# ShinYwings/SingleHDR-tf2

Hardware: AMD Instinct MI355X
Metric: HDR images/sec (512x512) end-to-end inference, deq+lin+hal (higher is better)
Workload: dtype f32

## Files before the change

include/shdr.h:

```cpp
#ifndef SHDR_H_
#define SHDR_H_

#include <stdint.h>

#ifdef __cplusplus
extern "C" {
#endif

void shdr_config_reload(void);

#define SHDR_OK          0
#define SHDR_E_SHAPE    (-1)
#define SHDR_E_ALIGN    (-2)
#define SHDR_E_ARCH     (-3)
#define SHDR_E_LAUNCH   (-4)
#define SHDR_E_NULL     (-5)

#define SHDR_ACT_NONE   0
#define SHDR_ACT_RELU   1
#define SHDR_ACT_LRELU  2
#define SHDR_ACT_TANH   3

#define SHDR_ALGO_AUTO    0
#define SHDR_ALGO_MFMA    1
#define SHDR_ALGO_DIRECT  2
#define SHDR_ALGO_MFMA_REG 3
#define SHDR_ALGO_MFMA_F16  4
#define SHDR_ALGO_MFMA_BF16 5
#define SHDR_ALGO_AUTO_F16  6
#define SHDR_ALGO_AUTO_BF16 7
#define SHDR_ALGO_AUTO_EXACT 8

const char* shdr_last_error(void);
const char* shdr_version(void);

uint32_t shdr_crc32c(const void* data, uint64_t n, uint32_t crc);

int shdr_same_pad(int in_size, int k, int stride, int* out_size, int* pad_before);

typedef struct shdr_conv2d_desc {
  int32_t N, H, W;
  int32_t C1, C2;
  int32_t Cout, KH, KW;
  int32_t stride;
  int32_t pad_t, pad_l;
  int32_t Ho, Wo;
  float   x2_scale;
  int32_t act1, act2;
  int32_t res_cstride;
  int32_t y_cstride;
  int32_t algo;
  int32_t cout_valid;
  int64_t w_batch_stride;
  int32_t y_pix_stride, y_off_h, y_off_w, y_H, y_W;
  int32_t prologue;
  int32_t pool;
} shdr_conv2d_desc;
enum { SHDR_POOL_MAX = 0, SHDR_POOL_AVG = 1 };
enum { SHDR_PROLOGUE_NONE = 0, SHDR_PROLOGUE_BILINEAR2X = 1,
       SHDR_PROLOGUE_RANGE_SCALE = 2 };

int shdr_conv2d_fwd_f32(const shdr_conv2d_desc* d,
                        const float* x1, const float* x2, const float* w,
                        const float* bias, const float* scale, const float* shift,
                        const float* residual, float* y, void* stream);

int shdr_conv2d_fwd_yrange_f32(const shdr_conv2d_desc* d,
                               const float* x1, const float* x2, const float* w,
                               const float* bias, const float* scale, const float* shift,
                               const float* residual, float* y, float* y_range, void* stream);

enum {
  SHDR_PLAN_DIRECT = 0,
  SHDR_PLAN_MFMA = 1,
  SHDR_PLAN_WINOGRAD_FUSED = 2,
  SHDR_PLAN_WINOGRAD_PLANES = 3,
  SHDR_PLAN_X3 = 4,
  SHDR_PLAN_X3N = 5
};
int shdr_conv2d_plan_f32(const shdr_conv2d_desc* d, int has_residual);
int64_t shdr_conv2d_prepared_filter_elems_f32(const shdr_conv2d_desc* d, int has_residual);
int shdr_conv2d_filter_is_plain_f32(const shdr_conv2d_desc* d, int has_residual);
int shdr_conv2d_prepare_filter_f32(const shdr_conv2d_desc* d, int has_residual, const float* w, float* prepared, void* stream);
int64_t shdr_conv2d_workspace_bytes_f32(const shdr_conv2d_desc* d, int has_residual);
int shdr_conv2d_fwd_prepared_f32(const shdr_conv2d_desc* d, const float* x1, const float* x2, const float* prepared,
                                 const float* bias, const float* scale, const float* shift, const float* residual, float* y,
                                 float* y_pool, void* workspace, void* stream);
int shdr_conv2d_fwd_prepared_ranged_f32(const shdr_conv2d_desc* d, const float* x1, const float* x2, const float* prepared,
                                        const float* bias, const float* scale, const float* shift, const float* residual, float* y,
                                        float* y_pool, void* workspace, const float* x1_range, const float* x2_range, float* y_range,
                                        void* stream);
int shdr_conv2d_projected_ok_f32(const shdr_conv2d_desc* d);
int shdr_conv2d_fwd_prepared_projected_f32(const shdr_conv2d_desc* d, const float* x1, const float* x2, const float* prepared,
                                           const float* bias, const float* scale, const float* shift, const float* proj, float* y_proj,
                                           float* y, float* y_pool, void* workspace, const float* x1_range, const float* x2_range,
                                           float* y_range, void* stream);

int shdr_conv2d_up2_lowres_ok_f32(const shdr_conv2d_desc* d);
int64_t shdr_conv2d_up2_lowres_filter_elems_f32(const shdr_conv2d_desc* d);
int shdr_conv2d_up2_lowres_prepare_filter_f32(const shdr_conv2d_desc* d, const float* w, float* prepared, void* stream);
int64_t shdr_conv2d_up2_lowres_workspace_bytes_f32(const shdr_conv2d_desc* d);
int shdr_conv2d_fwd_up2_lowres_f32(const shdr_conv2d_desc* d, const float* x, const float* prepared, const float* bias,
                                   const float* scale, const float* shift, float* y, void* workspace, const float* x_range,
                                   float* y_range, void* stream);

int shdr_conv2d_up2_fused_ok_f32(const shdr_conv2d_desc* d);
int shdr_conv2d_up2_narrow_enabled(void);
int64_t shdr_conv2d_up2_fused_filter_elems_f32(const shdr_conv2d_desc* d);
int shdr_conv2d_up2_fused_prepare_filter_f32(const shdr_conv2d_desc* d, const float* w, float* prepared, void* stream);
int shdr_conv2d_fwd_up2_fused_f32(const shdr_conv2d_desc* d, const float* x, const float* prepared, const float* bias,
                                  const float* scale, const float* shift, const float* proj, float* y_proj, float* y,
                                  const float* x_range, float* y_range, void* stream);

int shdr_conv2d_wgrad_f32(const shdr_conv2d_desc* d, const float* x, int which, const float* dz,
                          float* dw, void* stream);
int shdr_filter_transform_f32(const float* w, float* wt, int KH, int KW, int Cin, int Cout,
                              int c_begin, int c_count, float scale, void* stream);
int64_t shdr_conv2d_dgrad_workspace_bytes_f32(const shdr_conv2d_desc* d, int which);
int shdr_conv2d_dgrad_f32(const shdr_conv2d_desc* d, int which, const float* dz, const float* w, float* dx, void* workspace,
                          void* stream);
int shdr_conv2d_dgrad_tracks_range_f32(const shdr_conv2d_desc* d, int which);
int shdr_conv2d_dgrad_ranged_f32(const shdr_conv2d_desc* d, int which, const float* dz, const float* w, float* dx, void* workspace,
                                 const float* dz_range, float* dx_range, void* stream);
enum { SHDR_OP_CONV2D_FWD = 0, SHDR_OP_CONV2D_DGRAD = 1, SHDR_OP_CONV2D_WGRAD_WINOGRAD = 2, SHDR_OP_BATCHNORM = 3,
       SHDR_OP_ACT_BWD_BIAS = 4  };
#define SHDR_BN_MAX_BLOCKS 1024
int64_t shdr_workspace_bytes(int op, const shdr_conv2d_desc* d, int arg);
int shdr_bias_grad_f32(const float* dz, float* db, int64_t npix, int C, void* stream);

int shdr_soft_hist_fwd_f32(const float* x, float* y, int64_t npix, int C, int B, void* stream);
int shdr_soft_hist_bwd_f32(const float* x, const float* dy, float* dx, int64_t npix, int C, int B, void* stream);

int shdr_lin_frontend_fwd_f32(const float* img, float* y, int N, int H, int W,
                              int y_channels, void* stream);

int shdr_avgpool2_fwd_f32(const float* x, float* y, int N, int H, int W, int C, void* stream);
int shdr_maxpool2_fwd_f32(const float* x, float* y, int N, int H, int W, int C, void* stream);
int shdr_maxpool3s2_fwd_f32(const float* x, float* y, int N, int H, int W, int C, void* stream);
int shdr_resize2x_fwd_f32(const float* x, float* y, int N, int H, int W, int C, void* stream);
int shdr_gap_fwd_f32(const float* x, float* y, int N, int HW, int C, void* stream);

int shdr_invcrf_decode_fwd_f32(const float* feat, const float* wfc, const float* bfc,
                               const float* table, float* out, int B, int F, int K,
                               void* stream);
int shdr_increase_fwd_f32(const float* rf, float* out, int B, int K, void* stream);
int shdr_apply_rf_fwd_f32(const float* x, const float* rf, float* y, int B,
                          int64_t n_per_batch, int K, void* stream);

int shdr_clip_fwd_f32(const float* x, float* y, int64_t n, float lo, float hi, void* stream);
int shdr_vgg_preprocess_fwd_f32(const float* x, float* y, int64_t npix, int out_channels,
                                void* stream);
int shdr_reverse3_fwd_f32(const float* x, float* y, int64_t npix, void* stream);
int shdr_alpha_blend_fwd_f32(const float* b, const float* hal, float* a, float* alpha_out,
                             int64_t npix, float thr, void* stream);
int shdr_pack3_fwd_f32(const float* s0, const float* s1, const float* s2, const float* s3,
                       int nsrc, float* y, int out_channels, int64_t npix, void* stream);
int shdr_pad_channels_f32(const float* x, float* y, int64_t npix, int Cin, int Cout, void* stream);
int shdr_logc_fwd_f32(const float* x, float* y, int64_t n, void* stream);
int shdr_affine_act_f32(const float* x, const float* scale, const float* shift, const float* residual, float* y,
                        int64_t npix, int C, int act, void* stream);

int shdr_act_bwd_f32(const float* dy, const float* y, float* dx, int64_t n, int act, void* stream);
int shdr_clip_bwd_f32(const float* dy, const float* x, float* dx, int64_t n, float lo, float hi, void* stream);
int shdr_add_f32(const float* a, const float* b, float* y, int64_t n, void* stream);
int shdr_add_ranged_f32(const float* a, const float* b, float* y, int64_t n, float* y_range, void* stream);
int shdr_avgpool2_bwd_f32(const float* dy, float* dx, int N, int H, int W, int C, void* stream);
int shdr_maxpool2_bwd_f32(const float* x, const float* dy, float* dx, int N, int H, int W, int C, void* stream);
int shdr_maxpool3s2_bwd_f32(const float* x, const float* y, const float* dy, float* dx, int N, int H, int W, int C, void* stream);
int shdr_resize2x_bwd_f32(const float* dy, float* dx, int N, int H, int W, int C, void* stream);
int shdr_resize2x_bwd_ranged_f32(const float* dy, float* dx, int N, int H, int W, int C, float* dx_range, void* stream);
int shdr_gap_bwd_f32(const float* dy, float* dx, int N, int HW, int C, void* stream);
int shdr_upsample_zero2_f32(const float* dy, float* dx, int N, int H, int W, int C, void* stream);
int shdr_bn_stats_f32(const float* x, double* ws, float* mean, float* var, float* moving_mean,
                      float* moving_var, int64_t npix, int C, float momentum, void* stream);
int shdr_bn_train_apply_f32(const float* x, const float* mean, const float* var, const float* gamma,
                            const float* beta, float* y, int64_t npix, int C, float eps, int relu,
                            void* stream);
int shdr_bn_train_apply_ranged_f32(const float* x, const float* mean, const float* var, const float* gamma, const float* beta, float* y,
                                   int64_t npix, int C, float eps, int relu, float* y_range, void* stream);
int shdr_bn_bwd_f32(const float* dy, const float* x, const float* y_relu, const float* mean,
                    const float* var, const float* gamma, double* ws, float* dgamma, float* dbeta,
                    float* dx, int64_t npix, int C, float eps, void* stream);
int shdr_bn_bwd_ranged_f32(const float* dy, const float* x, const float* y_relu, const float* mean,
                           const float* var, const float* gamma, double* ws, float* dgamma, float* dbeta,
                           float* dx, int64_t npix, int C, float eps, float* dx_range, void* stream);
int shdr_invcrf_decode_bwd_f32(const float* dinv, const float* feat, const float* wfc,
                               const float* table, float* dfeat, float* dwfc, float* dbfc, int B,
                               int F, int K, void* stream);
int shdr_increase_bwd_f32(const float* rf, const float* dout, float* drf, int B, int K, void* stream);
int shdr_apply_rf_bwd_f32(const float* x, const float* rf, const float* dy, float* drf, float* dx,
                          int B, int64_t n_per_batch, int K, void* stream);
int shdr_diff_loss_f32(const float* a, const float* b, float* out, int B, int64_t n_per_sample,
                       int mode, void* stream);
int shdr_diff_loss_bwd_f32(const float* a, const float* b, const float* g, float* da, int B,
                           int64_t n_per_sample, int mode, int accumulate, void* stream);
int shdr_tv_loss_f32(const float* y, float* out, int N, int H, int W, int C, void* stream);
int shdr_tv_loss_bwd_f32(const float* y, const float* g, float* dy, int N, int H, int W, int C,
                         int accumulate, void* stream);
int shdr_logc_bwd_f32(const float* dy, const float* x, float* dx, int64_t n, void* stream);
int shdr_alpha_mask_f32(const float* x, float* alpha, int64_t npix, float thr, void* stream);
int shdr_alpha_blend_bwd_f32(const float* dA, const float* alpha, float* dhal, int64_t npix, void* stream);
int shdr_vgg_preprocess_bwd_f32(const float* dy, float* dx, int64_t npix, int in_channels, void* stream);
int shdr_adam_f32(float* p, const float* g, float* m, float* v, int64_t n, float lr_t, float beta1,
                  float beta2, float eps, float grad_scale, void* stream);

int shdr_winograd_filter_f32(const float* w, float* u, int Cin, int Cout, void* stream);
int64_t shdr_winograd_tiles(int N, int H, int W);
int shdr_winograd_input_f32(const float* x, float* v, int N, int H, int W, int C, void* stream);
int shdr_winograd_output_f32(const float* m, float* y, const float* bias, const float* scale,
                             const float* shift, int N, int H, int W, int C, int act1, int act2,
                             void* stream);

int shdr_lin_frontend_bwd_f32(const float* img, const float* dF, float* dimg, int N, int H, int W,
                              int y_channels, void* stream);
int shdr_alpha_blend_full_bwd_f32(const float* b, const float* hal, const float* dA, float* dB,
                                  float* dhal, int64_t npix, float thr, void* stream);
int shdr_unpack3_f32(const float* y, float* o0, float* o1, float* o2, float* o3, int nout,
                     int channels, int64_t npix, void* stream);
int shdr_sample_dot_f32(const float* a, const float* b, float* out, int B, int64_t n_per_sample, void* stream);
int shdr_mean_norm_fwd_f32(const float* r, const float* sum, float* out, int B, int64_t n_per_sample,
                           float eps, float target, void* stream);
int shdr_mean_norm_bwd_f32(const float* g, const float* sum, const float* gdot, float* dr, int B,
                           int64_t n_per_sample, float eps, float target, void* stream);

int shdr_act_bwd_bias_f32(const float* dy, const float* y, float* dz, float* db, float* ws, int64_t npix, int C, int act, void* stream);

int shdr_winograd_filter_packed_f32(const float* w, float* up, int Cin, int Cout, void* stream);
int shdr_conv2d_winograd_fused_f32(const float* x, const float* u, const float* bias, const float* scale,
                                   const float* shift, float* y, int N, int H, int W, int Cin, int Cout,
                                   int act1, int act2, void* stream);

int shdr_conv2d_winograd_fused2_f32(const float* x, const float* x2, const float* u, const float* bias,
                                    const float* scale, const float* shift, float* y, float* y_pool, int N, int H, int W,
                                    int C1, int C2, int Cout, int act1, int act2, void* stream);

int shdr_conv2d_winograd_fused_up2_f32(const float* x, const float* u, const float* bias, const float* scale,
                                       const float* shift, float* y, int N, int H, int W, int Cin, int Cout,
                                       int act1, int act2, void* stream);

int shdr_conv2d_x3_ok_f32(const shdr_conv2d_desc* d);
int64_t shdr_conv2d_x3_filter_elems_f32(const shdr_conv2d_desc* d);
int shdr_conv2d_x3_prepare_filter_f32(const shdr_conv2d_desc* d, const float* w, float* prepared, void* stream);
int shdr_conv2d_x3_input_absmax_f32(const float* x, int64_t n, float* prepared, void* stream);
int shdr_conv2d_fwd_x3_f32(const shdr_conv2d_desc* d, const float* x1, const float* x2, const float* prepared, const float* bias,
                           const float* scale, const float* shift, float* y, float* y_pool, void* stream);
int shdr_conv2d_fwd_x3_ranged_f32(const shdr_conv2d_desc* d, const float* x1, const float* x2, const float* prepared, const float* bias,
                                  const float* scale, const float* shift, float* y, float* y_pool, const float* x1_range,
                                  const float* x2_range, float* y_range, void* stream);
int shdr_conv2d_fwd_x3_residual_f32(const shdr_conv2d_desc* d, const float* x1, const float* x2, const float* prepared, const float* bias,
                                    const float* scale, const float* shift, const float* residual, float* y, const float* x1_range,
                                    const float* x2_range, float* y_range, void* stream);
int shdr_conv2d_fwd_x3_projected_f32(const shdr_conv2d_desc* d, const float* x1, const float* x2, const float* prepared, const float* bias,
                                     const float* scale, const float* shift, const float* proj, float* y_proj, float* y, float* y_pool,
                                     const float* x1_range, const float* x2_range, float* y_range, void* stream);
int shdr_absmax_f32(const float* x, int64_t n, float* range, void* stream);

int shdr_conv2d_x3n_ok_f32(const shdr_conv2d_desc* d);
int64_t shdr_conv2d_x3n_filter_elems_f32(const shdr_conv2d_desc* d);
int shdr_conv2d_x3n_prepare_filter_f32(const shdr_conv2d_desc* d, const float* w, float* prepared, void* stream);
int shdr_conv2d_fwd_x3n_f32(const shdr_conv2d_desc* d, const float* x1, const float* x2, const float* prepared, const float* bias,
                            const float* scale, const float* shift, const float* residual, float* y, float* y_pool, void* stream);
int shdr_conv2d_fwd_x3n_ranged_f32(const shdr_conv2d_desc* d, const float* x1, const float* x2, const float* prepared, const float* bias,
                                   const float* scale, const float* shift, const float* residual, float* y, float* y_pool,
                                   const float* x1_range, const float* x2_range, float* y_range, void* stream);

int shdr_x3_split_planes_f32(const float* x, int64_t n, const float* range, void* hi, void* lo, void* stream);
int shdr_conv2d_wgrad_x3_ok_f32(const shdr_conv2d_desc* d, int which);
int shdr_conv2d_wgrad_x3_f32(const shdr_conv2d_desc* d, const void* xh, const void* xl, int which, const void* zh, const void* zl,
                             const float* x_range, const float* z_range, float* dw, void* stream);

int shdr_conv2d_wgrad_winograd_f32(const float* x, const float* dz, float* du, float* dw, int N, int H, int W, int Cx,
                                   int Cout, int Ct, int ci_off, float x_scale, void* stream);

int shdr_u8_to_unit_f32(const uint8_t* x, float* y, int64_t npix, int reverse_channels, void* stream);
int shdr_resize_cubic_f32(const float* x, float* y, int N, int H, int W, int C, int Ho, int Wo, void* stream);
int shdr_pad_symmetric_f32(const float* x, float* y, int N, int H, int W, int C, int pad, void* stream);
int shdr_rgbe_encode_f32(const float* x, uint8_t* y, int64_t npix, int reverse_channels, void* stream);

int64_t shdr_rgbe_rle_encode(const uint8_t* rgbe, int width, int height, uint8_t* out, int64_t capacity);
int64_t shdr_rgbe_rle_decode(const uint8_t* data, int64_t size, int width, int height, uint8_t* rgbe);

#define SHDR_RLE_STAGES 4
int shdr_rgbe_rle_encode_batch_sizes(const int32_t* shapes, int n_images, int64_t* out_bytes, int64_t* workspace_bytes);
int shdr_rgbe_rle_encode_batch(const uint8_t* rgbe, const int32_t* shapes, const int32_t* shapes_dev, int n_images, uint8_t* out,
                               int64_t out_capacity, int64_t* offsets, void* workspace, void* stream);
int shdr_rgbe_rle_encode_batch_timed(const uint8_t* rgbe, const int32_t* shapes, const int32_t* shapes_dev, int n_images, uint8_t* out,
                                     int64_t out_capacity, int64_t* offsets, void* workspace, void* stream, float* stage_ms);

#define SHDR_RGBE_DEC_OK               0
#define SHDR_RGBE_DEC_TRUNCATED        1
#define SHDR_RGBE_DEC_CORRUPT_RUN      2
#define SHDR_RGBE_DEC_CORRUPT_LITERAL  3
#define SHDR_RGBE_DEC_TRUNCATED_FLAT   4
#define SHDR_RGBE_DEC_FALLBACK         5
int64_t shdr_rgbe_rle_decode_status(const uint8_t* data, int64_t size, int width, int height, uint8_t* rgbe, int* status, int* line,
                                    int64_t* stop);
#define SHDR_RGBE_DEC_STAGES 4
int shdr_rgbe_rle_decode_batch_sizes(const int32_t* shapes, const int64_t* src_off, int n_files, int64_t* out_bytes,
                                     int64_t* workspace_bytes);
int shdr_rgbe_rle_decode_batch(const uint8_t* src, int64_t src_bytes, const int64_t* src_off, const int64_t* src_off_dev,
                               const int32_t* shapes, const int32_t* shapes_dev, int n_files, uint8_t* out, int64_t out_bytes,
                               int64_t* out_off_dev, void* workspace, int64_t workspace_bytes, int32_t* status, int32_t* line,
                               int64_t* consumed, void* stream, float* stage_ms);

int shdr_hdr_load_resize_f32(const uint8_t* rgbe, float* y, int H0, int W0, int H, int W, void* stream);
int shdr_hdr_window_means_f32(const float* arena, const int64_t* offsets, const int32_t* dims, int n_files, float* partials,
                              float* means, void* stream);
int shdr_hdr_patch_sample_f32(const float* arena, const int64_t* offsets, const int32_t* dims, const float* means,
                              const int32_t* params, int param_stride, int N, int n_files, int P, float* y, void* stream);

#define SHDR_EXR_HALF   1
#define SHDR_EXR_FLOAT  2
int64_t shdr_exr_rle_decode(const uint8_t* data, int64_t size, uint8_t* out, int64_t capacity);
int shdr_exr_unpredict_u8(const uint8_t* payload, uint8_t* out, int64_t size, const int64_t* chunk_off, const uint8_t* coded,
                          int n_chunks, void* stream);
int shdr_exr_load_resize_f32(const uint8_t* planes, int64_t size, const int64_t* chunk_off, int n_chunks, int lines,
                             int64_t row_bytes, const int64_t* chan_off, const int32_t* chan_type, int H0, int W0, float* y,
                             int H, int W, int clip, void* stream);

#define SHDR_INFLATE_OK               0
#define SHDR_INFLATE_TRUNCATED        1
#define SHDR_INFLATE_HEADER           2
#define SHDR_INFLATE_DICTIONARY       3
#define SHDR_INFLATE_BLOCK_TYPE       4
#define SHDR_INFLATE_STORED_LENGTH    5
#define SHDR_INFLATE_COUNTS           6
#define SHDR_INFLATE_CODE_LENGTH_SET  7
#define SHDR_INFLATE_REPEAT           8
#define SHDR_INFLATE_RUN              9
#define SHDR_INFLATE_NO_END_OF_BLOCK 10
#define SHDR_INFLATE_LITERAL_SET     11
#define SHDR_INFLATE_DISTANCE_SET    12
#define SHDR_INFLATE_LITERAL_CODE    13
#define SHDR_INFLATE_DISTANCE_CODE   14
#define SHDR_INFLATE_DISTANCE_FAR    15
#define SHDR_INFLATE_OVERFLOW        16
#define SHDR_INFLATE_SHORT           17
#define SHDR_INFLATE_CHECKSUM        18
#define SHDR_INFLATE_RAW_SIZE        19
#define SHDR_INFLATE_MODE            20
int64_t shdr_inflate_host(const uint8_t* src, int64_t n, uint8_t* dst, int64_t capacity, int* status);
#define SHDR_INFLATE_STAGES 1
int shdr_inflate_batch_sizes(const int64_t* src_off, const int64_t* dst_off, int n_chunks, int64_t* src_bytes, int64_t* dst_bytes);
int shdr_inflate_batch(const uint8_t* src, int64_t src_bytes, const int64_t* src_off, const int64_t* src_off_dev, uint8_t* dst,
                       int64_t dst_bytes, const int64_t* dst_off, const int64_t* dst_off_dev, const uint8_t* mode, int n_chunks,
                       int32_t* status, int64_t* written, void* stream, float* stage_ms);

#define SHDR_PIZ_OK               0
#define SHDR_PIZ_TRUNCATED        1
#define SHDR_PIZ_BITMAP           2
#define SHDR_PIZ_LENGTH           3
#define SHDR_PIZ_NO_DATA          4
#define SHDR_PIZ_HUFF_HEADER      5
#define SHDR_PIZ_TABLE_TRUNCATED  6
#define SHDR_PIZ_TABLE_RUN        7
#define SHDR_PIZ_OVER_SUBSCRIBED  8
#define SHDR_PIZ_NBITS            9
#define SHDR_PIZ_BAD_CODE        10
#define SHDR_PIZ_DATA_TRUNCATED  11
#define SHDR_PIZ_RUN_NO_PREV     12
#define SHDR_PIZ_TOO_MANY        13
#define SHDR_PIZ_TOO_FEW         14
#define SHDR_PIZ_RAW_SIZE        15
#define SHDR_PIZ_MODE            16
int64_t shdr_piz_decode_host(const uint8_t* src, int64_t n, int width, int rows, const int32_t* chan_words, int n_chan, uint8_t* dst,
                             int64_t capacity, int* status);
#define SHDR_PIZ_STAGES 2
#define SHDR_PIZ_ROUND_STATS 9
int shdr_piz_batch_sizes(const int64_t* src_off, const int64_t* dst_off, const int32_t* geom, const int32_t* chan_words, int n_words,
                         int n_chunks, int sub_bits, int64_t* src_bytes, int64_t* dst_bytes, int64_t* workspace_bytes);
int shdr_piz_batch(const uint8_t* src, int64_t src_bytes, const int64_t* src_off, const int64_t* src_off_dev, uint8_t* dst,
                   int64_t dst_bytes, const int64_t* dst_off, const int64_t* dst_off_dev, const uint8_t* mode, const int32_t* geom,
                   const int32_t* geom_dev, const int32_t* chan_words, const int32_t* chan_words_dev, int n_words, int n_chunks,
                   int sub_bits, void* workspace, int64_t workspace_bytes, int32_t* status, int64_t* written, int32_t* rounds,
                   void* stream, float* stage_ms);

int64_t shdr_deflate_huffman_host(const uint8_t* src, int64_t n, uint8_t* dst, int64_t capacity);
int shdr_deflate_huffman_lengths_host(const uint8_t* src, int64_t n, uint8_t* lengths);
#define SHDR_DEFLATE_STAGES 3
#define SHDR_DEFLATE_TILE 1024
int shdr_deflate_huffman_batch_sizes(const int64_t* offsets, int n_chunks, int pad, int64_t* out_bytes, int64_t* workspace_bytes);
int shdr_deflate_huffman_batch(const uint8_t* data, const uint8_t* raw, const int64_t* offsets, const int64_t* offsets_dev,
                               int n_chunks, int pad, uint8_t* out, int64_t out_capacity, int64_t* out_offsets, uint8_t* coded,
                               void* workspace, void* stream, float* stage_ms);
int64_t shdr_deflate_lz_host(const uint8_t* src, int64_t n, uint8_t* dst, int64_t capacity);
#define SHDR_DEFLATE_LZ_LITERAL 0x80000000u
int shdr_deflate_lz_parse_host(const uint8_t* src, int64_t n, uint32_t* tokens);
#define SHDR_DEFLATE_LZ_TILE 1024
int shdr_deflate_lz_batch_sizes(const int64_t* offsets, int n_chunks, int pad, int64_t* out_bytes, int64_t* workspace_bytes);
int shdr_deflate_lz_batch(const uint8_t* data, const uint8_t* raw, const int64_t* offsets, const int64_t* offsets_dev,
                          int n_chunks, int pad, uint8_t* out, int64_t out_capacity, int64_t* out_offsets, uint8_t* coded,
                          void* workspace, void* stream, float* stage_ms);

int shdr_exr_pack_sizes(const int32_t* shapes, int n_images, int pixel_type, int lines, int64_t* n_chunks, int64_t* bytes,
                        int64_t* table, int64_t* chunk_off);
int shdr_exr_pack_f32(const float* pixels, const int32_t* shapes, int n_images, int pixel_type, int lines, int reverse_channels,
                      int saturate, const int64_t* table_dev, const int64_t* chunk_off, uint8_t* planar, uint8_t* predicted,
                      void* stream);
int shdr_exr_finish_chunks(uint8_t* records, uint8_t* tables, const int64_t* out_offsets, const int64_t* table_dev,
                           const int64_t* header_len, int n_images, int64_t n_chunks, int lines, void* stream);

int shdr_philox4x32_10(const uint32_t counter[4], const uint32_t key[2], uint32_t out[4]);
int shdr_camera_expose_f32(const float* hdr, const float* t, float* hdr_t, float* clipped, int N, int H, int W,
                           uint64_t seed, void* stream);
int shdr_jpeg_round_trip_f32(const float* ldr, const int32_t* quality, float* jpeg, float* loss_mask,
                             uint8_t* ws_planes, int32_t* ws_counts, int N, int H, int W, void* stream);

int shdr_flip_rot90_f32(const float* x, float* y, const int32_t* flip, const int32_t* rot, int N, int S, int C,
                        float divisor, void* stream);

int shdr_pair_patch_stats(const uint8_t* ldr, const float* hdr, int64_t arena_pixels, const int64_t* images_host,
                          const int64_t* images, int n_images, const int32_t* patches_host, const int32_t* patches, int n_patches,
                          int size, int32_t* count, float* mean, void* stream);
int shdr_pair_patch_gather_f32(const uint8_t* ldr, const float* hdr, int64_t arena_pixels, const int64_t* images_host,
                               const int64_t* images, int n_images, const int32_t* patches_host, const int32_t* patches,
                               int n_patches, const float* mean, const int32_t* samples_host, const int32_t* samples, int b, int size,
                               float* out_ldr, float* out_hdr, void* stream);


int64_t shdr_conv2d_packed_filter_elems_f16(int KH, int KW, int C1, int C2, int Cout);
int shdr_conv2d_pack_filter_f16(const float* w, void* wp, int KH, int KW, int C1, int C2, int Cout, float x2_scale, void* stream);
int shdr_conv2d_fwd_f16(const shdr_conv2d_desc* d, const void* x1, const void* x2, const void* wp, const float* bias, void* y,
                        int y_is_f32, void* stream);
int shdr_conv2d_fwd_fused_f16(const shdr_conv2d_desc* d, const void* x1, const void* x2, const void* wp, const float* bias,
                              const float* scale, const float* shift, const void* residual, int residual_is_f32, void* y, int y_is_f32,
                              void* stream);
int shdr_conv2d_wgrad_f16(const shdr_conv2d_desc* d, const void* x, int which, const void* dz, int dz_channels, int c1_rows,
                          int c2_rows, float* dw, void* stream);
int shdr_conv2d_patch_ok_f16(const shdr_conv2d_desc* d);
int shdr_conv2d_fwd_patch_f16(const shdr_conv2d_desc* d, const void* x1, const void* x2, const void* wp, const float* bias, void* y,
                              int y_is_f32, void* stream);
int shdr_conv2d_w3_ok_f16(const shdr_conv2d_desc* d);
int shdr_conv2d_fwd_w3_f16(const shdr_conv2d_desc* d, const void* x1, const void* x2, const void* wp, const float* bias, void* y,
                           void* stream);
int shdr_conv2d_wgrad_alltaps_ok_f16(const shdr_conv2d_desc* d, int which, int dz_channels);
int shdr_conv2d_wgrad_alltaps_f16(const shdr_conv2d_desc* d, const void* x, int which, const void* dz, int dz_channels, int c1_rows,
                                  int c2_rows, float* dw, void* stream);
int shdr_cast_f32_to_f16(const float* x, void* y, int64_t n, void* stream);
int shdr_cast_f16_to_f32(const void* x, float* y, int64_t n, void* stream);
int shdr_pad_channels_f32_to_f16(const float* x, void* y, int64_t npix, int Cin, int Cout, void* stream);
int shdr_pack3_f16(const float* s0, const float* s1, const float* s2, const float* s3, int nsrc, void* y, int out_channels,
                   int64_t npix, int vgg_preprocess, void* stream);
int shdr_unpack3_f16(const void* y, float* o0, float* o1, float* o2, float* o3, int nout, int channels, int64_t npix,
                     int vgg_preprocess_bwd, void* stream);
int shdr_act_bwd_bias_f16(const void* dy, const void* y, void* dz, float* db, float* ws, int64_t npix, int C, int act, void* stream);
int shdr_add_f16(const void* a, const void* b, void* y, int64_t n, int relu, void* stream);
int shdr_avgpool2_fwd_f16(const void* x, void* y, int N, int H, int W, int C, void* stream);
int shdr_avgpool2_bwd_f16(const void* dy, void* dx, int N, int H, int W, int C, void* stream);
int shdr_maxpool2_fwd_f16(const void* x, void* y, int N, int H, int W, int C, void* stream);
int shdr_maxpool2_bwd_f16(const void* x, const void* dy, void* dx, int N, int H, int W, int C, void* stream);
int shdr_maxpool3s2_fwd_f16(const void* x, void* y, int N, int H, int W, int C, void* stream);
int shdr_maxpool3s2_bwd_f16(const void* x, const void* y, const void* dy, void* dx, int N, int H, int W, int C, void* stream);
int shdr_resize2x_fwd_f16(const void* x, void* y, int N, int H, int W, int C, void* stream);
int shdr_resize2x_bwd_f16(const void* dy, void* dx, int N, int H, int W, int C, void* stream);
int shdr_upsample_zero2_f16(const void* dy, void* dx, int N, int H, int W, int C, void* stream);
int shdr_gap_fwd_f16(const void* x, float* y, int N, int HW, int C, void* stream);
int shdr_gap_bwd_f16(const float* dy, void* dx, int N, int HW, int C, void* stream);
int shdr_bn_stats_f16(const void* x, double* ws, float* mean, float* var, float* moving_mean, float* moving_var, int64_t npix, int C,
                      float momentum, void* stream);
int shdr_bn_train_apply_f16(const void* x, const float* mean, const float* var, const float* gamma, const float* beta, void* y,
                            int64_t npix, int C, float eps, int relu, void* stream);
int shdr_bn_bwd_f16(const void* dy, const void* x, const void* y_relu, const float* mean, const float* var, const float* gamma,
                    double* ws, float* dgamma, float* dbeta, void* dx, int64_t npix, int C, float eps, void* stream);
int shdr_lin_frontend_fwd_f16(const float* img, void* y, int N, int H, int W, int y_channels, void* stream);
int shdr_lin_frontend_bwd_f16(const float* img, const void* dF, float* dimg, int N, int H, int W, int y_channels, void* stream);

int64_t shdr_metrics_workspace_bytes(int N, int H, int W);
int shdr_pair_moments_f32(const float* pred, const float* gt, int N, int H, int W, int normalise, double* scale_pred,
                          double* scale_gt, double* peak, void* workspace, void* stream);
#define SHDR_METRICS_TILE_H 16
#define SHDR_METRICS_TILE_W 32
int shdr_hdr_metrics_f32(const float* pred, const float* gt, int N, int H, int W, float mu, const double* scale_pred,
                         const double* scale_gt, const double* peak, double* mse_l, double* mse_mu, double* l1_logc,
                         double* ssim_mu, void* workspace, void* stream);
int shdr_tonemap_u8_f32(const float* x, const double* scale, const double* peak, uint8_t* y, int N, int H, int W, float mu,
                        int reverse_channels, void* stream);

#define SHDR_JPEG_HUFF_BYTES 1416
#define SHDR_JPEG_TABLE_BYTES (512 + 4 * SHDR_JPEG_HUFF_BYTES)
#define SHDR_JPEG_E_CODE 1
#define SHDR_JPEG_E_BITS 2
#define SHDR_JPEG_E_OVERRUN 3
typedef struct shdr_jpeg_component {
  int32_t h, v;
  int32_t tq, dc_slot, ac_slot;
  int32_t bw, bh;
  int32_t blk_off;
  int32_t plane_off;
  int32_t cw, ch;
} shdr_jpeg_component;
typedef struct shdr_jpeg_image {
  int64_t blk_off;
  int64_t plane_off;
  int64_t out_off;
  int64_t table_off;
  int32_t width, height, ncomp;
  int32_t mcus_x, mcus_y, blocks_per_mcu, restart_interval;
  int32_t first_wg, n_wg;
  int32_t reserved, reserved2;
  shdr_jpeg_component comp[3];
} shdr_jpeg_image;
#define SHDR_JPEG_SEG_FIELDS 6
#define SHDR_JPEG_SEG_DWORD 0
#define SHDR_JPEG_SEG_BITS 1
#define SHDR_JPEG_SEG_FIRST_SUB 2
#define SHDR_JPEG_SEG_FIRST_BLOCK 3
#define SHDR_JPEG_SEG_BLOCKS 4
#define SHDR_JPEG_SEG_IMAGE 5
#define SHDR_JPEG_STAGES 6
typedef struct shdr_jpeg_batch {
  const uint8_t* data;
  const uint8_t* tables;
  const shdr_jpeg_image* images;
  const shdr_jpeg_image* images_dev;
  const int32_t* segs;
  const int32_t* segs_dev;
  const int32_t* sub_seg;
  const int32_t* sub_seg_dev;
  int32_t* passes;
  float* stage_ms;
  int64_t data_bytes, table_bytes, n_sub, n_blocks, plane_bytes, out_bytes;
  int32_t n_images, n_segs, subseq_bits, reserved;
} shdr_jpeg_batch;
int64_t shdr_jpeg_workspace_bytes(int64_t n_sub, int64_t n_blocks, int64_t plane_bytes);
int shdr_jpeg_entropy_decode(const shdr_jpeg_batch* batch, int16_t* coef, int32_t* errors, void* workspace, void* stream);
int shdr_jpeg_decode_u8(const shdr_jpeg_batch* batch, int16_t* coef, uint8_t* out, int32_t* errors, void* workspace, void* stream);
int shdr_jpeg_sync_rounds(const void* workspace, int64_t n_sub, int64_t n_blocks, int64_t plane_bytes, int32_t* rounds, void* stream);

#define SHDR_JPEG_SCAN_TILE 4096
typedef struct shdr_jpeg_scan_image {
  int64_t offset;
  int64_t length;
  int64_t first_tile;
  int32_t seg_cap;
  int32_t first_bound;
  int32_t first_seg;
  int32_t reserved;
} shdr_jpeg_scan_image;
typedef struct shdr_jpeg_scan_report {
  int64_t end;
  int64_t kept;
  int32_t n_rst;
  int32_t fill;
  int32_t end_marker;
// ... 45 lines not shown
```

singlehdr-tf2_amd/_lib.py:

```python
import ctypes
import os

_HERE = os.path.dirname(os.path.abspath(__file__))
LIB_PATH = os.environ.get("SHDR_LIB") or os.path.join(_HERE, "libshdr.so")

c_int = ctypes.c_int
c_i64 = ctypes.c_int64
c_f32 = ctypes.c_float
c_ptr = ctypes.c_void_p


class ConvDesc(ctypes.Structure):
    _fields_ = [("N", ctypes.c_int32), ("H", ctypes.c_int32), ("W", ctypes.c_int32),
                ("C1", ctypes.c_int32), ("C2", ctypes.c_int32),
                ("Cout", ctypes.c_int32), ("KH", ctypes.c_int32), ("KW", ctypes.c_int32),
                ("stride", ctypes.c_int32), ("pad_t", ctypes.c_int32), ("pad_l", ctypes.c_int32),
                ("Ho", ctypes.c_int32), ("Wo", ctypes.c_int32),
                ("x2_scale", ctypes.c_float),
                ("act1", ctypes.c_int32), ("act2", ctypes.c_int32),
                ("res_cstride", ctypes.c_int32), ("y_cstride", ctypes.c_int32),
                ("algo", ctypes.c_int32), ("cout_valid", ctypes.c_int32),
                ("w_batch_stride", ctypes.c_int64),
                ("y_pix_stride", ctypes.c_int32), ("y_off_h", ctypes.c_int32), ("y_off_w", ctypes.c_int32),
                ("y_H", ctypes.c_int32), ("y_W", ctypes.c_int32),
                ("prologue", ctypes.c_int32), ("pool", ctypes.c_int32)]


OP_CONV2D_FWD, OP_CONV2D_DGRAD, OP_CONV2D_WGRAD_WINOGRAD, OP_BATCHNORM, OP_ACT_BWD_BIAS = 0, 1, 2, 3, 4

SIGNATURES = {
    "shdr_last_error": (ctypes.c_char_p, []),
    "shdr_version": (ctypes.c_char_p, []),
    "shdr_u8_to_unit_f32": (c_int, [c_ptr, c_ptr, c_i64, c_int, c_ptr]),
    "shdr_resize_cubic_f32": (c_int, [c_ptr, c_ptr, c_int, c_int, c_int, c_int, c_int, c_int, c_ptr]),
    "shdr_pad_symmetric_f32": (c_int, [c_ptr, c_ptr, c_int, c_int, c_int, c_int, c_int, c_ptr]),
    "shdr_rgbe_encode_f32": (c_int, [c_ptr, c_ptr, c_i64, c_int, c_ptr]),
    "shdr_rgbe_rle_encode": (c_i64, [c_ptr, c_int, c_int, c_ptr, c_i64]),
    "shdr_rgbe_rle_decode": (c_i64, [c_ptr, c_i64, c_int, c_int, c_ptr]),
    "shdr_rgbe_rle_encode_batch_sizes": (c_int, [c_ptr, c_int, ctypes.POINTER(c_i64), ctypes.POINTER(c_i64)]),
    "shdr_rgbe_rle_encode_batch": (c_int, [c_ptr, c_ptr, c_ptr, c_int, c_ptr, c_i64, c_ptr, c_ptr, c_ptr]),
    "shdr_rgbe_rle_encode_batch_timed": (c_int, [c_ptr, c_ptr, c_ptr, c_int, c_ptr, c_i64, c_ptr, c_ptr, c_ptr, c_ptr]),
    "shdr_rgbe_rle_decode_status": (c_i64, [c_ptr, c_i64, c_int, c_int, c_ptr, ctypes.POINTER(c_int), ctypes.POINTER(c_int),
                                            ctypes.POINTER(c_i64)]),
    "shdr_rgbe_rle_decode_batch_sizes": (c_int, [c_ptr, c_ptr, c_int, ctypes.POINTER(c_i64), ctypes.POINTER(c_i64)]),
    "shdr_rgbe_rle_decode_batch": (c_int, [c_ptr, c_i64, c_ptr, c_ptr, c_ptr, c_ptr, c_int, c_ptr, c_i64, c_ptr, c_ptr, c_i64, c_ptr, c_ptr,
                                           c_ptr, c_ptr, c_ptr]),
    "shdr_hdr_load_resize_f32": (c_int, [c_ptr, c_ptr, c_int, c_int, c_int, c_int, c_ptr]),
    "shdr_hdr_window_means_f32": (c_int, [c_ptr, c_ptr, c_ptr, c_int, c_ptr, c_ptr, c_ptr]),
    "shdr_hdr_patch_sample_f32": (c_int, [c_ptr] * 5 + [c_int] * 4 + [c_ptr, c_ptr]),
    "shdr_exr_rle_decode": (c_i64, [c_ptr, c_i64, c_ptr, c_i64]),
    "shdr_exr_unpredict_u8": (c_int, [c_ptr, c_ptr, c_i64, c_ptr, c_ptr, c_int, c_ptr]),
    "shdr_exr_load_resize_f32": (c_int, [c_ptr, c_i64, c_ptr, c_int, c_int, c_i64, c_ptr, c_ptr, c_int, c_int, c_ptr, c_int, c_int,
                                         c_int, c_ptr]),
    "shdr_deflate_huffman_host": (c_i64, [c_ptr, c_i64, c_ptr, c_i64]),
    "shdr_deflate_huffman_lengths_host": (c_int, [c_ptr, c_i64, c_ptr]),
    "shdr_deflate_huffman_batch_sizes": (c_int, [c_ptr, c_int, c_int, ctypes.POINTER(c_i64), ctypes.POINTER(c_i64)]),
    "shdr_deflate_huffman_batch": (c_int, [c_ptr, c_ptr, c_ptr, c_ptr, c_int, c_int, c_ptr, c_i64, c_ptr, c_ptr, c_ptr, c_ptr, c_ptr]),
    "shdr_deflate_lz_host": (c_i64, [c_ptr, c_i64, c_ptr, c_i64]),
    "shdr_deflate_lz_parse_host": (c_int, [c_ptr, c_i64, c_ptr]),
    "shdr_deflate_lz_batch_sizes": (c_int, [c_ptr, c_int, c_int, ctypes.POINTER(c_i64), ctypes.POINTER(c_i64)]),
    "shdr_deflate_lz_batch": (c_int, [c_ptr, c_ptr, c_ptr, c_ptr, c_int, c_int, c_ptr, c_i64, c_ptr, c_ptr, c_ptr, c_ptr, c_ptr]),
    "shdr_inflate_host": (c_i64, [c_ptr, c_i64, c_ptr, c_i64, ctypes.POINTER(c_int)]),
    "shdr_inflate_batch_sizes": (c_int, [c_ptr, c_ptr, c_int, ctypes.POINTER(c_i64), ctypes.POINTER(c_i64)]),
    "shdr_piz_decode_host": (c_i64, [c_ptr, c_i64, c_int, c_int, c_ptr, c_int, c_ptr, c_i64, ctypes.POINTER(c_int)]),
    "shdr_piz_batch_sizes": (c_int, [c_ptr, c_ptr, c_ptr, c_ptr, c_int, c_int, c_int] + [ctypes.POINTER(c_i64)] * 3),
    "shdr_piz_batch": (c_int, [c_ptr, c_i64, c_ptr, c_ptr, c_ptr, c_i64, c_ptr, c_ptr, c_ptr, c_ptr, c_ptr, c_ptr, c_ptr, c_int, c_int, c_int,
                               c_ptr, c_i64, c_ptr, c_ptr, c_ptr, c_ptr, c_ptr]),
    "shdr_inflate_batch": (c_int, [c_ptr, c_i64, c_ptr, c_ptr, c_ptr, c_i64, c_ptr, c_ptr, c_ptr, c_int, c_ptr, c_ptr, c_ptr, c_ptr]),
    "shdr_exr_pack_sizes": (c_int, [c_ptr, c_int, c_int, c_int, ctypes.POINTER(c_i64), ctypes.POINTER(c_i64), c_ptr, c_ptr]),
    "shdr_exr_pack_f32": (c_int, [c_ptr, c_ptr, c_int, c_int, c_int, c_int, c_int, c_ptr, c_ptr, c_ptr, c_ptr, c_ptr]),
    "shdr_exr_finish_chunks": (c_int, [c_ptr, c_ptr, c_ptr, c_ptr, c_ptr, c_int, c_i64, c_int, c_ptr]),
    "shdr_philox4x32_10": (c_int, [c_ptr, c_ptr, c_ptr]),
    "shdr_camera_expose_f32": (c_int, [c_ptr, c_ptr, c_ptr, c_ptr, c_int, c_int, c_int, ctypes.c_uint64, c_ptr]),
    "shdr_jpeg_round_trip_f32": (c_int, [c_ptr] * 6 + [c_int, c_int, c_int, c_ptr]),
    "shdr_flip_rot90_f32": (c_int, [c_ptr, c_ptr, c_ptr, c_ptr, c_int, c_int, c_int, c_f32, c_ptr]),
    "shdr_pair_patch_stats": (c_int, [c_ptr, c_ptr, c_i64, c_ptr, c_ptr, c_int, c_ptr, c_ptr, c_int, c_int, c_ptr, c_ptr, c_ptr]),
    "shdr_pair_patch_gather_f32": (c_int, [c_ptr, c_ptr, c_i64, c_ptr, c_ptr, c_int, c_ptr, c_ptr, c_int, c_ptr, c_ptr, c_ptr, c_int,
                                           c_int, c_ptr, c_ptr, c_ptr]),
    "shdr_conv2d_winograd_fused_f32": (c_int, [c_ptr] * 6 + [c_int] * 7 + [c_ptr]),
    "shdr_conv2d_winograd_fused2_f32": (c_int, [c_ptr] * 8 + [c_int] * 8 + [c_ptr]),
    "shdr_conv2d_winograd_fused_up2_f32": (c_int, [c_ptr] * 6 + [c_int] * 7 + [c_ptr]),
    "shdr_conv2d_x3_ok_f32": (c_int, [ctypes.POINTER(ConvDesc)]),
    "shdr_conv2d_x3_filter_elems_f32": (c_i64, [ctypes.POINTER(ConvDesc)]),
    "shdr_conv2d_x3_prepare_filter_f32": (c_int, [ctypes.POINTER(ConvDesc), c_ptr, c_ptr, c_ptr]),
    "shdr_conv2d_fwd_x3_f32": (c_int, [ctypes.POINTER(ConvDesc)] + [c_ptr] * 9),
    "shdr_conv2d_fwd_x3_ranged_f32": (c_int, [ctypes.POINTER(ConvDesc)] + [c_ptr] * 12),
    "shdr_absmax_f32": (c_int, [c_ptr, c_i64, c_ptr, c_ptr]),
    "shdr_x3_split_planes_f32": (c_int, [c_ptr, c_i64, c_ptr, c_ptr, c_ptr, c_ptr]),
    "shdr_conv2d_wgrad_x3_ok_f32": (c_int, [ctypes.POINTER(ConvDesc), c_int]),
    "shdr_conv2d_wgrad_x3_f32": (c_int, [ctypes.POINTER(ConvDesc), c_ptr, c_ptr, c_int, c_ptr, c_ptr, c_ptr, c_ptr, c_ptr, c_ptr]),
    "shdr_config_reload": (None, []),
    "shdr_conv2d_x3_input_absmax_f32": (c_int, [c_ptr, c_i64, c_ptr, c_ptr]),
    "shdr_conv2d_x3n_ok_f32": (c_int, [ctypes.POINTER(ConvDesc)]),
    "shdr_conv2d_x3n_filter_elems_f32": (c_i64, [ctypes.POINTER(ConvDesc)]),
    "shdr_conv2d_x3n_prepare_filter_f32": (c_int, [ctypes.POINTER(ConvDesc), c_ptr, c_ptr, c_ptr]),
    "shdr_conv2d_fwd_x3n_f32": (c_int, [ctypes.POINTER(ConvDesc)] + [c_ptr] * 10),
    "shdr_conv2d_fwd_x3n_ranged_f32": (c_int, [ctypes.POINTER(ConvDesc)] + [c_ptr] * 13),
    "shdr_act_bwd_bias_f32": (c_int, [c_ptr, c_ptr, c_ptr, c_ptr, c_ptr, c_i64, c_int, c_int, c_ptr]),
    "shdr_winograd_filter_packed_f32": (c_int, [c_ptr, c_ptr, c_int, c_int, c_ptr]),
    "shdr_conv2d_wgrad_winograd_f32": (c_int, [c_ptr] * 4 + [c_int] * 7 + [c_f32, c_ptr]),
    "shdr_crc32c": (ctypes.c_uint32, [c_ptr, ctypes.c_uint64, ctypes.c_uint32]),
    "shdr_same_pad": (c_int, [c_int, c_int, c_int, ctypes.POINTER(c_int), ctypes.POINTER(c_int)]),
    "shdr_conv2d_fwd_f32": (c_int, [ctypes.POINTER(ConvDesc)] + [c_ptr] * 9),
    "shdr_conv2d_fwd_yrange_f32": (c_int, [ctypes.POINTER(ConvDesc)] + [c_ptr] * 10),
    "shdr_conv2d_plan_f32": (c_int, [ctypes.POINTER(ConvDesc), c_int]),
    "shdr_conv2d_prepared_filter_elems_f32": (c_i64, [ctypes.POINTER(ConvDesc), c_int]),
    "shdr_conv2d_filter_is_plain_f32": (c_int, [ctypes.POINTER(ConvDesc), c_int]),
    "shdr_conv2d_prepare_filter_f32": (c_int, [ctypes.POINTER(ConvDesc), c_int, c_ptr, c_ptr, c_ptr]),
    "shdr_conv2d_workspace_bytes_f32": (c_i64, [ctypes.POINTER(ConvDesc), c_int]),
    "shdr_conv2d_fwd_prepared_f32": (c_int, [ctypes.POINTER(ConvDesc)] + [c_ptr] * 11),
    "shdr_conv2d_fwd_prepared_ranged_f32": (c_int, [ctypes.POINTER(ConvDesc)] + [c_ptr] * 14),
    "shdr_conv2d_projected_ok_f32": (c_int, [ctypes.POINTER(ConvDesc)]),
    "shdr_conv2d_fwd_prepared_projected_f32": (c_int, [ctypes.POINTER(ConvDesc)] + [c_ptr] * 15),
    "shdr_conv2d_up2_lowres_ok_f32": (c_int, [ctypes.POINTER(ConvDesc)]),
    "shdr_conv2d_up2_lowres_filter_elems_f32": (c_i64, [ctypes.POINTER(ConvDesc)]),
    "shdr_conv2d_up2_lowres_prepare_filter_f32": (c_int, [ctypes.POINTER(ConvDesc), c_ptr, c_ptr, c_ptr]),
    "shdr_conv2d_up2_lowres_workspace_bytes_f32": (c_i64, [ctypes.POINTER(ConvDesc)]),
    "shdr_conv2d_fwd_up2_lowres_f32": (c_int, [ctypes.POINTER(ConvDesc)] + [c_ptr] * 10),
    "shdr_conv2d_up2_fused_ok_f32": (c_int, [ctypes.POINTER(ConvDesc)]),
    "shdr_conv2d_up2_narrow_enabled": (c_int, []),
    "shdr_conv2d_up2_fused_filter_elems_f32": (c_i64, [ctypes.POINTER(ConvDesc)]),
    "shdr_conv2d_up2_fused_prepare_filter_f32": (c_int, [ctypes.POINTER(ConvDesc), c_ptr, c_ptr, c_ptr]),
    "shdr_conv2d_fwd_up2_fused_f32": (c_int, [ctypes.POINTER(ConvDesc)] + [c_ptr] * 11),
    "shdr_conv2d_fwd_x3_projected_f32": (c_int, [ctypes.POINTER(ConvDesc)] + [c_ptr] * 14),
    "shdr_conv2d_fwd_x3_residual_f32": (c_int, [ctypes.POINTER(ConvDesc)] + [c_ptr] * 12),
    "shdr_conv2d_dgrad_workspace_bytes_f32": (c_i64, [ctypes.POINTER(ConvDesc), c_int]),
    "shdr_conv2d_dgrad_f32": (c_int, [ctypes.POINTER(ConvDesc), c_int, c_ptr, c_ptr, c_ptr, c_ptr, c_ptr]),
    "shdr_conv2d_dgrad_tracks_range_f32": (c_int, [ctypes.POINTER(ConvDesc), c_int]),
    "shdr_conv2d_dgrad_ranged_f32": (c_int, [ctypes.POINTER(ConvDesc), c_int, c_ptr, c_ptr, c_ptr, c_ptr, c_ptr, c_ptr, c_ptr]),
    "shdr_workspace_bytes": (c_i64, [c_int, ctypes.POINTER(ConvDesc), c_int]),
    "shdr_soft_hist_bwd_f32": (c_int, [c_ptr, c_ptr, c_ptr, c_i64, c_int, c_int, c_ptr]),
    "shdr_conv2d_wgrad_f32": (c_int, [ctypes.POINTER(ConvDesc), c_ptr, c_int, c_ptr, c_ptr, c_ptr]),
    "shdr_filter_transform_f32": (c_int, [c_ptr, c_ptr, c_int, c_int, c_int, c_int, c_int, c_int, c_f32, c_ptr]),
    "shdr_bias_grad_f32": (c_int, [c_ptr, c_ptr, c_i64, c_int, c_ptr]),
    "shdr_soft_hist_fwd_f32": (c_int, [c_ptr, c_ptr, c_i64, c_int, c_int, c_ptr]),
    "shdr_lin_frontend_fwd_f32": (c_int, [c_ptr, c_ptr, c_int, c_int, c_int, c_int, c_ptr]),
    "shdr_avgpool2_fwd_f32": (c_int, [c_ptr, c_ptr, c_int, c_int, c_int, c_int, c_ptr]),
    "shdr_maxpool2_fwd_f32": (c_int, [c_ptr, c_ptr, c_int, c_int, c_int, c_int, c_ptr]),
    "shdr_maxpool3s2_fwd_f32": (c_int, [c_ptr, c_ptr, c_int, c_int, c_int, c_int, c_ptr]),
    "shdr_resize2x_fwd_f32": (c_int, [c_ptr, c_ptr, c_int, c_int, c_int, c_int, c_ptr]),
    "shdr_gap_fwd_f32": (c_int, [c_ptr, c_ptr, c_int, c_int, c_int, c_ptr]),
    "shdr_invcrf_decode_fwd_f32": (c_int, [c_ptr] * 5 + [c_int, c_int, c_int, c_ptr]),
    "shdr_increase_fwd_f32": (c_int, [c_ptr, c_ptr, c_int, c_int, c_ptr]),
    "shdr_apply_rf_fwd_f32": (c_int, [c_ptr, c_ptr, c_ptr, c_int, c_i64, c_int, c_ptr]),
    "shdr_clip_fwd_f32": (c_int, [c_ptr, c_ptr, c_i64, c_f32, c_f32, c_ptr]),
    "shdr_vgg_preprocess_fwd_f32": (c_int, [c_ptr, c_ptr, c_i64, c_int, c_ptr]),
    "shdr_reverse3_fwd_f32": (c_int, [c_ptr, c_ptr, c_i64, c_ptr]),
    "shdr_alpha_blend_fwd_f32": (c_int, [c_ptr, c_ptr, c_ptr, c_ptr, c_i64, c_f32, c_ptr]),
    "shdr_pack3_fwd_f32": (c_int, [c_ptr] * 4 + [c_int, c_ptr, c_int, c_i64, c_ptr]),
    "shdr_logc_fwd_f32": (c_int, [c_ptr, c_ptr, c_i64, c_ptr]),
    "shdr_affine_act_f32": (c_int, [c_ptr] * 5 + [c_i64, c_int, c_int, c_ptr]),
    "shdr_pad_channels_f32": (c_int, [c_ptr, c_ptr, c_i64, c_int, c_int, c_ptr]),
    "shdr_act_bwd_f32": (c_int, [c_ptr, c_ptr, c_ptr, c_i64, c_int, c_ptr]),
    "shdr_clip_bwd_f32": (c_int, [c_ptr, c_ptr, c_ptr, c_i64, c_f32, c_f32, c_ptr]),
    "shdr_add_f32": (c_int, [c_ptr, c_ptr, c_ptr, c_i64, c_ptr]),
    "shdr_add_ranged_f32": (c_int, [c_ptr, c_ptr, c_ptr, c_i64, c_ptr, c_ptr]),
    "shdr_avgpool2_bwd_f32": (c_int, [c_ptr, c_ptr, c_int, c_int, c_int, c_int, c_ptr]),
    "shdr_maxpool2_bwd_f32": (c_int, [c_ptr, c_ptr, c_ptr, c_int, c_int, c_int, c_int, c_ptr]),
    "shdr_maxpool3s2_bwd_f32": (c_int, [c_ptr, c_ptr, c_ptr, c_ptr, c_int, c_int, c_int, c_int, c_ptr]),
    "shdr_resize2x_bwd_f32": (c_int, [c_ptr, c_ptr, c_int, c_int, c_int, c_int, c_ptr]),
    "shdr_resize2x_bwd_ranged_f32": (c_int, [c_ptr, c_ptr, c_int, c_int, c_int, c_int, c_ptr, c_ptr]),
    "shdr_gap_bwd_f32": (c_int, [c_ptr, c_ptr, c_int, c_int, c_int, c_ptr]),
    "shdr_upsample_zero2_f32": (c_int, [c_ptr, c_ptr, c_int, c_int, c_int, c_int, c_ptr]),
    "shdr_bn_stats_f32": (c_int, [c_ptr] * 6 + [c_i64, c_int, c_f32, c_ptr]),
    "shdr_bn_train_apply_f32": (c_int, [c_ptr] * 6 + [c_i64, c_int, c_f32, c_int, c_ptr]),
    "shdr_bn_train_apply_ranged_f32": (c_int, [c_ptr] * 6 + [c_i64, c_int, c_f32, c_int, c_ptr, c_ptr]),
    "shdr_bn_bwd_f32": (c_int, [c_ptr] * 10 + [c_i64, c_int, c_f32, c_ptr]),
    "shdr_bn_bwd_ranged_f32": (c_int, [c_ptr] * 10 + [c_i64, c_int, c_f32, c_ptr, c_ptr]),
    "shdr_invcrf_decode_bwd_f32": (c_int, [c_ptr] * 7 + [c_int, c_int, c_int, c_ptr]),
    "shdr_increase_bwd_f32": (c_int, [c_ptr, c_ptr, c_ptr, c_int, c_int, c_ptr]),
    "shdr_apply_rf_bwd_f32": (c_int, [c_ptr] * 5 + [c_int, c_i64, c_int, c_ptr]),
    "shdr_diff_loss_f32": (c_int, [c_ptr, c_ptr, c_ptr, c_int, c_i64, c_int, c_ptr]),
    "shdr_diff_loss_bwd_f32": (c_int, [c_ptr, c_ptr, c_ptr, c_ptr, c_int, c_i64, c_int, c_int, c_ptr]),
    "shdr_tv_loss_f32": (c_int, [c_ptr, c_ptr, c_int, c_int, c_int, c_int, c_ptr]),
    "shdr_tv_loss_bwd_f32": (c_int, [c_ptr, c_ptr, c_ptr, c_int, c_int, c_int, c_int, c_int, c_ptr]),
    "shdr_logc_bwd_f32": (c_int, [c_ptr, c_ptr, c_ptr, c_i64, c_ptr]),
    "shdr_alpha_mask_f32": (c_int, [c_ptr, c_ptr, c_i64, c_f32, c_ptr]),
    "shdr_alpha_blend_bwd_f32": (c_int, [c_ptr, c_ptr, c_ptr, c_i64, c_ptr]),
    "shdr_vgg_preprocess_bwd_f32": (c_int, [c_ptr, c_ptr, c_i64, c_int, c_ptr]),
    "shdr_winograd_filter_f32": (c_int, [c_ptr, c_ptr, c_int, c_int, c_ptr]),
    "shdr_winograd_tiles": (c_i64, [c_int, c_int, c_int]),
    "shdr_winograd_input_f32": (c_int, [c_ptr, c_ptr, c_int, c_int, c_int, c_int, c_ptr]),
    "shdr_winograd_output_f32": (c_int, [c_ptr] * 5 + [c_int, c_int, c_int, c_int, c_int, c_int, c_ptr]),
    "shdr_lin_frontend_bwd_f32": (c_int, [c_ptr, c_ptr, c_ptr, c_int, c_int, c_int, c_int, c_ptr]),
    "shdr_alpha_blend_full_bwd_f32": (c_int, [c_ptr] * 5 + [c_i64, c_f32, c_ptr]),
    "shdr_unpack3_f32": (c_int, [c_ptr] * 5 + [c_int, c_int, c_i64, c_ptr]),
    "shdr_sample_dot_f32": (c_int, [c_ptr, c_ptr, c_ptr, c_int, c_i64, c_ptr]),
    "shdr_mean_norm_fwd_f32": (c_int, [c_ptr, c_ptr, c_ptr, c_int, c_i64, c_f32, c_f32, c_ptr]),
    "shdr_mean_norm_bwd_f32": (c_int, [c_ptr, c_ptr, c_ptr, c_ptr, c_int, c_i64, c_f32, c_f32, c_ptr]),
    "shdr_conv2d_packed_filter_elems_f16": (c_i64, [c_int] * 5),
    "shdr_conv2d_pack_filter_f16": (c_int, [c_ptr, c_ptr] + [c_int] * 5 + [c_f32, c_ptr]),
    "shdr_conv2d_fwd_f16": (c_int, [ctypes.POINTER(ConvDesc)] + [c_ptr] * 5 + [c_int, c_ptr]),
    "shdr_conv2d_fwd_fused_f16": (c_int, [ctypes.POINTER(ConvDesc)] + [c_ptr] * 7 + [c_int, c_ptr, c_int, c_ptr]),
    "shdr_conv2d_wgrad_f16": (c_int, [ctypes.POINTER(ConvDesc), c_ptr, c_int, c_ptr, c_int, c_int, c_int, c_ptr, c_ptr]),
    "shdr_conv2d_patch_ok_f16": (c_int, [ctypes.POINTER(ConvDesc)]),
    "shdr_conv2d_fwd_patch_f16": (c_int, [ctypes.POINTER(ConvDesc)] + [c_ptr] * 5 + [c_int, c_ptr]),
    "shdr_conv2d_w3_ok_f16": (c_int, [ctypes.POINTER(ConvDesc)]),
    "shdr_conv2d_fwd_w3_f16": (c_int, [ctypes.POINTER(ConvDesc)] + [c_ptr] * 5 + [c_ptr]),
    "shdr_conv2d_wgrad_alltaps_ok_f16": (c_int, [ctypes.POINTER(ConvDesc), c_int, c_int]),
    "shdr_conv2d_wgrad_alltaps_f16": (c_int, [ctypes.POINTER(ConvDesc), c_ptr, c_int, c_ptr, c_int, c_int, c_int, c_ptr, c_ptr]),
    "shdr_cast_f32_to_f16": (c_int, [c_ptr, c_ptr, c_i64, c_ptr]),
    "shdr_cast_f16_to_f32": (c_int, [c_ptr, c_ptr, c_i64, c_ptr]),
    "shdr_pad_channels_f32_to_f16": (c_int, [c_ptr, c_ptr, c_i64, c_int, c_int, c_ptr]),
    "shdr_pack3_f16": (c_int, [c_ptr] * 4 + [c_int, c_ptr, c_int, c_i64, c_int, c_ptr]),
    "shdr_unpack3_f16": (c_int, [c_ptr] * 5 + [c_int, c_int, c_i64, c_int, c_ptr]),
    "shdr_act_bwd_bias_f16": (c_int, [c_ptr, c_ptr, c_ptr, c_ptr, c_ptr, c_i64, c_int, c_int, c_ptr]),
    "shdr_add_f16": (c_int, [c_ptr, c_ptr, c_ptr, c_i64, c_int, c_ptr]),
    "shdr_avgpool2_fwd_f16": (c_int, [c_ptr, c_ptr, c_int, c_int, c_int, c_int, c_ptr]),
    "shdr_avgpool2_bwd_f16": (c_int, [c_ptr, c_ptr, c_int, c_int, c_int, c_int, c_ptr]),
    "shdr_maxpool2_fwd_f16": (c_int, [c_ptr, c_ptr, c_int, c_int, c_int, c_int, c_ptr]),
    "shdr_maxpool2_bwd_f16": (c_int, [c_ptr, c_ptr, c_ptr, c_int, c_int, c_int, c_int, c_ptr]),
    "shdr_maxpool3s2_fwd_f16": (c_int, [c_ptr, c_ptr, c_int, c_int, c_int, c_int, c_ptr]),
    "shdr_maxpool3s2_bwd_f16": (c_int, [c_ptr, c_ptr, c_ptr, c_ptr, c_int, c_int, c_int, c_int, c_ptr]),
    "shdr_resize2x_fwd_f16": (c_int, [c_ptr, c_ptr, c_int, c_int, c_int, c_int, c_ptr]),
    "shdr_resize2x_bwd_f16": (c_int, [c_ptr, c_ptr, c_int, c_int, c_int, c_int, c_ptr]),
    "shdr_upsample_zero2_f16": (c_int, [c_ptr, c_ptr, c_int, c_int, c_int, c_int, c_ptr]),
    "shdr_gap_fwd_f16": (c_int, [c_ptr, c_ptr, c_int, c_int, c_int, c_ptr]),
    "shdr_gap_bwd_f16": (c_int, [c_ptr, c_ptr, c_int, c_int, c_int, c_ptr]),
    "shdr_bn_stats_f16": (c_int, [c_ptr] * 6 + [c_i64, c_int, c_f32, c_ptr]),
    "shdr_bn_train_apply_f16": (c_int, [c_ptr] * 6 + [c_i64, c_int, c_f32, c_int, c_ptr]),
    "shdr_bn_bwd_f16": (c_int, [c_ptr] * 10 + [c_i64, c_int, c_f32, c_ptr]),
    "shdr_lin_frontend_fwd_f16": (c_int, [c_ptr, c_ptr, c_int, c_int, c_int, c_int, c_ptr]),
    "shdr_lin_frontend_bwd_f16": (c_int, [c_ptr, c_ptr, c_ptr, c_int, c_int, c_int, c_int, c_ptr]),
    "shdr_adam_f32": (c_int, [c_ptr, c_ptr, c_ptr, c_ptr, c_i64, c_f32, c_f32, c_f32, c_f32, c_f32, c_ptr]),
    "shdr_metrics_workspace_bytes": (c_i64, [c_int, c_int, c_int]),
    "shdr_pair_moments_f32": (c_int, [c_ptr, c_ptr, c_int, c_int, c_int, c_int] + [c_ptr] * 5),
    "shdr_hdr_metrics_f32": (c_int, [c_ptr, c_ptr, c_int, c_int, c_int, c_f32] + [c_ptr] * 9),
    "shdr_tonemap_u8_f32": (c_int, [c_ptr] * 4 + [c_int] * 3 + [c_f32, c_int, c_ptr]),
    "shdr_jpeg_workspace_bytes": (c_i64, [c_i64, c_i64, c_i64]),
    "shdr_jpeg_entropy_decode": (c_int, [c_ptr] * 5),
    "shdr_jpeg_decode_u8": (c_int, [c_ptr] * 6),
    "shdr_jpeg_sync_rounds": (c_int, [c_ptr, c_i64, c_i64, c_i64, c_ptr, c_ptr]),
    "shdr_jpeg_scan_workspace_bytes": (c_i64, [c_int, c_i64]),
    "shdr_jpeg_scan": (c_int, [c_ptr, c_i64, c_ptr, c_ptr, c_int, c_ptr, c_ptr, c_i64, c_ptr, c_ptr, c_ptr]),
    "shdr_jpeg_compact": (c_int, [c_ptr, c_i64, c_ptr, c_ptr, c_int, c_ptr, c_i64, c_ptr, c_int, c_i64, c_ptr, c_i64, c_ptr, c_ptr, c_ptr]),
    "shdr_jpeg_scan_host": (c_int, [c_ptr, c_i64, c_ptr, c_int, c_ptr, c_ptr, c_i64, c_ptr, c_int, c_i64, c_ptr, c_i64]),
    "shdr_jpeg_encode_blocks": (c_i64, [c_ptr, ctypes.POINTER(c_i64)]),
    "shdr_jpeg_encode_header_host": (c_int, [c_ptr, c_ptr]),
    "shdr_jpeg_encode_transform_host": (c_i64, [c_ptr, c_ptr, c_ptr, c_i64]),
    "shdr_jpeg_encode_entropy_host": (c_i64, [c_ptr, c_i64, c_ptr, c_ptr, c_i64]),
    "shdr_jpeg_encode_host": (c_i64, [c_ptr, c_ptr, c_ptr, c_i64]),
    "shdr_jpeg_encode_batch_sizes": (c_int, [c_ptr, c_int] + [ctypes.POINTER(c_i64)] * 3),
    "shdr_jpeg_encode_batch": (c_int, [c_ptr, c_int, c_ptr, c_ptr, c_ptr, c_ptr, c_int, c_ptr, c_i64, c_ptr, c_ptr, c_ptr, c_ptr, c_ptr]),
    "shdr_jpeg_encode_entropy_batch": (c_int, [c_ptr, c_i64, c_ptr, c_ptr, c_int, c_ptr, c_i64, c_ptr, c_ptr, c_ptr, c_ptr, c_ptr]),
}

_lib = None


def load():
    global _lib
    if _lib is not None:
        return _lib
    if not os.path.exists(LIB_PATH):
        raise RuntimeError(
            "libshdr.so not found at %s -- build it with `python singlehdr-tf2_amd/build.py` "
            "(there is no CPU/PyTorch fallback for the hot path)" % LIB_PATH)
    lib = ctypes.CDLL(LIB_PATH)
    for name, (res, args) in SIGNATURES.items():
        fn = getattr(lib, name)
        fn.restype = res
        fn.argtypes = args
    _lib = lib
    return lib


def check(rc, what):
    if rc != 0:
        msg = load().shdr_last_error()
        raise RuntimeError("%s failed (code %d): %s" % (what, rc, msg.decode() if msg else ""))
```

singlehdr-tf2_amd/_ops.py:

```python
import collections
import ctypes
import math

import numpy as np
import torch

try:
    from . import _lib
except ImportError:
    import _lib

AUTOGRAD = None


def _needs_grad(*tensors):
    return AUTOGRAD is not None and torch.is_grad_enabled() and any(
        isinstance(t, torch.Tensor) and t.requires_grad for t in tensors)


WINOGRAD = True


ACT_NONE, ACT_RELU, ACT_LRELU, ACT_TANH = 0, 1, 2, 3
ALGO_AUTO, ALGO_MFMA, ALGO_DIRECT, ALGO_MFMA_REG = 0, 1, 2, 3
# ... 188 lines not shown
def conv2d_up2(x, w, bias=None, act1=ACT_NONE, scale=None, shift=None, act2=ACT_NONE, proj=None, lowres=False, one_launch=False):
    if lowres and proj is not None and not _is_h(x) and _AUTO_ALGO[PRECISION] == ALGO_AUTO and WINOGRAD and not EXACT_FP32 \
            and not _needs_grad(x, w, bias, scale, shift):
        yj = _conv2d_up2_fused(x, w, bias, act1, scale, shift, act2, proj)
        if yj is not None:
            return yj
    if lowres and proj is None and not _is_h(x) and _AUTO_ALGO[PRECISION] == ALGO_AUTO and WINOGRAD and not EXACT_FP32 \
            and not _needs_grad(x, w, bias, scale, shift):
        if one_launch and up2_narrow_enabled():
            y = _conv2d_up2_fused(x, w, bias, act1, scale, shift, act2)
            if y is not None:
                return y
        y = _conv2d_up2_lowres(x, w, bias, act1, scale, shift, act2)
        if y is not None:
            return y
    algo = _AUTO_ALGO[PRECISION]
    if _is_h(x) or algo != ALGO_AUTO or not WINOGRAD or _needs_grad(x, w, bias, scale, shift):
        if proj is not None:
            return None
        return conv2d(resize2x(x), w, bias, act1=act1, scale=scale, shift=shift, act2=act2)
    return _conv2d_raw(x, w, bias, 1, None, 1.0, act1, scale, shift, None, act2, algo, None, None, None, None, 0, None,
                       prologue=PROLOGUE_BILINEAR2X, proj=proj)


def up2_narrow_enabled():
    return bool(_lib.load().shdr_conv2d_up2_narrow_enabled())


def _up2_layer(form, x, w, bias, act1, scale, shift, act2):
    lib = _lib.load()
    x, w_var = _d(x), w
    w = _d(w)
    if x.dim() != 4 or w.dim() != 4 or tuple(w.shape[:2]) != (3, 3) or w.shape[2] != x.shape[3]:
        return None
    n, h, wd, c1 = x.shape
    cout = w.shape[3]
    d = _lib.ConvDesc()
    d.N, d.H, d.W, d.C1, d.C2 = n, 2 * h, 2 * wd, c1, 0
    d.Cout, d.KH, d.KW, d.stride = cout, 3, 3, 1
    d.cout_valid, d.y_cstride = cout, cout
    d.pad_t, d.pad_l, d.Ho, d.Wo = 1, 1, 2 * h, 2 * wd
    d.x2_scale = 1.0
    d.act1, d.act2 = act1, act2
    d.algo = ALGO_AUTO
    d.prologue = PROLOGUE_BILINEAR2X
    if not int(getattr(lib, "shdr_conv2d_up2_%s_ok_f32" % form)(ctypes.byref(d))):
        return None
    _chk(x, "x")
    _chk(w, "w")
    for t, nm in ((bias, "bias"), (scale, "scale"), (shift, "shift")):
        if t is not None and (_chk(_d(t), nm).numel() != cout):
            raise ValueError("conv2d_up2: %s must have %d elements" % (nm, cout))
    persistent = _is_persistent(w_var)
    nprep = int(getattr(lib, "shdr_conv2d_up2_%s_filter_elems_f32" % form)(ctypes.byref(d)))
    key = ("up2_" + form, c1, cout, nprep)
    prepared = _filter_cache_get(w_var, "_shdr_packed", key) if persistent else None
    if prepared is None:
        prepared = torch.empty(nprep, device=w.device, dtype=torch.float32)
        name = "shdr_conv2d_up2_%s_prepare_filter_f32" % form
        _lib.check(getattr(lib, name)(ctypes.byref(d), _ptr(w), _ptr(prepared), _stream()), name)
        if persistent:
            _filter_cache_put(w_var, "_shdr_packed", key, prepared)
    return d, x, prepared


def _conv2d_up2_lowres(x, w, bias, act1, scale, shift, act2):
    layer = _up2_layer("lowres", x, w, bias, act1, scale, shift, act2)
    if layer is None:
        return None
    lib = _lib.load()
    x_in = x
    d, x, prepared = layer
    xr = _range_of(x_in)
    if xr is None:
        RANGE_MISSES[(tuple(x.shape), None, tuple(_d(w).shape))] += 1
    ws = torch.empty(int(lib.shdr_conv2d_up2_lowres_workspace_bytes_f32(ctypes.byref(d))), device=x.device, dtype=torch.uint8)
    out = torch.empty((d.N, d.H, d.W, d.Cout), device=x.device, dtype=torch.float32)
    yr = _new_slot(x.device)
    rc = lib.shdr_conv2d_fwd_up2_lowres_f32(ctypes.byref(d), _ptr(x), _ptr(prepared), _ptr(_d(bias)), _ptr(_d(scale)), _ptr(_d(shift)),
                                            _ptr(out), _ptr(ws), _ptr(xr), _ptr(yr), _stream())
    _lib.check(rc, "shdr_conv2d_fwd_up2_lowres_f32")
    return _set_range(out, yr)


def _conv2d_up2_fused(x, w, bias, act1, scale, shift, act2, proj=None, want_y=None):
    if proj is not None and _d(w).shape[-1] != 64:
        return None
    layer = _up2_layer("fused", x, w, bias, act1, scale, shift, act2)
    if layer is None:
        return None
    lib = _lib.load()
    x_in = x
    d, x, prepared = layer
    if proj is not None:
        proj = _chk(_d(proj), "proj")
        if tuple(proj.shape) != (3, d.Cout):
            raise ValueError("conv2d_up2: proj must be [3, %d]" % d.Cout)
    if want_y is None:
        want_y = proj is None
    xr = _range_of(x_in)
    if xr is None:
        RANGE_MISSES[(tuple(x.shape), None, tuple(_d(w).shape))] += 1
        xr = _new_slot(x.device)
        _lib.check(lib.shdr_absmax_f32(_ptr(x), x.numel(), _ptr(xr), _stream()), "shdr_absmax_f32")
    out = torch.empty((d.N, d.H, d.W, d.Cout), device=x.device, dtype=torch.float32) if want_y else None
    yj = torch.empty((d.N, d.H, d.W, 3), device=x.device, dtype=torch.float32) if proj is not None else None
    yr = _new_slot(x.device) if want_y else None
    rc = lib.shdr_conv2d_fwd_up2_fused_f32(ctypes.byref(d), _ptr(x), _ptr(prepared), _ptr(_d(bias)), _ptr(_d(scale)), _ptr(_d(shift)),
                                           _ptr(proj), _ptr(yj), _ptr(out), _ptr(xr), _ptr(yr), _stream())
    _lib.check(rc, "shdr_conv2d_fwd_up2_fused_f32")
    if proj is not None:
        PROJECTED_LAUNCHES[0] += 1
    if want_y:
        _set_range(out, yr)
    return out if proj is None else ((yj, out) if want_y else yj)


def _conv2d_raw(x, w, bias, stride, x2, x2_scale, act1, scale, shift, residual, act2, algo, out, cout_valid, pad, out_hw,
                w_batch_stride, pool, prologue=0, proj=None):
    lib = _lib.load()
    x_in, x2_in = x, x2
    x = _chk(_d(x), "x")
    w_var = w
    w = _chk(_d(w), "w")
    n, h, wd, c1 = x.shape
    if prologue == PROLOGUE_BILINEAR2X:
        h, wd = 2 * h, 2 * wd
    kh, kw, cin, cout_gemm = w.shape
    cout = cout_gemm if cout_valid is None else int(cout_valid)
    c2 = 0
    if x2 is not None:
        x2 = _chk(_d(x2), "x2")
        if x2.shape[:3] != x.shape[:3]:
            raise ValueError("conv2d: x2 spatial shape %s != x %s" % (tuple(x2.shape), tuple(x.shape)))
        c2 = x2.shape[3]
    if cin != c1 + c2:
        raise ValueError("conv2d: filter expects %d input channels, got %d+%d" % (cin, c1, c2))
    ho, pt = same_pad(h, kh, stride)
    wo, pl = same_pad(wd, kw, stride)
    if pad is not None:
        pt, pl = pad
    if out_hw is not None:
        ho, wo = out_hw
    d = _lib.ConvDesc()
    d.N, d.H, d.W, d.C1, d.C2 = n, h, wd, c1, c2
    d.Cout, d.KH, d.KW, d.stride = cout_gemm, kh, kw, stride
    d.cout_valid = cout
    d.pad_t, d.pad_l, d.Ho, d.Wo = pt, pl, ho, wo
    d.x2_scale = float(x2_scale)
    d.act1, d.act2 = act1, act2
    d.algo = _auto(algo)
    d.w_batch_stride = int(w_batch_stride)
    d.prologue = int(prologue)
    d.pool = POOL_AVG if pool == "avg" else POOL_MAX
    res_cs = 0
    if residual is not None:
        residual = _chk(_d(residual), "residual")
        if tuple(residual.shape[:3]) != (n, ho, wo) or residual.shape[3] < cout:
            raise ValueError("conv2d: residual shape %s incompatible with output [%d,%d,%d,%d]"
                             % (tuple(residual.shape), n, ho, wo, cout))
        res_cs = residual.shape[3]
    d.res_cstride = res_cs
    if proj is not None:
        if algo != ALGO_AUTO or not WINOGRAD or residual is not None or not int(lib.shdr_conv2d_projected_ok_f32(ctypes.byref(d))):
            return None
        proj = _chk(_d(proj), "proj")
        if tuple(proj.shape) != (3, cout):
            raise ValueError("conv2d: proj must be [3, %d]" % cout)
    elif out is None:
        out = None if pool == "only" else torch.empty((n, ho, wo, cout), device=x.device, dtype=torch.float32)
    else:
        _chk(out, "out")
        if tuple(out.shape) != (n, ho, wo, cout):
            raise ValueError("conv2d: bad out shape")
        _set_range(out, None)
    d.y_cstride = cout
    for t, nm, ln in ((bias, "bias", cout), (scale, "scale", cout), (shift, "shift", cout)):
        if t is not None and (_chk(_d(t), nm).numel() != ln):
            raise ValueError("conv2d: %s must have %d elements" % (nm, ln))
    if algo != ALGO_AUTO or not WINOGRAD:
        if pool:
            raise ValueError("conv2d: the pooled output needs algo AUTO")
        rc = lib.shdr_conv2d_fwd_f32(ctypes.byref(d), _ptr(x), _ptr(x2), _ptr(w), _ptr(_d(bias)),
                                     _ptr(_d(scale)), _ptr(_d(shift)), _ptr(residual), _ptr(out), _stream())
        _lib.check(rc, "shdr_conv2d_fwd_f32")
        return out
    has_res = int(residual is not None)
    prepared = _prepared_filter(lib, w_var, d, has_res)
    plan = int(lib.shdr_conv2d_plan_f32(ctypes.byref(d), has_res))
    split = plan in (4, 5)
    xr1 = _range_of(x_in) if split else None
    xr2 = _range_of(x2_in) if (split and x2 is not None) else None
    if split and (xr1 is None or (x2 is not None and xr2 is None)):
        RANGE_MISSES[(tuple(x.shape), None if x2 is None else tuple(x2.shape), tuple(w.shape))] += 1
    ws = None
    nws = int(lib.shdr_conv2d_workspace_bytes_f32(ctypes.byref(d), has_res))
    if nws > 256 or (nws > 0 and (not split or xr1 is None or (x2 is not None and xr2 is None))):
        ws = torch.empty(nws, device=x.device, dtype=torch.uint8)
    yp = None
    if pool:
        if ho % 2 or wo % 2:
            raise ValueError("conv2d: pool needs even output height / width")
        yp = torch.empty((n, ho // 2, wo // 2, cout), device=x.device, dtype=torch.float32)
        if out is None and plan not in (2, 4):
            out = torch.empty((n, ho, wo, cout), device=x.device, dtype=torch.float32)
    yr = _new_slot(x.device) if (split or (plan in (0, 1) and prologue == PROLOGUE_NONE and out is not None)) else None
    if proj is not None:
        yj = torch.empty((n, ho, wo, 3), device=x.device, dtype=torch.float32)
        rc = lib.shdr_conv2d_fwd_prepared_projected_f32(ctypes.byref(d), _ptr(x), _ptr(x2), _ptr(prepared), _ptr(_d(bias)), _ptr(_d(scale)),
                                                        _ptr(_d(shift)), _ptr(proj), _ptr(yj), None, _ptr(yp), _ptr(ws), _ptr(xr1),
                                                        _ptr(xr2), _ptr(yr), _stream())
        _lib.check(rc, "shdr_conv2d_fwd_prepared_projected_f32")
        PROJECTED_LAUNCHES[0] += 1
        if yp is not None:
            _set_range(yp, yr)
        return (yj, yp) if pool else yj
    rc = lib.shdr_conv2d_fwd_prepared_ranged_f32(ctypes.byref(d), _ptr(x), _ptr(x2), _ptr(prepared), _ptr(_d(bias)), _ptr(_d(scale)),
                                                 _ptr(_d(shift)), _ptr(residual), _ptr(out), _ptr(yp), _ptr(ws), _ptr(xr1), _ptr(xr2),
                                                 _ptr(yr), _stream())
    _lib.check(rc, "shdr_conv2d_fwd_prepared_ranged_f32")
    if yr is not None:
        for t in (out, yp):
            if t is not None:
                _set_range(t, yr)
    if pool == "only":
        return yp
    return (out, yp) if pool else out


def _is_persistent(w):
    return (w.requires_grad and w.is_leaf) or getattr(w, "_shdr_const", False)


def _filter_cache_get(w, attr, key):
    store = getattr(w, attr, None)
    if store is None or store[0] != w._version:
        return None
    ent = store[1].get(key)
    if ent is None:
        return None
    tensor, stream_id, event = ent
    if event is not None and torch.cuda.current_stream().cuda_stream != stream_id and not torch.cuda.is_current_stream_capturing() \
            and not event.query():
        torch.cuda.current_stream().wait_event(event)
    return tensor


def _filter_cache_put(w, attr, key, tensor):
    store = getattr(w, attr, None)
    if store is None or store[0] != w._version:
        store = (w._version, {})
        setattr(w, attr, store)
    event = None
    if not torch.cuda.is_current_stream_capturing():
        event = torch.cuda.Event()
        event.record()
    store[1][key] = (tensor, torch.cuda.current_stream().cuda_stream, event)
    return tensor


def clear_filter_caches(w):
    for attr in ("_shdr_packed", "_shdr_packed_h", "_shdr_wino"):
        if hasattr(w, attr):
            delattr(w, attr)


def _prepared_filter(lib, w, d, has_res):
    if int(lib.shdr_conv2d_filter_is_plain_f32(ctypes.byref(d), has_res)):
        return _d(w)
    persistent = _is_persistent(w)
    key = None
    if persistent:
        key = (int(lib.shdr_conv2d_plan_f32(ctypes.byref(d), has_res)), d.C1, d.C2, float(d.x2_scale))
        cached = _filter_cache_get(w, "_shdr_packed", key)
        if cached is not None:
            return cached
    n = int(lib.shdr_conv2d_prepared_filter_elems_f32(ctypes.byref(d), has_res))
    prepared = torch.empty(n, device=w.device, dtype=torch.float32)
    _lib.check(lib.shdr_conv2d_prepare_filter_f32(ctypes.byref(d), has_res, _ptr(_d(w)), _ptr(prepared), _stream()),
               "shdr_conv2d_prepare_filter_f32")
    if persistent:
        _filter_cache_put(w, "_shdr_packed", key, prepared)
    return prepared


_PLAN_NAMES = {0: "direct", 1: "mfma", 2: "fused", 3: "planes", 4: "x3", 5: "x3n"}


def conv2d_plan(x_shape, w_shape, c2=0, stride=1, x2_scale=1.0, has_residual=False, cout_valid=None):
    lib = _lib.load()
    n, h, wd, c1 = x_shape
    kh, kw, cin, cout = w_shape
    d = _lib.ConvDesc()
    d.N, d.H, d.W, d.C1, d.C2 = n, h, wd, c1, c2
    d.Cout, d.KH, d.KW, d.stride = cout, kh, kw, stride
    d.cout_valid = cout_valid or cout
    d.Ho, d.pad_t = same_pad(h, kh, stride)
    d.Wo, d.pad_l = same_pad(wd, kw, stride)
    d.x2_scale = float(x2_scale)
    d.algo = _auto(ALGO_AUTO) if WINOGRAD else ALGO_MFMA
    return _PLAN_NAMES[int(lib.shdr_conv2d_plan_f32(ctypes.byref(d), int(has_residual)))]


def winograd_path(cin, cout):
    p = conv2d_plan((1, 64, 64, cin), (3, 3, cin, cout))
    return p if p in ("fused", "planes") else None


def conv2d_dgrad(dz, w, x_shape, c1, c2, which, stride=1, x2_scale=1.0):
    lib = _lib.load()
    dz_in = dz
    dz, w = _chk(_d(dz), "dz"), _chk(_d(w), "w")
    n, h, wd, cx = x_shape
    kh, kw, cin, cout = w.shape
    if cin != c1 + c2 or cx != (c2 if which else c1):
        raise ValueError("conv2d_dgrad: filter %s / sources %d+%d / x %s do not match" % (tuple(w.shape), c1, c2, tuple(x_shape)))
    d = _lib.ConvDesc()
    d.N, d.H, d.W, d.C1, d.C2 = n, h, wd, c1, c2
    d.Cout, d.KH, d.KW, d.stride = cout, kh, kw, stride
    d.cout_valid = dz.shape[3]
    d.Ho, d.pad_t = same_pad(h, kh, stride)
    d.Wo, d.pad_l = same_pad(wd, kw, stride)
    d.x2_scale = float(x2_scale)
    d.algo = _auto(_AUTO_ALGO[PRECISION]) if WINOGRAD or PRECISION != "fp32" else ALGO_MFMA
    if tuple(dz.shape[:3]) != (n, d.Ho, d.Wo) or dz.shape[3] > cout:
        raise ValueError("conv2d_dgrad: dz shape %s does not match the forward output" % (tuple(dz.shape),))
    nws = int(lib.shdr_conv2d_dgrad_workspace_bytes_f32(ctypes.byref(d), int(which)))
    if nws < 0:
        raise ValueError("conv2d_dgrad: bad descriptor")
    ws = torch.empty(max(nws, 16), device=dz.device, dtype=torch.uint8)
    dx = torch.empty(tuple(x_shape), device=dz.device, dtype=torch.float32)
    zr = _range_of(dz_in)
    xr = _new_slot(dz.device) if int(lib.shdr_conv2d_dgrad_tracks_range_f32(ctypes.byref(d), int(which))) else None
    if zr is None and xr is not None:
        RANGE_MISSES[("dgrad", tuple(dz.shape), tuple(w.shape))] += 1
    _lib.check(lib.shdr_conv2d_dgrad_ranged_f32(ctypes.byref(d), int(which), _ptr(dz), _ptr(w), _ptr(dx), _ptr(ws), _ptr(zr), _ptr(xr), _stream()),
               "shdr_conv2d_dgrad_ranged_f32")
    if xr is not None:
        _set_range(dx, xr)
    return dx


def soft_hist_bwd(img, dy, max_bin):
    lib = _lib.load()
    img, dy = _chk(_d(img), "img"), _chk(_d(dy), "dy")
    c = img.shape[-1]
    dx = torch.empty_like(img)
    _lib.check(lib.shdr_soft_hist_bwd_f32(_ptr(img), _ptr(dy), _ptr(dx), img.numel() // c, c, int(max_bin), _stream()), "shdr_soft_hist_bwd_f32")
    return dx


def _nhwc_op(fn_name, x, out_shape):
    lib = _lib.load()
    x_in = x
    if _is_h(x):
        x = _chkh(_d(x), "x")
        fn_name = fn_name[:-4] + "_f16"
    else:
        x = _chk(_d(x), "x")
    n, h, w, c = x.shape
    y = torch.empty(out_shape, device=x.device, dtype=x.dtype)
    rc = getattr(lib, fn_name)(_ptr(x), _ptr(y), n, h, w, c, _stream())
    _lib.check(rc, fn_name)
    return _carry_range(y, x_in)


def avgpool2(x):
    if _needs_grad(x):
        return AUTOGRAD.avgpool2(x)
    n, h, w, c = x.shape
    return _nhwc_op("shdr_avgpool2_fwd_f32", x, (n, h // 2, w // 2, c))


def maxpool2(x):
    if _needs_grad(x):
        return AUTOGRAD.maxpool2(x)
    n, h, w, c = x.shape
    return _nhwc_op("shdr_maxpool2_fwd_f32", x, (n, h // 2, w // 2, c))


def maxpool3s2(x):
    if _needs_grad(x):
        return AUTOGRAD.maxpool3s2(x)
    n, h, w, c = x.shape
    return _nhwc_op("shdr_maxpool3s2_fwd_f32", x, (n, same_pad(h, 3, 2)[0], same_pad(w, 3, 2)[0], c))


def resize2x(x):
    if _needs_grad(x):
        return AUTOGRAD.resize2x(x)
    n, h, w, c = x.shape
    return _nhwc_op("shdr_resize2x_fwd_f32", x, (n, 2 * h, 2 * w, c))


def global_avg_pool(x):
    if _needs_grad(x):
        return AUTOGRAD.global_avg_pool(x)
    lib = _lib.load()
    n, h, w, c = x.shape
    y = torch.empty((n, c), device=x.device, dtype=torch.float32)
    if _is_h(x):
        _lib.check(lib.shdr_gap_fwd_f16(_ptr(_chkh(_d(x), "x")), _ptr(y), n, h * w, c, _stream()), "shdr_gap_fwd_f16")
        return y
    x = _chk(_d(x), "x")
    _lib.check(lib.shdr_gap_fwd_f32(_ptr(x), _ptr(y), n, h * w, c, _stream()), "shdr_gap_fwd_f32")
    return y


def soft_hist(img, max_bin):
    lib = _lib.load()
    img = _chk(_d(img), "img")
    c = img.shape[-1]
    npix = img.numel() // c
    y = torch.empty(tuple(img.shape[:-1]) + (int(max_bin) * c,), device=img.device, dtype=torch.float32)
    _lib.check(lib.shdr_soft_hist_fwd_f32(_ptr(img), _ptr(y), npix, c, int(max_bin), _stream()),
               "shdr_soft_hist_fwd_f32")
    return y


def lin_frontend(img, channels=96, dtype=None):
    dtype = dtype or (HALF if native_fp16() else torch.float32)
    if _needs_grad(img):
        return AUTOGRAD.lin_frontend(img, channels, dtype)
    lib = _lib.load()
    img_in = img
    img = _chk(_d(img), "img")
    n, h, w, c = img.shape
    if c != 3:
        raise ValueError("lin_frontend: expected 3 channels, got %d" % c)
    y = torch.empty((n, h, w, channels), device=img.device, dtype=dtype)
    fn = "shdr_lin_frontend_fwd_f16" if dtype == HALF else "shdr_lin_frontend_fwd_f32"
    _lib.check(getattr(lib, fn)(_ptr(img), _ptr(y), n, h, w, channels, _stream()), fn)
    b = _bound_of(img_in)
    return y if b is None else set_bound(y, max(1.0, 8.0 * b))


def invcrf_decode(feat, wfc, bfc, table):
    if _needs_grad(feat, wfc, bfc):
        return AUTOGRAD.invcrf_decode(feat, wfc, bfc, table)
    lib = _lib.load()
    feat, wfc, bfc, table = (_chk(_d(t), nm) for t, nm in
                             ((feat, "feat"), (wfc, "wfc"), (bfc, "bfc"), (table, "table")))
    b, f = feat.shape
    k = table.shape[0]
    if tuple(wfc.shape) != (f, 11) or bfc.numel() != 11 or tuple(table.shape) != (k, 12):
        raise ValueError("invcrf_decode: expected wfc [F,11], bfc [11], table [K,12]")
    out = torch.empty((b, k), device=feat.device, dtype=torch.float32)
    _lib.check(lib.shdr_invcrf_decode_fwd_f32(_ptr(feat), _ptr(wfc), _ptr(bfc), _ptr(table), _ptr(out),
                                              b, f, k, _stream()), "shdr_invcrf_decode_fwd_f32")
    return out


def increase(rf):
    if _needs_grad(rf):
        return AUTOGRAD.increase(rf)
    lib = _lib.load()
    rf = _chk(_d(rf), "rf")
    b, k = rf.shape
    out = torch.empty_like(rf)
    _lib.check(lib.shdr_increase_fwd_f32(_ptr(rf), _ptr(out), b, k, _stream()), "shdr_increase_fwd_f32")
    return out


def apply_rf(x, rf):
    if _needs_grad(x, rf):
        return AUTOGRAD.apply_rf(x, rf)
    lib = _lib.load()
    x = _chk(_d(x), "x")
    rf = _chk(_d(rf), "rf")
    b = x.shape[0]
    if rf.shape[0] != b:
        raise ValueError("apply_rf: batch mismatch %d vs %d" % (b, rf.shape[0]))
    y = torch.empty_like(x)
    _lib.check(lib.shdr_apply_rf_fwd_f32(_ptr(x), _ptr(rf), _ptr(y), b, x.numel() // b, rf.shape[1],
                                         _stream()), "shdr_apply_rf_fwd_f32")
    return y


def clip(x, lo, hi):
    if _needs_grad(x):
        return AUTOGRAD.clip(x, lo, hi)
    lib = _lib.load()
    x = _chk(_d(x), "x")
    y = torch.empty_like(x)
    _lib.check(lib.shdr_clip_fwd_f32(_ptr(x), _ptr(y), x.numel(), float(lo), float(hi), _stream()),
               "shdr_clip_fwd_f32")
    return set_bound(y, max(abs(float(lo)), abs(float(hi))))


def logc(x):
    if _needs_grad(x):
        return AUTOGRAD.logc(x)
    lib = _lib.load()
    x = _chk(_d(x), "x")
    y = torch.empty_like(x)
    _lib.check(lib.shdr_logc_fwd_f32(_ptr(x), _ptr(y), x.numel(), _stream()), "shdr_logc_fwd_f32")
    return y


def _pix3(x, name):
    x = _chk(_d(x), name)
    if x.shape[-1] != 3:
        raise ValueError("%s: expected 3 channels, got %d" % (name, x.shape[-1]))
    return x, x.numel() // 3


def vgg_preprocess(x, out_channels=3, dtype=torch.float32):
    if _needs_grad(x):
        return AUTOGRAD.vgg_preprocess(x, out_channels, dtype)
    lib = _lib.load()
    x_in = x
    x, npix = _pix3(x, "x")
    if dtype == HALF:
        y = torch.empty(tuple(x.shape[:-1]) + (out_channels,), device=x.device, dtype=HALF)
        _lib.check(lib.shdr_pack3_f16(_ptr(x), None, None, None, 1, _ptr(y), out_channels, npix, 1, _stream()), "shdr_pack3_f16")
        return y
    y = torch.empty(tuple(x.shape[:-1]) + (out_channels,), device=x.device, dtype=torch.float32)
    _lib.check(lib.shdr_vgg_preprocess_fwd_f32(_ptr(x), _ptr(y), npix, out_channels, _stream()),
               "shdr_vgg_preprocess_fwd_f32")
    b = _bound_of(x_in)
    return y if b is None else set_bound(y, 255.0 * b + 124.0)


def reverse3(x):
    if _needs_grad(x):
        return AUTOGRAD.reverse3(x)
    lib = _lib.load()
    x, npix = _pix3(x, "x")
    y = torch.empty_like(x)
    _lib.check(lib.shdr_reverse3_fwd_f32(_ptr(x), _ptr(y), npix, _stream()), "shdr_reverse3_fwd_f32")
    return y


def alpha_blend(b_pred, hal_bgr, thr=0.12, return_alpha=False):
    if _needs_grad(b_pred, hal_bgr):
        if return_alpha:
            raise NotImplementedError("alpha_blend: return_alpha is not available on the taped path")
        return AUTOGRAD.alpha_blend(b_pred, hal_bgr, thr)
    lib = _lib.load()
    b_pred, npix = _pix3(b_pred, "b_pred")
    hal_bgr, npix2 = _pix3(hal_bgr, "hal_bgr")
    if npix != npix2:
        raise ValueError("alpha_blend: shape mismatch")
    a = torch.empty_like(b_pred)
    alpha = torch.empty(tuple(b_pred.shape[:-1]) + (1,), device=a.device, dtype=torch.float32) if return_alpha else None
    _lib.check(lib.shdr_alpha_blend_fwd_f32(_ptr(b_pred), _ptr(hal_bgr), _ptr(a), _ptr(alpha), npix,
                                            float(thr), _stream()), "shdr_alpha_blend_fwd_f32")
    return (a, alpha) if return_alpha else a


def pack3(srcs, out_channels=None, dtype=torch.float32):
    if _needs_grad(*srcs):
        return AUTOGRAD.pack3(list(srcs), out_channels, dtype)
    lib = _lib.load()
    srcs_in = list(srcs)
    srcs = [_pix3(s, "src%d" % i)[0] for i, s in enumerate(srcs)]
    n = len(srcs)
    if not 1 <= n <= 4:
        raise ValueError("pack3: 1..4 sources")
    if any(s.shape != srcs[0].shape for s in srcs):
        raise ValueError("pack3: shape mismatch")
    oc = out_channels or 3 * n
    y = torch.empty(tuple(srcs[0].shape[:-1]) + (oc,), device=srcs[0].device, dtype=dtype)
    p = [_ptr(s) for s in srcs] + [None] * (4 - n)
    if dtype == HALF:
        _lib.check(lib.shdr_pack3_f16(p[0], p[1], p[2], p[3], n, _ptr(y), oc, srcs[0].numel() // 3, 0, _stream()), "shdr_pack3_f16")
        return y
    _lib.check(lib.shdr_pack3_fwd_f32(p[0], p[1], p[2], p[3], n, _ptr(y), oc, srcs[0].numel() // 3,
                                      _stream()), "shdr_pack3_fwd_f32")
    if n == 1:
        return _carry_range(y, srcs_in[0])
    bounds = [_bound_of(t) for t in srcs_in]
    return y if None in bounds else set_bound(y, max(bounds))


def _conv_desc(x_shape, w_shape, stride, c2, x2_scale, cout_valid):
    n, h, wd, c1 = x_shape
    kh, kw, cin, cout_gemm = w_shape
    ho, pt = same_pad(h, kh, stride)
    wo, pl = same_pad(wd, kw, stride)
    d = _lib.ConvDesc()
    d.N, d.H, d.W, d.C1, d.C2 = n, h, wd, c1, c2
    d.Cout, d.KH, d.KW, d.stride = cout_gemm, kh, kw, stride
    d.cout_valid = cout_valid or cout_gemm
    d.pad_t, d.pad_l, d.Ho, d.Wo = pt, pl, ho, wo
    d.x2_scale = float(x2_scale)
    return d


def pad_channels(x, channels):
    lib = _lib.load()
    x = _chk(_d(x), "x")
    c = x.shape[-1]
    if c == channels:
        return x
    y = torch.empty(tuple(x.shape[:-1]) + (channels,), device=x.device, dtype=torch.float32)
    _lib.check(lib.shdr_pad_channels_f32(_ptr(x), _ptr(y), x.numel() // c, c, channels, _stream()), "shdr_pad_channels_f32")
    return y


def _up16(c):
    return (c + 15) // 16 * 16


WGRAD_X3_MIN_CH = 128

# ... 1722 lines not shown
```

singlehdr-tf2_amd/csrc/conv_x3.hip:

```cpp
#include <hip/hip_fp16.h>
#include <stdlib.h>

#include <type_traits>

#include "shdr_internal.h"

namespace {

using f32x4 = __attribute__((ext_vector_type(4))) float;
using f16x8 = __attribute__((ext_vector_type(8))) _Float16;
using f16x4 = __attribute__((ext_vector_type(4))) _Float16;
using u32x4 = __attribute__((ext_vector_type(4))) unsigned;

constexpr int X3_HEADER_FLOATS = 16;
constexpr int BN = 64, NT = 4, MT = 4;
constexpr int IMG_HALVES = BN * 32;
constexpr int UNIT_HALVES = 2 * IMG_HALVES;
constexpr int LRW = 10, LRPIX = LRW * LRW;
constexpr int LRJ = (LRPIX * 8 + 255) / 256;
template <int KH, int KW>
struct X3G {
  static constexpr int PH = 16 + KH - 1, PWID = 16 + KW - 1, PPIX = PH * PWID;
  static constexpr int PJ = (PPIX * 8 + 255) / 256;
  static constexpr int PATCH_HALVES = PPIX * 32;
  static constexpr int LDS_BYTES = (2 * PATCH_HALVES + 2 * UNIT_HALVES) * 2;
  static constexpr int LDS_BYTES_UP = LDS_BYTES + LRPIX * 32 * 4;
  static constexpr int RANGE_BYTES = 16;
};

struct X3Args {
  const float* x1;
  const float* x2;
  const _Float16* wp;
  const float* hdr;
  const float* bias;
  const float* scale;
  const float* shift;
  float* y;
  float* yp;
  const float* res;
  int res_cs;
  int N, H, W, C1, C2, Cout, tiles_x, tiles_y, nblk_m, nblk_n, act1, act2;
  int Hl, Wl;
  int Hin, Win;
  int in_s, bh, bw;
  int pool_avg;
  const unsigned* xr1;
  const unsigned* xr2;
  unsigned* yr;
  int nphase;
  int pth[4], ptw[4], pbh[4], pbw[4];
  const _Float16* pwp[4];
  const float* proj;
  float* yproj;
};

__device__ __forceinline__ void x3_range_scale(const unsigned* r1, const unsigned* r2, float& xs, float& ixs) {
  xs = 1.0f;
  ixs = 1.0f;
  unsigned b = r1 ? *r1 : 0u;
  if (r2) {
    const unsigned b2 = *r2;
    b = b2 > b ? b2 : b;
  }
  if (b != 0u && b < 0x7f800000u) {
    int ex;
    frexpf(__uint_as_float(b), &ex);
    int T = 11 - ex;
    T = T < -126 ? -126 : (T > 126 ? 126 : T);
    xs = ldexpf(1.0f, T);
    ixs = ldexpf(1.0f, -T);
  }
}
__device__ __forceinline__ void x3_split4(const f32x4 v, float xs, unsigned (&h)[2], unsigned (&l)[2]) {
  const float k2048 = 2048.0f;
#pragma unroll
  for (int p = 0; p < 2; ++p) {
    float t0, t1;
    asm("v_fma_mixlo_f16 %0, %1, %2, 0" : "=v"(h[p]) : "v"(v[2 * p]), "s"(xs));
    asm("v_fma_mixhi_f16 %0, %1, %2, 0" : "+v"(h[p]) : "v"(v[2 * p + 1]), "s"(xs));
    asm("v_fma_mix_f32 %0, %1, %2, -%3 op_sel_hi:[0,0,1]" : "=v"(t0) : "v"(v[2 * p]), "s"(xs), "v"(h[p]));
    asm("v_fma_mix_f32 %0, %1, %2, -%3 op_sel:[0,0,1] op_sel_hi:[0,0,1]" : "=v"(t1) : "v"(v[2 * p + 1]), "s"(xs), "v"(h[p]));
    asm("v_fma_mixlo_f16 %0, %1, %2, 0" : "=v"(l[p]) : "v"(t0), "s"(k2048));
    asm("v_fma_mixhi_f16 %0, %1, %2, 0" : "+v"(l[p]) : "v"(t1), "s"(k2048));
  }
}
template <int NW = 4>
__device__ __forceinline__ void x3_range_out(unsigned* slot, float m, int lane, int wave, unsigned seen, unsigned* lds) {
#pragma unroll
  for (int off = 32; off > 0; off >>= 1) m = fmaxf(m, __shfl_xor(m, off, 64));
  if (lane == 0) lds[wave] = __float_as_uint(m);
  asm volatile("s_waitcnt lgkmcnt(0)\n\ts_barrier" ::: "memory");
  if (threadIdx.x == 0) {
    const unsigned b01 = lds[0] > lds[1] ? lds[0] : lds[1], b23 = lds[2] > lds[3] ? lds[2] : lds[3];
    unsigned b = b01 > b23 ? b01 : b23;
    if (NW == 8) {
      const unsigned b45 = lds[4] > lds[5] ? lds[4] : lds[5], b67 = lds[6] > lds[7] ? lds[6] : lds[7];
      const unsigned b47 = b45 > b67 ? b45 : b67;
      b = b47 > b ? b47 : b;
    }
#ifndef SHDR_ABL_NO_RANGE_ATOMIC
    if (b > seen) atomicMax(slot, b);
#endif
  }
}

template <int NW, bool PROJ>
__device__ __forceinline__ void x3_tile_epilogue(const X3Args& a, f32x4 (&acc)[MT][NT], int img, int oh_row0, int ow, int pc, int fg, int n0, float ixs,
                                                 int lane, int wave, unsigned* range_lds) {
  const float inv_s = a.hdr[1] * ixs;
  const unsigned yr_seen = a.yr ? __hip_atomic_load(a.yr, __ATOMIC_RELAXED, __HIP_MEMORY_SCOPE_AGENT) : 0u;
  int ep0 = n0;
  asm volatile("" : "+s"(ep0));
  f32x4 bias_r[NT], scale_r[NT], shift_r[NT];
#pragma unroll
  for (int ni = 0; ni < NT; ++ni) {
    const int cl = ni * 16 + 4 * fg;
    const bool cv = ep0 + cl < a.Cout;
    bias_r[ni] = (a.bias && cv) ? *reinterpret_cast<const f32x4*>(a.bias + ep0 + cl) : (f32x4){0.f, 0.f, 0.f, 0.f};
    scale_r[ni] = (a.scale && cv) ? *reinterpret_cast<const f32x4*>(a.scale + ep0 + cl) : (f32x4){1.f, 1.f, 1.f, 1.f};
    shift_r[ni] = (a.scale && cv) ? *reinterpret_cast<const f32x4*>(a.shift + ep0 + cl) : (f32x4){0.f, 0.f, 0.f, 0.f};
  }
  f32x4 res_r[MT / 2][NT][2];
  if (a.res) {
#pragma unroll
    for (int mp = 0; mp < MT / 2; ++mp)
#pragma unroll
      for (int ni = 0; ni < NT; ++ni)
#pragma unroll
        for (int r = 0; r < 2; ++r) {
          const int oh = oh_row0 + 2 * mp + r;
          res_r[mp][ni][r] = (oh < a.H && ow < a.W && ep0 + ni * 16 + 4 * fg < a.Cout)
                                 ? *reinterpret_cast<const f32x4*>(a.res + ((size_t)(img * a.H + oh) * a.W + ow) * a.res_cs + ep0 + ni * 16 + 4 * fg)
                                 : (f32x4){0.f, 0.f, 0.f, 0.f};
        }
  }
  float ym = 0.0f;
#pragma unroll
  for (int mp = 0; mp < MT / 2; ++mp) {
    const int oh = oh_row0 + 2 * mp;
    if (oh >= a.H) continue;
    float pj[2][3] = {{0.f, 0.f, 0.f}, {0.f, 0.f, 0.f}};
#pragma unroll
    for (int ni = 0; ni < NT; ++ni) {
      const int cl = ni * 16 + 4 * fg;
      f32x4 v[2];
#pragma unroll
      for (int r = 0; r < 2; ++r) {
        v[r] = acc[2 * mp + r][ni] * inv_s;
        asm("" : "+v"(v[r]));
        v[r] += bias_r[ni];
        shdr::act_apply4<0>(v[r], a.act1);
        if (a.scale) v[r] = v[r] * scale_r[ni] + shift_r[ni];
        if (a.res) v[r] += res_r[mp][ni][r];
        shdr::act_apply4<0>(v[r], a.act2);
        if (a.y && oh + r < a.H && ow < a.W && n0 + cl < a.Cout)
          *reinterpret_cast<f32x4*>(a.y + ((size_t)(img * a.H + oh + r) * a.W + ow) * a.Cout + n0 + cl) = v[r];
        if (PROJ && a.proj) {
#pragma unroll
          for (int j = 0; j < 3; ++j) {
            const f32x4 q = *reinterpret_cast<const f32x4*>(a.proj + j * 64 + cl);
            pj[r][j] += v[r][0] * q[0] + v[r][1] * q[1] + v[r][2] * q[2] + v[r][3] * q[3];
          }
        }
#ifndef SHDR_ABL_NO_YM
        if (a.yr && oh + r < a.H) ym = fmaxf(fmaxf(fmaxf(fmaxf(ym, fabsf(v[r][0])), fabsf(v[r][1])), fabsf(v[r][2])), fabsf(v[r][3]));
#endif
      }
      if (a.yp) {
        f32x4 m;
#pragma unroll
        for (int e = 0; e < 4; ++e) {
          if (a.pool_avg) {
            const float t = v[0][e] + __shfl_xor(v[0][e], 1, 64), b = v[1][e] + __shfl_xor(v[1][e], 1, 64);
            m[e] = 0.25f * (t + b);
          } else {
            m[e] = fmaxf(v[0][e], v[1][e]);
            m[e] = fmaxf(m[e], __shfl_xor(m[e], 1, 64));
          }
        }
        if (!(pc & 1) && ow < a.W && n0 + cl < a.Cout)
          *reinterpret_cast<f32x4*>(a.yp + ((size_t)(img * (a.H >> 1) + (oh >> 1)) * (a.W >> 1) + (ow >> 1)) * a.Cout + n0 + cl) = m;
      }
    }
    if (PROJ && a.proj) {
#pragma unroll
      for (int r = 0; r < 2; ++r) {
#pragma unroll
        for (int j = 0; j < 3; ++j) {
          float t = pj[r][j];
          t += __shfl_xor(t, 16, 64);
          t += __shfl_xor(t, 32, 64);
          pj[r][j] = t;
        }
        if (fg == 0 && oh + r < a.H && ow < a.W) {
          float* o = a.yproj + ((size_t)(img * a.H + oh + r) * a.W + ow) * 3;
          o[0] = pj[r][0]; o[1] = pj[r][1]; o[2] = pj[r][2];
        }
      }
    }
  }
#ifndef SHDR_ABL_NO_TAIL
  if (a.yr)
    x3_range_out<NW>(a.yr, ow < a.W ? ym : 0.0f, lane, wave, yr_seen, range_lds);
#endif
}

__device__ __forceinline__ int xcd_remap(int bid, int nwg) {
  const int q = nwg >> 3, r = nwg & 7, xcd = bid & 7, idx = bid >> 3;
  return (xcd < r ? xcd * (q + 1) : r * (q + 1) + (xcd - r) * q) + idx;
}
__host__ __device__ inline int f4(int row) { return (-(row >> 2)) & 3; }
__host__ __device__ inline int sx(int col) { return ((col >> 2) & 1) * 2; }
__device__ __forceinline__ int pcol(int fi) { return fi < 4 ? fi : (fi >= 12 ? fi - 8 : fi + 4); }

template <bool UP, int KH, int KW, bool MP = false, int LOOK = 1>
__global__ __launch_bounds__(256, 2) void conv_x3_kernel(const X3Args a) {
  using G = X3G<KH, KW>;
  constexpr int PWID = G::PWID, PPIX = G::PPIX, PJ = G::PJ, PATCH_HALVES = G::PATCH_HALVES, NTAPS = KH * KW;
  static_assert(!UP || (KH == 3 && KW == 3), "the up-sampling prologue belongs to the 3 x 3 stride-1 form");
  static_assert(!MP || (!UP && KH == 4 && KW == 4), "the phase loop is built on the 4 x 4 patch geometry");
  static_assert(LOOK >= 1 && LOOK <= 2 && LOOK <= KW, "filter look-ahead: 1 or 2 taps");
  extern __shared__ __attribute__((aligned(16))) _Float16 xsm[];
#define patch_h (xsm)
#define patch_l (xsm + PATCH_HALVES)
#define filt (xsm + 2 * PATCH_HALVES)
#define lrs (reinterpret_cast<float*>(xsm + 2 * PATCH_HALVES + 2 * UNIT_HALVES))

  const int tid = threadIdx.x, lane = tid & 63;
  const int wave = __builtin_amdgcn_readfirstlane(tid >> 6);
  const int L = xcd_remap(blockIdx.x, a.nblk_m * a.nblk_n);
  const int pn = L % a.nblk_n;
  int pm = L / a.nblk_n;
  const int tx = pm % a.tiles_x;
  pm /= a.tiles_x;
  const int ty = pm % a.tiles_y;
  const int img = pm / a.tiles_y;
  const int n0 = pn * BN, oh0 = ty * 16, ow0 = tx * 16;

  int ppix[PJ];
  int pdst[PJ];
  int pcnt = 0;
  auto patch_geometry = [&](int bh, int bw) __attribute__((always_inline)) {
    pcnt = 0;
#pragma unroll
    for (int j = 0; j < (UP ? 0 : PJ); ++j) {
      const int p = tid + 256 * j;
      const int pix = p >> 3, q = p & 7;
      const int py = pix / PWID, px = pix - py * PWID;
      const int ih = a.in_s * (oh0 + py) + bh, iw = a.in_s * (ow0 + px) + bw;
      const bool ok = pix < PPIX && (unsigned)ih < (unsigned)a.Hin && (unsigned)iw < (unsigned)a.Win;
      ppix[j] = ok ? (img * a.Hin + ih) * a.Win + iw : -1;
      pdst[j] = pix < PPIX ? pix * 32 + 8 * ((q >> 1) ^ sx(px)) + 4 * (q & 1) : -1;
      pcnt += __ballot(ppix[j] >= 0) != 0ull;
    }
  };
  if (!MP) patch_geometry(a.bh, a.bw);
  if (!MP && !UP) pcnt = __builtin_amdgcn_readfirstlane(pcnt);
  int lpix[LRJ];
  if (UP) {
#pragma unroll
    for (int j = 0; j < LRJ; ++j) {
      const int p = tid + 256 * j;
      const int pix = p >> 3;
      const int ly = pix / LRW, lx = pix - ly * LRW;
      const int r = (oh0 >> 1) - 1 + ly, c = (ow0 >> 1) - 1 + lx;
      lpix[j] = (pix < LRPIX && (unsigned)r < (unsigned)a.Hl && (unsigned)c < (unsigned)a.Wl) ? (img * a.Hl + r) * a.Wl + c : -1;
      pcnt += __ballot(lpix[j] >= 0) != 0ull;
    }
    pcnt = __builtin_amdgcn_readfirstlane(pcnt);
  }
  const int nch1 = a.C1 >> 5, nch = (a.C1 + a.C2) >> 5;
  int nunits = nch * NTAPS;
  constexpr int DEPTH = (NTAPS == 1 && !UP && !MP) ? 2 : 1;
  using Set0 = std::integral_constant<int, 0>;
  using Set1 = std::integral_constant<int, DEPTH - 1>;
  f32x4 pr_sets[DEPTH][PJ];
#define pr (pr_sets[0])
  auto zero_patch = [&](auto setc) __attribute__((always_inline)) {
    constexpr int S = decltype(setc)::value;
#pragma unroll
    for (int j = 0; j < (UP ? LRJ : PJ); ++j) pr_sets[S][j] = (f32x4){0.f, 0.f, 0.f, 0.f};
#pragma unroll
    for (int j = 0; j < (UP ? LRJ : PJ); ++j) asm volatile("" : "+v"(pr_sets[S][j]));
  };
  auto load_lr = [&](int c, bool zeroed) __attribute__((always_inline)) {
#pragma unroll
    for (int j = 0; j < LRJ; ++j) {
      const int q = (tid + 256 * j) & 7;
      if (!zeroed) pr[j] = (f32x4){0.f, 0.f, 0.f, 0.f};
      if (lpix[j] >= 0) pr[j] = *reinterpret_cast<const f32x4*>(a.x1 + (size_t)(unsigned)lpix[j] * (unsigned)a.C1 + (c << 5) + 4 * q);
    }
  };
  auto park_lr = [&]() __attribute__((always_inline)) {
#pragma unroll
    for (int j = 0; j < LRJ; ++j)
      if (tid + 256 * j < LRPIX * 8) *reinterpret_cast<f32x4*>(lrs + 4 * (tid + 256 * j)) = pr[j];
  };
  float xs = 1.0f, ixs = 1.0f;
  auto split_store = [&](int dst, const f32x4 v4) __attribute__((always_inline)) {
    unsigned h[2], l[2];
    x3_split4(v4, xs, h, l);
    *reinterpret_cast<uint2*>(patch_h + dst) = make_uint2(h[0], h[1]);
    *reinterpret_cast<uint2*>(patch_l + dst) = make_uint2(l[0], l[1]);
  };
  auto expand_store = [&]() __attribute__((always_inline)) {
    const int r0 = (oh0 >> 1) - 1, c0 = (ow0 >> 1) - 1;
    int t0 = tid;
    asm volatile("" : "+v"(t0));
#pragma unroll
    for (int j = 0; j < PJ; ++j) {
      const int p = t0 + 256 * j;
      const int pix = p >> 3, q = p & 7;
      if (pix >= PPIX) continue;
      const int py = pix / PWID, px = pix - py * PWID;
      const int ih = oh0 - 1 + py, iw = ow0 - 1 + px;
      f32x4 v = (f32x4){0.f, 0.f, 0.f, 0.f};
      if ((unsigned)ih < (unsigned)a.Hin && (unsigned)iw < (unsigned)a.Win) {
        const int mr = ih >> 1, mc = iw >> 1;
        const int ra = (ih & 1) ? mr : max(mr - 1, 0), rb = (ih & 1) ? min(mr + 1, a.Hl - 1) : mr;
        const int ca = (iw & 1) ? mc : max(mc - 1, 0), cb = (iw & 1) ? min(mc + 1, a.Wl - 1) : mc;
        const float* s00 = lrs + ((ra - r0) * LRW + (ca - c0)) * 32 + 4 * q;
        const int dx = (cb - ca) * 32, dy = (rb - ra) * LRW * 32;
        const float wx = (iw & 1) ? 0.25f : 0.75f, wy = (ih & 1) ? 0.25f : 0.75f;
        const f32x4 q00 = *reinterpret_cast<const f32x4*>(s00), q01 = *reinterpret_cast<const f32x4*>(s00 + dx);
        const f32x4 q10 = *reinterpret_cast<const f32x4*>(s00 + dy), q11 = *reinterpret_cast<const f32x4*>(s00 + dy + dx);
#pragma unroll
        for (int e = 0; e < 4; ++e) {
          const float t = q00[e] + (q01[e] - q00[e]) * wx;
          const float u = q10[e] + (q11[e] - q10[e]) * wx;
          v[e] = t + (u - t) * wy;
        }
      }
      split_store(pix * 32 + 8 * ((q >> 1) ^ sx(px)) + 4 * (q & 1), v);
      if (j & 1) __builtin_amdgcn_sched_barrier(0);
    }
  };
  auto load_patch = [&](int c, auto setc, bool zeroed = false) __attribute__((always_inline)) {
    constexpr int S = decltype(setc)::value;
    if (UP) { load_lr(c, zeroed); return; }
    const bool second = c >= nch1;
    const float* src = second ? a.x2 : a.x1;
    const int Cs = second ? a.C2 : a.C1;
    const int c0 = (second ? c - nch1 : c) << 5;
#pragma unroll
    for (int j = 0; j < PJ; ++j) {
      const int q = (tid + 256 * j) & 7;
      if (!zeroed) pr_sets[S][j] = (f32x4){0.f, 0.f, 0.f, 0.f};
      if (ppix[j] >= 0) pr_sets[S][j] = *reinterpret_cast<const f32x4*>(src + (size_t)(unsigned)ppix[j] * (unsigned)Cs + c0 + 4 * q);
    }
  };
  auto store_patch = [&](auto setc) __attribute__((always_inline)) {
    constexpr int S = decltype(setc)::value;
    if (UP) { expand_store(); return; }
#pragma unroll
    for (int j = 0; j < PJ; ++j)
      if (pdst[j] >= 0) split_store(pdst[j], pr_sets[S][j]);
  };
  constexpr int FJ = 2;
  const _Float16* wbase = a.wp + (size_t)pn * nunits * UNIT_HALVES;
  int fdst[FJ];
#pragma unroll
  for (int j = 0; j < FJ; ++j) {
    const int p = tid + 256 * j;
    const int im = p >> 8, co = (p & 255) >> 2, slot = p & 3;
    fdst[j] = im * IMG_HALVES + co * 32 + 8 * (slot ^ f4(co));
  }
  constexpr int NFR = LOOK < 2 ? 1 : 2;
  static_assert(LOOK < 2 || (!MP && KH == 3 && KW == 3), "LOOK = 2 is built for the nine-tap kernels");
  u32x4 fr[NFR][FJ];
#pragma unroll
  for (int s = 0; s < NFR; ++s)
#pragma unroll
    for (int j = 0; j < FJ; ++j) fr[s][j] = (u32x4){0u, 0u, 0u, 0u};
  const unsigned foff = 16u * (unsigned)tid + 2048u;
  auto issue_filt = [&](int u, int s) __attribute__((always_inline)) {
    const _Float16* ub = wbase + (size_t)(u < nunits ? u : nunits - 1) * UNIT_HALVES;
    asm volatile("global_load_dwordx4 %0, %1, %2 offset:-2048" : "+v"(fr[s][0]) : "v"(foff), "s"(ub) : "memory");
    asm volatile("global_load_dwordx4 %0, %1, %2 offset:2048" : "+v"(fr[s][1]) : "v"(foff), "s"(ub) : "memory");
  };
  constexpr int PJL = UP ? LRJ : PJ;
  constexpr int WB = (LOOK - 1) * FJ;
#define X3_WAIT_VM(N) asm volatile("s_waitcnt vmcnt(%0)" : : "n"(N) : "memory")
  auto wait_store_filt = [&](int v, int s, int np, bool st) __attribute__((always_inline)) {
    if (np < 0) X3_WAIT_VM(0);
    else if (np >= PJL) X3_WAIT_VM(WB + PJL);
    else if (np >= PJL - 1) X3_WAIT_VM(WB + PJL - 1);
    else if (np >= PJL - 2) X3_WAIT_VM(WB + PJL - 2);
    else X3_WAIT_VM(WB);
    asm volatile("" : "+v"(fr[s][0]), "+v"(fr[s][1]) : : "memory");
    if (st) {
#pragma unroll
      for (int j = 0; j < FJ; ++j) *reinterpret_cast<u32x4*>(filt + (v & 1) * UNIT_HALVES + fdst[j]) = fr[s][j];
    }
  };

  f32x4 acc[MT][NT];
#pragma unroll
  for (int mi = 0; mi < MT; ++mi)
#pragma unroll
    for (int ni = 0; ni < NT; ++ni) acc[mi][ni] = (f32x4){0.f, 0.f, 0.f, 0.f};

  const int fi = lane & 15, fg = lane >> 4;
  int acol[KW], b_rd[NT];
  const int pc = pcol(fi);
#pragma unroll
  for (int kw = 0; kw < KW; ++kw) acol[kw] = (pc + kw) * 32 + 8 * (fg ^ sx(pc + kw));
#pragma unroll
  for (int ni = 0; ni < NT; ++ni) {
    const int row = ni * 16 + fi;
    b_rd[ni] = row * 32 + 8 * (fg ^ f4(row));
  }

  int kh_n = KH, kw_n = KW;
#pragma unroll 1
  for (int phase = 0; phase < (MP ? a.nphase : 1); ++phase) {
  if (MP) {
    kh_n = a.pth[phase];
    kw_n = a.ptw[phase];
    nunits = nch * kh_n * kw_n;
    wbase = a.pwp[phase] + (size_t)pn * nunits * UNIT_HALVES;
    patch_geometry(a.pbh[phase], a.pbw[phase]);
    pcnt = __builtin_amdgcn_readfirstlane(pcnt);
    if (phase > 0) __syncthreads();
  }
  load_patch(0, Set0{});
  if (DEPTH == 2 && nch > 1) load_patch(1, Set1{});
  issue_filt(0, 0);
  if (!MP || phase == 0) x3_range_scale(a.xr1, a.xr2, xs, ixs);
  if (UP) {
    park_lr();
    __syncthreads();
  }
  store_patch(Set0{});
  wait_store_filt(0, 0, -1, true);
  if (LOOK == 2) issue_filt(1, 1);
  auto chunk = [&](int c, auto cur, auto nxt) __attribute__((always_inline)) {
    const bool pf = c + DEPTH < nch;
    zero_patch(cur);
    __builtin_amdgcn_sched_barrier(0);
    issue_filt((MP ? c * kh_n * kw_n : c * NTAPS) + LOOK, LOOK % NFR);
    __builtin_amdgcn_sched_barrier(0);
    if (pf) load_patch(c + DEPTH, cur, true);
    __builtin_amdgcn_sched_barrier(0);
    const int np = pf ? pcnt : 0;
#define X3_SLOT(D) (NFR == 1 ? 0 : (kh * KW + kw + (D)) % NFR)
#define X3_TAP(FIRST)                                                                                                          \
  {                                                                                                                             \
    if (MP && kw >= kw_n) continue;                                                                                            \
    const int u = MP ? (c * kh_n + kh) * kw_n + kw : c * NTAPS + kh * KW + kw;                                                 \
    __syncthreads();                                                                                                           \
    if (!(FIRST) || kw > 0) issue_filt(u + LOOK, X3_SLOT(LOOK));                                                               \
    const _Float16* F = filt + (u & 1) * UNIT_HALVES;                                                                          \
    const int rowh = (wave * MT + kh) * PWID * 32;                                                                             \
                                                                                                                               \
    f16x8 wh[NT], ws[NT], wl[NT], ph[2], pl[2];                                                                                \
    auto read_a = [&](int mi, int slot) __attribute__((always_inline)) {                                                       \
      const int o = rowh + mi * PWID * 32 + acol[kw];                                                                          \
      ph[slot] = *reinterpret_cast<const f16x8*>(patch_h + o);                                                                 \
      pl[slot] = *reinterpret_cast<const f16x8*>(patch_l + o);                                                                 \
    };                                                                                                                         \
_Pragma("unroll")                                                                                                              \
    for (int ni = 0; ni < NT; ++ni) {                                                                                          \
      wh[ni] = *reinterpret_cast<const f16x8*>(F + b_rd[ni]);                                                                  \
      wl[ni] = *reinterpret_cast<const f16x8*>(F + IMG_HALVES + b_rd[ni]);                                                     \
    }                                                                                                                          \
    read_a(0, 0);                                                                                                              \
_Pragma("unroll")                                                                                                              \
    for (int ni = 0; ni < NT; ++ni) ws[ni] = wh[ni] * (_Float16)(1.0f / 2048.0f);                                              \
_Pragma("unroll")                                                                                                              \
    for (int mi = 0; mi < MT; ++mi) {                                                                                          \
      if (mi + 1 < MT) read_a(mi + 1, (mi + 1) & 1);                                                                           \
      __builtin_amdgcn_sched_barrier(0);                                                                                       \
_Pragma("unroll")                                                                                                              \
      for (int ni = 0; ni < NT; ++ni) acc[mi][ni] = __builtin_amdgcn_mfma_f32_16x16x32_f16(wh[ni], ph[mi & 1], acc[mi][ni], 0, 0, 0); \
_Pragma("unroll")                                                                                                              \
      for (int ni = 0; ni < NT; ++ni) acc[mi][ni] = __builtin_amdgcn_mfma_f32_16x16x32_f16(ws[ni], pl[mi & 1], acc[mi][ni], 0, 0, 0); \
_Pragma("unroll")                                                                                                              \
      for (int ni = 0; ni < NT; ++ni) acc[mi][ni] = __builtin_amdgcn_mfma_f32_16x16x32_f16(wl[ni], ph[mi & 1], acc[mi][ni], 0, 0, 0); \
      __builtin_amdgcn_sched_barrier(0);                                                                                       \
    }                                                                                                                          \
    wait_store_filt(u + 1, X3_SLOT(1), ((FIRST) && kw < LOOK) ? np : 0, u + 1 < nunits);                                       \
  }
    if (LOOK == 1) {
      {
        const int kh = 0;
#pragma unroll
        for (int kw = 0; kw < KW; ++kw) X3_TAP(true)
      }
#pragma unroll 1
      for (int kh = 1; kh < (MP ? kh_n : KH); ++kh) {
#pragma unroll
        for (int kw = 0; kw < KW; ++kw) X3_TAP(false)
      }
    } else {
#pragma unroll
      for (int kh = 0; kh < KH; ++kh) {
#pragma unroll
        for (int kw = 0; kw < KW; ++kw) X3_TAP(kh == 0)
      }
      asm volatile("s_waitcnt vmcnt(0)" : "+v"(fr[0][0]), "+v"(fr[0][1]) : : "memory");
#pragma unroll
      for (int j = 0; j < FJ; ++j) fr[NFR - 1][j] = fr[0][j];
    }
#undef X3_TAP
#undef X3_SLOT
    if (c + 1 < nch) {
      if (UP) {
        park_lr();
        __syncthreads();
      } else {
        __syncthreads();
      }
      store_patch(nxt);
    }
  };
#pragma unroll 1
  for (int c = 0; c < nch; c += DEPTH) {
    chunk(c, Set0{}, Set1{});
    if (DEPTH == 2 && c + 1 < nch) chunk(c + 1, Set1{}, Set0{});
  }
  }
#undef pr
#undef X3_WAIT_VM

  x3_tile_epilogue<4, true>(a, acc, img, oh0 + wave * MT, ow0 + pc, pc, fg, n0, ixs, lane, wave,
                            reinterpret_cast<unsigned*>(reinterpret_cast<char*>(xsm) + (UP ? G::LDS_BYTES_UP : G::LDS_BYTES)));
}

#undef patch_h
#undef patch_l
#undef filt
#undef lrs

constexpr int X1_BP = 128;
template <int NS>
__global__ __launch_bounds__(256, 2) void conv_x3_1x1_kernel(const X3Args a) {
  constexpr int MT1 = 2 * NS, BP = X1_BP;
  constexpr int PJ1 = BP * 8 / 256;
  constexpr int IMG = BP * 32;
  static_assert(NS * (BP / (MT1 * 16)) == 4, "four waves: NS cout slices x pixel groups");
  __shared__ __attribute__((aligned(16))) _Float16 x1sm[2 * 2 * IMG];
  __shared__ unsigned x1rw[4];

  const int tid = threadIdx.x, lane = tid & 63;
  const int wave = __builtin_amdgcn_readfirstlane(tid >> 6);
  const int slice = wave % NS, grp = wave / NS;
  const int L = xcd_remap(blockIdx.x, a.nblk_m * a.nblk_n);
  const int pn = L % a.nblk_n, pm = L / a.nblk_n;
  const int P0 = pm * BP, Ptot = a.N * a.H * a.W;

  int ppix[PJ1];
  const int pdst = (tid >> 3) * 32 + 8 * (((tid & 7) >> 1) ^ sx((tid >> 3) & 15)) + 4 * (tid & 1);
#pragma unroll
  for (int j = 0; j < PJ1; ++j) {
    const int P = P0 + (tid >> 3) + 32 * j;
    ppix[j] = -1;
    if (P < Ptot) {
      const int ow = P % a.W, t = P / a.W;
      const int oh = t % a.H, img = t / a.H;
      const int ih = a.in_s * oh + a.bh, iw = a.in_s * ow + a.bw;
      if ((unsigned)ih < (unsigned)a.Hin && (unsigned)iw < (unsigned)a.Win) ppix[j] = (img * a.Hin + ih) * a.Win + iw;
    }
  }
  const int nch1 = a.C1 >> 5, nch = (a.C1 + a.C2) >> 5;
  using Set0 = std::integral_constant<int, 0>;
  using Set1 = std::integral_constant<int, 1>;
  f32x4 pr_sets[2][PJ1];
  auto load_patch = [&](int c, auto setc) __attribute__((always_inline)) {
    constexpr int S = decltype(setc)::value;
    const bool second = c >= nch1;
    const float* src = second ? a.x2 : a.x1;
    const int Cs = second ? a.C2 : a.C1;
    const int c0 = (second ? c - nch1 : c) << 5;
#pragma unroll
    for (int j = 0; j < PJ1; ++j) {
      pr_sets[S][j] = (f32x4){0.f, 0.f, 0.f, 0.f};
      if (ppix[j] >= 0) pr_sets[S][j] = *reinterpret_cast<const f32x4*>(src + (size_t)(unsigned)ppix[j] * (unsigned)Cs + c0 + 4 * (tid & 7));
    }
  };
  float xs = 1.0f, ixs = 1.0f;
  auto store_patch = [&](int buf, auto setc) __attribute__((always_inline)) {
    constexpr int S = decltype(setc)::value;
#pragma unroll
    for (int j = 0; j < PJ1; ++j) {
      unsigned h[2], l[2];
      x3_split4(pr_sets[S][j], xs, h, l);
      *reinterpret_cast<uint2*>(x1sm + buf * 2 * IMG + pdst + 1024 * j) = make_uint2(h[0], h[1]);
      *reinterpret_cast<uint2*>(x1sm + buf * 2 * IMG + IMG + pdst + 1024 * j) = make_uint2(l[0], l[1]);
    }
  };
  const int fi = lane & 15, fg = lane >> 4;
  const _Float16* wsl = a.wp + (size_t)(pn * NS + slice) * nch * UNIT_HALVES + fi * 32 + 8 * fg;
  f16x8 f0h[2], f0l[2], f1h[2], f1l[2];
  auto load_w = [&](int c, int half, f16x8 (&h)[2], f16x8 (&l)[2]) __attribute__((always_inline)) {
    const _Float16* g = wsl + (size_t)c * UNIT_HALVES + half * 2 * 16 * 32;
#pragma unroll
    for (int k = 0; k < 2; ++k) {
      h[k] = *reinterpret_cast<const f16x8*>(g + k * 16 * 32);
      l[k] = *reinterpret_cast<const f16x8*>(g + IMG_HALVES + k * 16 * 32);
    }
  };

  f32x4 acc[MT1][NT];
#pragma unroll
  for (int mi = 0; mi < MT1; ++mi)
#pragma unroll
    for (int ni = 0; ni < NT; ++ni) acc[mi][ni] = (f32x4){0.f, 0.f, 0.f, 0.f};
  const int pc = pcol(fi);
  const int a_rd = (grp * MT1 * 16 + pc) * 32 + 8 * (fg ^ sx(pc));

  auto half_pass = [&](int buf, auto halfc, const f16x8 (&wh)[2], const f16x8 (&wl)[2]) __attribute__((always_inline)) {
    constexpr int H = decltype(halfc)::value;
    const int bo = buf * 2 * IMG + a_rd;
    f16x8 ws[2], ph[2], pl[2];
    auto read_a = [&](int mi, int slot) __attribute__((always_inline)) {
      ph[slot] = *reinterpret_cast<const f16x8*>(x1sm + bo + mi * 16 * 32);
      pl[slot] = *reinterpret_cast<const f16x8*>(x1sm + IMG + bo + mi * 16 * 32);
    };
    read_a(0, 0);
#pragma unroll
    for (int k = 0; k < 2; ++k) ws[k] = wh[k] * (_Float16)(1.0f / 2048.0f);
#pragma unroll
    for (int mi = 0; mi < MT1; ++mi) {
      if (mi + 1 < MT1) read_a(mi + 1, (mi + 1) & 1);
      __builtin_amdgcn_sched_barrier(0);
#pragma unroll
      for (int k = 0; k < 2; ++k) acc[mi][2 * H + k] = __builtin_amdgcn_mfma_f32_16x16x32_f16(wh[k], ph[mi & 1], acc[mi][2 * H + k], 0, 0, 0);
#pragma unroll
      for (int k = 0; k < 2; ++k) acc[mi][2 * H + k] = __builtin_amdgcn_mfma_f32_16x16x32_f16(ws[k], pl[mi & 1], acc[mi][2 * H + k], 0, 0, 0);
#pragma unroll
      for (int k = 0; k < 2; ++k) acc[mi][2 * H + k] = __builtin_amdgcn_mfma_f32_16x16x32_f16(wl[k], ph[mi & 1], acc[mi][2 * H + k], 0, 0, 0);
      __builtin_amdgcn_sched_barrier(0);
    }
  };
  using Half0 = std::integral_constant<int, 0>;
  using Half1 = std::integral_constant<int, 1>;

  load_patch(0, Set0{});
  if (nch > 1) load_patch(1, Set1{});
  load_w(0, 0, f0h, f0l);
  x3_range_scale(a.xr1, a.xr2, xs, ixs);
  store_patch(0, Set0{});
  if (nch > 2) load_patch(2, Set0{});
  auto chunk = [&](int c, auto nxt) __attribute__((always_inline)) {
    __syncthreads();
    load_w(c, 1, f1h, f1l);
    if (c + 1 < nch) {
      store_patch((c + 1) & 1, nxt);
      if (c + 3 < nch) load_patch(c + 3, nxt);
    }
    half_pass(c & 1, Half0{}, f0h, f0l);
    if (c + 1 < nch) load_w(c + 1, 0, f0h, f0l);
    half_pass(c & 1, Half1{}, f1h, f1l);
  };
#pragma unroll 1
  for (int c = 0; c < nch; c += 2) {
    chunk(c, Set1{});
    if (c + 1 < nch) chunk(c + 1, Set0{});
  }

  const float inv_s = a.hdr[1] * ixs;
  const unsigned yr_seen = a.yr ? __hip_atomic_load(a.yr, __ATOMIC_RELAXED, __HIP_MEMORY_SCOPE_AGENT) : 0u;
  int ep0 = (pn * NS + slice) * BN;
  asm volatile("" : "+s"(ep0));
  f32x4 bias_r[NT], scale_r[NT], shift_r[NT];
#pragma unroll
  for (int ni = 0; ni < NT; ++ni) {
    const int cl = ni * 16 + 4 * fg;
    bias_r[ni] = a.bias ? *reinterpret_cast<const f32x4*>(a.bias + ep0 + cl) : (f32x4){0.f, 0.f, 0.f, 0.f};
    scale_r[ni] = a.scale ? *reinterpret_cast<const f32x4*>(a.scale + ep0 + cl) : (f32x4){1.f, 1.f, 1.f, 1.f};
    shift_r[ni] = a.scale ? *reinterpret_cast<const f32x4*>(a.shift + ep0 + cl) : (f32x4){0.f, 0.f, 0.f, 0.f};
  }
  const int Pw = P0 + grp * MT1 * 16 + pc;
  float ym = 0.0f;
  constexpr int EB = 4;
#pragma unroll
  for (int m0 = 0; m0 < MT1; m0 += EB) {
    f32x4 res_r[EB][NT];
    if (a.res) {
#pragma unroll
      for (int e = 0; e < EB; ++e)
#pragma unroll
        for (int ni = 0; ni < NT; ++ni) {
          const int P = Pw + 16 * (m0 + e);
          res_r[e][ni] = P < Ptot ? *reinterpret_cast<const f32x4*>(a.res + (size_t)P * a.res_cs + ep0 + ni * 16 + 4 * fg) : (f32x4){0.f, 0.f, 0.f, 0.f};
        }
    }
#pragma unroll
    for (int e = 0; e < EB; ++e) {
      const int P = Pw + 16 * (m0 + e);
      if (P0 + grp * MT1 * 16 + 16 * (m0 + e) >= Ptot) continue;
#pragma unroll
      for (int ni = 0; ni < NT; ++ni) {
        f32x4 v = acc[m0 + e][ni] * inv_s;
        asm("" : "+v"(v));
        v += bias_r[ni];
        shdr::act_apply4<0>(v, a.act1);
        if (a.scale) v = v * scale_r[ni] + shift_r[ni];
        if (a.res) v += res_r[e][ni];
        shdr::act_apply4<0>(v, a.act2);
        if (P < Ptot) {
          *reinterpret_cast<f32x4*>(a.y + (size_t)P * a.Cout + ep0 + ni * 16 + 4 * fg) = v;
          if (a.yr) ym = fmaxf(fmaxf(fmaxf(fmaxf(ym, fabsf(v[0])), fabsf(v[1])), fabsf(v[2])), fabsf(v[3]));
        }
      }
    }
  }
  if (a.yr) x3_range_out(a.yr, ym, lane, wave, yr_seen, x1rw);
}

constexpr int XW_THREADS = 512, XW_BN = 128;
constexpr long XW_UP_MIN_COUT = 128;
struct XWG {
  using G = X3G<3, 3>;
  static constexpr int PJ = (G::PPIX * 8 + XW_THREADS - 1) / XW_THREADS;
  static constexpr int RANGE_BYTES = 32;
  static constexpr int LR_BYTES = LRPIX * 32 * 4;
  static constexpr int LDS_BYTES = (2 * 2 * G::PATCH_HALVES + 2 * 2 * UNIT_HALVES) * 2;
};
template <bool UP>
__global__ __launch_bounds__(XW_THREADS, 2) void conv_x3_wide_kernel(const X3Args a) {
  using G = X3G<3, 3>;
  constexpr int KH = 3, KW = 3, PWID = G::PWID, PPIX = G::PPIX, PJ = XWG::PJ, PATCH_HALVES = G::PATCH_HALVES, NTAPS = 9;
  static_assert((PJ - 1) * XW_THREADS < PPIX * 8 && PJ == 6, "every piece but the last is inside the patch for every thread");
  extern __shared__ __attribute__((aligned(16))) _Float16 xsm[];
#define patch_buf(B) (xsm + (B) * 2 * PATCH_HALVES)
#define filt (xsm + 4 * PATCH_HALVES)
#define lrs (reinterpret_cast<float*>(xsm + 4 * PATCH_HALVES + 4 * UNIT_HALVES))

  const int tid = threadIdx.x, lane = tid & 63;
  const int wave = __builtin_amdgcn_readfirstlane(tid >> 6);
  const int slice = wave >> 2, wq = wave & 3;
  const int L = xcd_remap(blockIdx.x, a.nblk_m * a.nblk_n);
  const int pn = L % a.nblk_n;
  int pm = L / a.nblk_n;
  const int tx = pm % a.tiles_x;
  pm /= a.tiles_x;
  const int ty = pm % a.tiles_y;
  const int img = pm / a.tiles_y;
  const int n0 = pn * XW_BN + slice * BN, oh0 = ty * 16, ow0 = tx * 16;

  constexpr int PL = UP ? (LRPIX * 8 + XW_THREADS - 1) / XW_THREADS : PJ;
  constexpr int T0 = UP ? 4 : 3;
  int ppix[PL], pdst[PJ];
  int pcnt = 0;
  if (UP) {
#pragma unroll
    for (int j = 0; j < PL; ++j) {
      const int p = tid + XW_THREADS * j;
      const int pix = p >> 3;
      const int ly = pix / LRW, lx = pix - ly * LRW;
      const int r = (oh0 >> 1) - 1 + ly, c = (ow0 >> 1) - 1 + lx;
      ppix[j] = (pix < LRPIX && (unsigned)r < (unsigned)a.Hl && (unsigned)c < (unsigned)a.Wl) ? (img * a.Hl + r) * a.Wl + c : -1;
      pcnt += __ballot(ppix[j] >= 0) != 0ull;
    }
  }
#pragma unroll
  for (int j = 0; j < (UP ? 0 : PJ); ++j) {
    const int p = tid + XW_THREADS * j;
    const int pix = p >> 3, q = p & 7;
    const int py = pix / PWID, px = pix - py * PWID;
    const int ih = oh0 + py + a.bh, iw = ow0 + px + a.bw;
    const bool ok = pix < PPIX && (unsigned)ih < (unsigned)a.Hin && (unsigned)iw < (unsigned)a.Win;
    ppix[j] = ok ? (img * a.Hin + ih) * a.Win + iw : -1;
    pdst[j] = pix < PPIX ? pix * 32 + 8 * ((q >> 1) ^ sx(px)) + 4 * (q & 1) : -1;
    pcnt += __ballot(ppix[j] >= 0) != 0ull;
  }
  pcnt = __builtin_amdgcn_readfirstlane(pcnt);
  const int nch1 = a.C1 >> 5, nch = (a.C1 + a.C2) >> 5;
  const int nunits = nch * NTAPS;
  f32x4 pr[PL];
  auto zero_patch = [&]() __attribute__((always_inline)) {
#pragma unroll
    for (int j = 0; j < PL; ++j) pr[j] = (f32x4){0.f, 0.f, 0.f, 0.f};
#pragma unroll
    for (int j = 0; j < PL; ++j) asm volatile("" : "+v"(pr[j]));
  };
  auto load_patch = [&](int c, bool zeroed) __attribute__((always_inline)) {
    if (UP) {
#pragma unroll
      for (int j = 0; j < PL; ++j) {
        const int q = (tid + XW_THREADS * j) & 7;
        if (!zeroed) pr[j] = (f32x4){0.f, 0.f, 0.f, 0.f};
        if (ppix[j] >= 0) pr[j] = *reinterpret_cast<const f32x4*>(a.x1 + (size_t)(unsigned)ppix[j] * (unsigned)a.C1 + (c << 5) + 4 * q);
      }
      return;
    }
    const bool second = c >= nch1;
    const float* src = second ? a.x2 : a.x1;
    const int Cs = second ? a.C2 : a.C1;
    const int c0 = (second ? c - nch1 : c) << 5;
#pragma unroll
    for (int j = 0; j < (UP ? 0 : PJ); ++j) {
      const int q = (tid + XW_THREADS * j) & 7;
      if (!zeroed) pr[j] = (f32x4){0.f, 0.f, 0.f, 0.f};
      if (ppix[j] >= 0) pr[j] = *reinterpret_cast<const f32x4*>(src + (size_t)(unsigned)ppix[j] * (unsigned)Cs + c0 + 4 * q);
    }
  };
  float xs = 1.0f, ixs = 1.0f;
  auto park_lr = [&]() __attribute__((always_inline)) {
#pragma unroll
    for (int j = 0; j < (UP ? PL : 0); ++j)
      if (tid + XW_THREADS * j < LRPIX * 8) *reinterpret_cast<f32x4*>(lrs + 4 * (tid + XW_THREADS * j)) = pr[j];
  };
  auto split_store = [&](int buf, int j) __attribute__((always_inline)) {
    f32x4 v = (f32x4){0.f, 0.f, 0.f, 0.f};
    int dst;
    if (UP) {
      const int r0 = (oh0 >> 1) - 1, c0 = (ow0 >> 1) - 1;
      int t0 = tid;
      asm volatile("" : "+v"(t0));
      const int p = t0 + XW_THREADS * j;
      const int pix = p >> 3, q = p & 7;
      if (pix >= PPIX) return;
      const int py = pix / PWID, px = pix - py * PWID;
      const int ih = oh0 - 1 + py, iw = ow0 - 1 + px;
      if ((unsigned)ih < (unsigned)a.Hin && (unsigned)iw < (unsigned)a.Win) {
        const int mr = ih >> 1, mc = iw >> 1;
        const int ra = (ih & 1) ? mr : max(mr - 1, 0), rb = (ih & 1) ? min(mr + 1, a.Hl - 1) : mr;
        const int ca = (iw & 1) ? mc : max(mc - 1, 0), cb2 = (iw & 1) ? min(mc + 1, a.Wl - 1) : mc;
        const float* s00 = lrs + ((ra - r0) * LRW + (ca - c0)) * 32 + 4 * q;
        const int dx = (cb2 - ca) * 32, dy = (rb - ra) * LRW * 32;
        const float wx = (iw & 1) ? 0.25f : 0.75f, wy = (ih & 1) ? 0.25f : 0.75f;
        const f32x4 q00 = *reinterpret_cast<const f32x4*>(s00), q01 = *reinterpret_cast<const f32x4*>(s00 + dx);
        const f32x4 q10 = *reinterpret_cast<const f32x4*>(s00 + dy), q11 = *reinterpret_cast<const f32x4*>(s00 + dy + dx);
#pragma unroll
        for (int e = 0; e < 4; ++e) {
          const float t = q00[e] + (q01[e] - q00[e]) * wx;
          const float u = q10[e] + (q11[e] - q10[e]) * wx;
          v[e] = t + (u - t) * wy;
        }
      }
      dst = pix * 32 + 8 * ((q >> 1) ^ sx(px)) + 4 * (q & 1);
    } else {
      if (j == PJ - 1 && pdst[j] < 0) return;
      v = pr[UP ? 0 : j];
      dst = pdst[j];
    }
    unsigned h[2], l[2];
    x3_split4(v, xs, h, l);
    *reinterpret_cast<uint2*>(patch_buf(buf) + dst) = make_uint2(h[0], h[1]);
    *reinterpret_cast<uint2*>(patch_buf(buf) + PATCH_HALVES + dst) = make_uint2(l[0], l[1]);
  };
  constexpr int FJ = 2;
  const int ht = tid & 255;
  const _Float16* wbase = a.wp + (size_t)(pn * 2 + slice) * nunits * UNIT_HALVES;
#define fsl (filt + slice * 2 * UNIT_HALVES)
  int fdst[FJ];
#pragma unroll
  for (int j = 0; j < FJ; ++j) {
    const int p = ht + 256 * j;
    const int im = p >> 8, co = (p & 255) >> 2, slot = p & 3;
    fdst[j] = im * IMG_HALVES + co * 32 + 8 * (slot ^ f4(co));
  }
  u32x4 fr[2][FJ];
#pragma unroll
  for (int s = 0; s < 2; ++s)
#pragma unroll
    for (int j = 0; j < FJ; ++j) fr[s][j] = (u32x4){0u, 0u, 0u, 0u};
  const unsigned foff = 16u * (unsigned)ht + 2048u;
  auto issue_filt = [&](int u, int s) __attribute__((always_inline)) {
    const _Float16* ub = wbase + (size_t)(u < nunits ? u : nunits - 1) * UNIT_HALVES;
    asm volatile("global_load_dwordx4 %0, %1, %2 offset:-2048" : "+v"(fr[s][0]) : "v"(foff), "s"(ub) : "memory");
    asm volatile("global_load_dwordx4 %0, %1, %2 offset:2048" : "+v"(fr[s][1]) : "v"(foff), "s"(ub) : "memory");
  };
  constexpr int WB = FJ;
#define XW_WAIT_VM(N) asm volatile("s_waitcnt vmcnt(%0)" : : "n"(N) : "memory")
  auto wait_store_filt = [&](int v, int s, int np, bool st) __attribute__((always_inline)) {
    static_assert(PL <= 6, "the rungs below cover up to six patch loads per thread");
    if (np < 0) XW_WAIT_VM(0);
    else if (np >= 6) XW_WAIT_VM(WB + 6);
    else if (np >= 5) XW_WAIT_VM(WB + 5);
    else if (np >= 4) XW_WAIT_VM(WB + 4);
    else if (np >= 3) XW_WAIT_VM(WB + 3);
    else if (np >= 2) XW_WAIT_VM(WB + 2);
    else if (np >= 1) XW_WAIT_VM(WB + 1);
    else XW_WAIT_VM(WB);
    asm volatile("" : "+v"(fr[s][0]), "+v"(fr[s][1]) : : "memory");
    if (st) {
#pragma unroll
      for (int j = 0; j < FJ; ++j) *reinterpret_cast<u32x4*>(fsl + (v & 1) * UNIT_HALVES + fdst[j]) = fr[s][j];
    }
  };

  f32x4 acc[MT][NT];
#pragma unroll
  for (int mi = 0; mi < MT; ++mi)
#pragma unroll
    for (int ni = 0; ni < NT; ++ni) acc[mi][ni] = (f32x4){0.f, 0.f, 0.f, 0.f};

  const int fi = lane & 15, fg = lane >> 4;
  int acol[KW], b_rd[NT];
  const int pc = pcol(fi);
#pragma unroll
  for (int kw = 0; kw < KW; ++kw) acol[kw] = (pc + kw) * 32 + 8 * (fg ^ sx(pc + kw));
#pragma unroll
  for (int ni = 0; ni < NT; ++ni) {
    const int row = ni * 16 + fi;
    b_rd[ni] = row * 32 + 8 * (fg ^ f4(row));
  }

  static_assert(NT == MT, "one filter fragment pair of the next tap is read in front of each MFMA group");
  load_patch(0, false);
  issue_filt(0, 0);
  issue_filt(1, 1);
  x3_range_scale(a.xr1, a.xr2, xs, ixs);
  if (UP) {
    park_lr();
    __syncthreads();
  }
#pragma unroll
  for (int j = 0; j < PJ; ++j) {
    split_store(0, j);
    if (UP && (j & 1)) __builtin_amdgcn_sched_barrier(0);
  }
  wait_store_filt(0, 0, -1, true);
  wait_store_filt(1, 1, -1, true);
  issue_filt(2, 0);
  __syncthreads();
  f16x8 wh[NT], wl[NT];
#pragma unroll
  for (int ni = 0; ni < NT; ++ni) {
    wh[ni] = *reinterpret_cast<const f16x8*>(fsl + b_rd[ni]);
    wl[ni] = *reinterpret_cast<const f16x8*>(fsl + IMG_HALVES + b_rd[ni]);
  }
#pragma unroll 1
  for (int c = 0; c < nch; ++c) {
    const bool pf = c + 1 < nch;
    const int cb = c & 1;
    zero_patch();
    __builtin_amdgcn_sched_barrier(0);
    issue_filt(c * NTAPS + 3, 1);
    __builtin_amdgcn_sched_barrier(0);
    if (pf) load_patch(c + 1, true);
    __builtin_amdgcn_sched_barrier(0);
    const int np = pf ? pcnt : 0;
#pragma unroll
    for (int kh = 0; kh < KH; ++kh) {
#pragma unroll
      for (int kw = 0; kw < KW; ++kw) {
        const int t = kh * KW + kw;
        const int u = c * NTAPS + t;
        __syncthreads();
        if (t == 3) {
#pragma unroll
          for (int j = 0; j < PL; ++j) asm volatile("" : "+v"(pr[j]));
          if (UP && pf) park_lr();
          __builtin_amdgcn_sched_barrier(0);
        }
        if (t > 0) issue_filt(u + 3, (t + 3) & 1);
        const _Float16* F = fsl + ((u + 1) & 1) * UNIT_HALVES;
        const int rowh = (wq * MT + kh) * PWID * 32;

        f16x8 ws[NT], nwh[NT], nwl[NT], ph[2], pl[2];
        auto read_a = [&](int mi, int slot) __attribute__((always_inline)) {
          const int o = rowh + mi * PWID * 32 + acol[kw];
          ph[slot] = *reinterpret_cast<const f16x8*>(patch_buf(cb) + o);
          pl[slot] = *reinterpret_cast<const f16x8*>(patch_buf(cb) + PATCH_HALVES + o);
        };
        read_a(0, 0);
#pragma unroll
        for (int ni = 0; ni < NT; ++ni) ws[ni] = wh[ni] * (_Float16)(1.0f / 2048.0f);
#pragma unroll
        for (int mi = 0; mi < MT; ++mi) {
          if (mi + 1 < MT) read_a(mi + 1, (mi + 1) & 1);
          nwh[mi] = *reinterpret_cast<const f16x8*>(F + b_rd[mi]);
          nwl[mi] = *reinterpret_cast<const f16x8*>(F + IMG_HALVES + b_rd[mi]);
          __builtin_amdgcn_sched_barrier(0);
#pragma unroll
          for (int ni = 0; ni < NT; ++ni) acc[mi][ni] = __builtin_amdgcn_mfma_f32_16x16x32_f16(wh[ni], ph[mi & 1], acc[mi][ni], 0, 0, 0);
#pragma unroll
          for (int ni = 0; ni < NT; ++ni) acc[mi][ni] = __builtin_amdgcn_mfma_f32_16x16x32_f16(ws[ni], pl[mi & 1], acc[mi][ni], 0, 0, 0);
#pragma unroll
          for (int ni = 0; ni < NT; ++ni) acc[mi][ni] = __builtin_amdgcn_mfma_f32_16x16x32_f16(wl[ni], ph[mi & 1], acc[mi][ni], 0, 0, 0);
          __builtin_amdgcn_sched_barrier(0);
          if (mi == 1 && t >= T0 && t - T0 < PJ - 2) {
            if (pf) split_store(cb ^ 1, t - T0);
            __builtin_amdgcn_sched_barrier(0);
          }
        }
        wait_store_filt(u + 2, t & 1, t < 2 ? np : 0, u + 2 < nunits);
#pragma unroll
        for (int ni = 0; ni < NT; ++ni) {
          wh[ni] = nwh[ni];
          wl[ni] = nwl[ni];
        }
      }
    }
    asm volatile("s_waitcnt vmcnt(0)" : "+v"(fr[1][0]), "+v"(fr[1][1]) : : "memory");
#pragma unroll
    for (int j = 0; j < FJ; ++j) fr[0][j] = fr[1][j];
    if (pf) {
      split_store(cb ^ 1, PJ - 2);
      split_store(cb ^ 1, PJ - 1);
    }
  }
#undef XW_WAIT_VM

  x3_tile_epilogue<8, false>(a, acc, img, oh0 + wq * MT, ow0 + pc, pc, fg, n0, ixs, lane, wave,
                             reinterpret_cast<unsigned*>(reinterpret_cast<char*>(xsm) + XWG::LDS_BYTES + (UP ? XWG::LR_BYTES : 0)));
}
#undef patch_buf
#undef filt
#undef fsl
#undef lrs

__global__ __launch_bounds__(256) void x3_absmax_kernel(const float* __restrict__ w, long n, unsigned* __restrict__ out) {
  float m = 0.f;
  for (long i = (long)blockIdx.x * 256 + threadIdx.x; i < n; i += (long)gridDim.x * 256) m = fmaxf(m, fabsf(w[i]));
#pragma unroll
  for (int off = 32; off > 0; off >>= 1) m = fmaxf(m, __shfl_xor(m, off, 64));
  if ((threadIdx.x & 63) == 0) atomicMax(out, __float_as_uint(m));
}
__global__ __launch_bounds__(256) void x3_absmax_big_kernel(const float* __restrict__ x, long n4, unsigned* __restrict__ out) {
  __shared__ float part[4];
  float m = 0.f;
  for (long i = (long)blockIdx.x * 256 + threadIdx.x; i < n4; i += (long)gridDim.x * 256) {
    const f32x4 v = reinterpret_cast<const f32x4*>(x)[i];
    m = fmaxf(fmaxf(m, fmaxf(fabsf(v[0]), fabsf(v[1]))), fmaxf(fabsf(v[2]), fabsf(v[3])));
  }
#pragma unroll
  for (int off = 32; off > 0; off >>= 1) m = fmaxf(m, __shfl_xor(m, off, 64));
  if ((threadIdx.x & 63) == 0) part[threadIdx.x >> 6] = m;
  __syncthreads();
  if (threadIdx.x == 0) atomicMax(out, __float_as_uint(fmaxf(fmaxf(part[0], part[1]), fmaxf(part[2], part[3]))));
}
__global__ __launch_bounds__(256) void x3_pack_kernel(const float* __restrict__ w, float* __restrict__ hdr, _Float16* __restrict__ out, int Ct,
                                                      int C1, int Cout, float x2_scale, int KWF, int TH, int TW, int p0, int q0, int step) {
  const float mx = fmaxf(__uint_as_float(reinterpret_cast<const unsigned*>(hdr)[0]) * fmaxf(1.0f, fabsf(x2_scale)), 1e-30f);
  int ex;
  frexpf(mx, &ex);
  int S = 14 - ex;
  S = S < -100 ? -100 : (S > 100 ? 100 : S);
  const float s = ldexpf(1.0f, S);
  if (blockIdx.x == 0 && threadIdx.x == 0) hdr[1] = ldexpf(1.0f, -S);
  const int ntaps = TH * TW;
  const int nunits = (Ct >> 5) * ntaps;
  const long total = (long)((Cout + 63) / 64) * nunits * 64 * 32;
  for (long e = (long)blockIdx.x * 256 + threadIdx.x; e < total; e += (long)gridDim.x * 256) {
    const int k = (int)(e & 31), co = (int)((e >> 5) & 63);
    const long t = e >> 11;
    const int u = (int)(t % nunits), nb = (int)(t / nunits);
    const int chunk = u / ntaps, t2 = u - ntaps * chunk;
    const int ta = t2 / TW, tb = t2 - TW * ta;
    const int tap = (p0 + step * ta) * KWF + (q0 + step * tb);
    const int ch = chunk * 32 + k;
    float v = nb * 64 + co < Cout ? w[((size_t)tap * Ct + ch) * Cout + nb * 64 + co] * s : 0.0f;
    if (ch >= C1) v *= x2_scale;
    const _Float16 h = (_Float16)v;
    _Float16* o = out + ((size_t)(nb * nunits + u) * 2) * IMG_HALVES + co * 32 + k;
    o[0] = h;
    o[IMG_HALVES] = (_Float16)(v - (float)h);
  }
}

}

namespace {

struct X3Phase { int th, tw, p0, q0, step, bh, bw; };
int x3_phases(const shdr_conv2d_desc* d, X3Phase ph[4]) {
  if (d->stride == 1 || d->KH == 1) {
    ph[0] = X3Phase{d->KH, d->KW, 0, 0, d->stride, -d->pad_t, -d->pad_l};
    return 1;
  }
  int n = 0;
  for (int p0 = 0; p0 < 2; ++p0)
    for (int q0 = 0; q0 < 2; ++q0) ph[n++] = X3Phase{(d->KH - p0 + 1) / 2, (d->KW - q0 + 1) / 2, p0, q0, 2, p0 - d->pad_t, q0 - d->pad_l};
  return n;
}
inline int64_t x3_phase_floats(const X3Phase& p, int Ct, int Cout) { return X3_HEADER_FLOATS + (int64_t)p.th * p.tw * Ct * ((Cout + 63) / 64 * 64); }

template <bool UP, int KH, int KW, bool MP, int LOOK>
int launch_x3_look(const X3Args& a, hipStream_t st) {
  constexpr int lds = (UP ? X3G<KH, KW>::LDS_BYTES_UP : X3G<KH, KW>::LDS_BYTES) + X3G<KH, KW>::RANGE_BYTES;
  static bool attr_done[shdr::kMaxDevices] = {};
  const int dev_slot = shdr::device_slot();
  if (!attr_done[dev_slot]) {
    hipError_t e = hipFuncSetAttribute(reinterpret_cast<const void*>(&conv_x3_kernel<UP, KH, KW, MP, LOOK>), hipFuncAttributeMaxDynamicSharedMemorySize, lds);
    if (e != hipSuccess) return shdr::fail(SHDR_E_ARCH, "hipFuncSetAttribute: %s", hipGetErrorString(e));
    attr_done[dev_slot] = true;
  }
  const long nblk = (long)a.nblk_m * a.nblk_n;
  if (nblk > 0x7fffffffL) return shdr::fail(SHDR_E_SHAPE, "conv2d_x3: grid of %ld blocks", nblk);
  hipLaunchKernelGGL((conv_x3_kernel<UP, KH, KW, MP, LOOK>), dim3((unsigned)nblk), dim3(256), lds, st, a);
  return shdr::check_launch("conv_x3_kernel");
}
template <bool UP, int KH, int KW, bool MP = false>
int launch_x3(const X3Args& a, hipStream_t st) {
  int look = 2;
  if (const char* e = SHDR_ENV("SHDR_X3_LOOK")) look = atoi(e);
  constexpr bool look2 = KH == 3 && KW == 3 && !MP;
  if (look >= 2 && look2) return launch_x3_look<UP, KH, KW, MP, look2 ? 2 : 1>(a, st);
  return launch_x3_look<UP, KH, KW, MP, 1>(a, st);
}

int launch_x3_1x1(const X3Args& a0, hipStream_t st) {
  X3Args a = a0;
  const long npix = (long)a.N * a.H * a.W;
  const int ns = a.Cout % 256 == 0 ? 4 : 2;
  a.nblk_m = (int)((npix + X1_BP - 1) / X1_BP);
  a.nblk_n = a.Cout / (64 * ns);
  const long nblk = (long)a.nblk_m * a.nblk_n;
  if (nblk > 0x7fffffffL) return shdr::fail(SHDR_E_SHAPE, "conv2d_x3: grid of %ld blocks", nblk);
  if (ns == 4) hipLaunchKernelGGL((conv_x3_1x1_kernel<4>), dim3((unsigned)nblk), dim3(256), 0, st, a);
  else hipLaunchKernelGGL((conv_x3_1x1_kernel<2>), dim3((unsigned)nblk), dim3(256), 0, st, a);
  return shdr::check_launch("conv_x3_1x1_kernel");
}

template <bool UP>
int launch_x3_wide(const X3Args& a0, hipStream_t st) {
  X3Args a = a0;
  a.nblk_n = a.Cout / XW_BN;
  constexpr int lds = XWG::LDS_BYTES + (UP ? XWG::LR_BYTES : 0) + XWG::RANGE_BYTES;
  static bool attr_done[shdr::kMaxDevices] = {};
  const int dev_slot = shdr::device_slot();
  if (!attr_done[dev_slot]) {
    hipError_t e = hipFuncSetAttribute(reinterpret_cast<const void*>(&conv_x3_wide_kernel<UP>), hipFuncAttributeMaxDynamicSharedMemorySize, lds);
    if (e != hipSuccess) return shdr::fail(SHDR_E_ARCH, "hipFuncSetAttribute: %s", hipGetErrorString(e));
    attr_done[dev_slot] = true;
  }
  const long nblk = (long)a.nblk_m * a.nblk_n;
  if (nblk > 0x7fffffffL) return shdr::fail(SHDR_E_SHAPE, "conv2d_x3: grid of %ld blocks", nblk);
  hipLaunchKernelGGL((conv_x3_wide_kernel<UP>), dim3((unsigned)nblk), dim3(XW_THREADS), lds, st, a);
  return shdr::check_launch("conv_x3_wide_kernel");
}

}

extern "C" int shdr_conv2d_x3_ok_f32(const shdr_conv2d_desc* d) {
  if (!d || d->C1 <= 0 || d->C1 % 32 || d->C2 % 32 || (d->Cout % 64 && (d->Cout != 32 || d->stride != 1 || SHDR_ENV("SHDR_NO_X3_COUT32")))) return 0;
  const int cv = d->cout_valid > 0 ? d->cout_valid : d->Cout;
  if (cv != d->Cout || d->w_batch_stride != 0 || d->y_pix_stride > 1) return 0;
  if ((long)d->N * d->H * d->W * (d->C1 > d->C2 ? d->C1 : d->C2) >= (1L << 31)) return 0;
  if (SHDR_ENV("SHDR_NO_X3")) return 0;
  if (d->act1 == SHDR_ACT_TANH || d->act2 == SHDR_ACT_TANH) return 0;
  if (d->stride == 1) {
    const bool k3 = d->KH == 3 && d->KW == 3 && d->pad_t == 1 && d->pad_l == 1;
    int k1_min = 64;
    if (const char* e = SHDR_ENV("SHDR_X3_1X1_MIN_K")) k1_min = atoi(e);
    const bool k1 = d->KH == 1 && d->KW == 1 && d->pad_t == 0 && d->pad_l == 0 && d->C1 + d->C2 >= k1_min && SHDR_ENV("SHDR_NO_X3_1X1") == nullptr;
    if (!(k3 || k1) || d->Ho != d->H || d->Wo != d->W) return 0;
  } else if (d->stride == 2 && d->KH == 1 && d->KW == 1) {
    if (d->pad_t != 0 || d->pad_l != 0 || d->C2 != 0 || d->prologue != SHDR_PROLOGUE_NONE || d->Ho != (d->H + 1) / 2 || d->Wo != (d->W + 1) / 2 ||
        d->C1 < 64 || SHDR_ENV("SHDR_NO_X3_1X1") || SHDR_ENV("SHDR_NO_X3_STRIDE2"))
      return 0;
  } else {
    int ho = 0, wo = 0, pt = 0, pl = 0;
    shdr_same_pad(d->H, 7, 2, &ho, &pt);
    shdr_same_pad(d->W, 7, 2, &wo, &pl);
    if (d->stride != 2 || d->KH != 7 || d->KW != 7 || d->C2 != 0 || d->prologue != SHDR_PROLOGUE_NONE || d->Ho != ho || d->Wo != wo || d->pad_t != pt ||
        d->pad_l != pl || SHDR_ENV("SHDR_NO_X3_STRIDE2"))
      return 0;
  }
  const long blocks = (long)d->N * ((d->Ho + 15) / 16) * ((d->Wo + 15) / 16) * ((d->Cout + 63) / 64);
  long min_blocks = 192;
  if (const char* e = SHDR_ENV("SHDR_X3_MIN_BLOCKS")) min_blocks = atol(e);
  return blocks >= min_blocks ? 1 : 0;
}

extern "C" int64_t shdr_conv2d_x3_filter_elems_f32(const shdr_conv2d_desc* d) {
  if (!d || d->C1 <= 0 || (d->C1 + d->C2) % 32 || (d->Cout % 64 && d->Cout != 32) || (d->stride != 1 && d->stride != 2)) return -1;
  X3Phase ph[4];
  const int n = x3_phases(d, ph);
  int64_t total = 0;
  for (int i = 0; i < n; ++i) total += x3_phase_floats(ph[i], d->C1 + d->C2, d->Cout);
  return total;
}

extern "C" int shdr_conv2d_x3_prepare_filter_premax_f32(const shdr_conv2d_desc* d, const float* w, float* prepared, int premax, void* stream);
extern "C" int shdr_conv2d_x3_prepare_filter_f32(const shdr_conv2d_desc* d, const float* w, float* prepared, void* stream) {
  return shdr_conv2d_x3_prepare_filter_premax_f32(d, w, prepared, 0, stream);
}
extern "C" int shdr_conv2d_x3_prepare_filter_premax_f32(const shdr_conv2d_desc* d, const float* w, float* prepared, int premax, void* stream) {
  SHDR_REQUIRE(d && w && prepared, SHDR_E_NULL, "conv2d_x3_prepare_filter: null pointer");
  const int Ct = d->C1 + d->C2;
  SHDR_REQUIRE(Ct > 0 && Ct % 32 == 0 && d->C1 % 32 == 0 && d->Cout > 0 && (d->Cout % 64 == 0 || d->Cout == 32), SHDR_E_SHAPE,
               "conv2d_x3_prepare_filter: need C %% 32 == 0, Cout %% 64 == 0 (or Cout 32)");
  SHDR_REQUIRE(shdr::aligned16(prepared), SHDR_E_ALIGN, "conv2d_x3_prepare_filter: prepared must be 16-byte aligned");
  hipStream_t st = reinterpret_cast<hipStream_t>(stream);
  const float x2s = d->C2 > 0 ? d->x2_scale : 1.0f;
  X3Phase ph[4];
  const int n = x3_phases(d, ph);
  const long nw = (long)d->KH * d->KW * Ct * d->Cout;
  float* out = prepared;
  SHDR_REQUIRE(!premax || n == 1, SHDR_E_SHAPE, "conv2d_x3_prepare_filter: premax is for single-phase (stride-1) layers");
  for (int i = 0; i < n; ++i) {
    if (!premax) {
      if (hipMemsetAsync(out, 0, X3_HEADER_FLOATS * sizeof(float), st) != hipSuccess) return shdr::fail(SHDR_E_LAUNCH, "conv2d_x3_prepare_filter: memset");
      const int gmax = shdr::stream_grid(nw) < 64 ? shdr::stream_grid(nw) : 64;
      hipLaunchKernelGGL(x3_absmax_kernel, dim3(gmax), dim3(256), 0, st, w, nw, reinterpret_cast<unsigned*>(out));
    }
    const long np = (long)ph[i].th * ph[i].tw * Ct * ((d->Cout + 63) / 64 * 64);
    hipLaunchKernelGGL(x3_pack_kernel, dim3(shdr::stream_grid(np)), dim3(256), 0, st, w, out, reinterpret_cast<_Float16*>(out + X3_HEADER_FLOATS), Ct,
                       d->C1, d->Cout, x2s, d->KW, ph[i].th, ph[i].tw, ph[i].p0, ph[i].q0, ph[i].step);
    out += x3_phase_floats(ph[i], Ct, d->Cout);
  }
  return shdr::check_launch("conv2d_x3_prepare_filter");
}

extern "C" int shdr_absmax_f32(const float* x, int64_t n, float* range, void* stream) {
  SHDR_REQUIRE(x && range, SHDR_E_NULL, "absmax: null pointer");
  SHDR_REQUIRE(n > 0, SHDR_E_SHAPE, "absmax: n must be positive");
  hipStream_t st = reinterpret_cast<hipStream_t>(stream);
  unsigned* slot = reinterpret_cast<unsigned*>(range);
  const int64_t n4 = shdr::aligned16(x) ? n / 4 : 0;
  if (n4 > 0) {
    int grid = shdr::stream_grid(n4);
    if (grid > 1024) grid = 1024;
    hipLaunchKernelGGL(x3_absmax_big_kernel, dim3(grid), dim3(256), 0, st, x, (long)n4, slot);
  }
  if (n - 4 * n4 > 0) hipLaunchKernelGGL(x3_absmax_kernel, dim3(n4 > 0 ? 1 : (shdr::stream_grid(n) < 64 ? shdr::stream_grid(n) : 64)), dim3(256), 0, st, x + 4 * n4, (long)(n - 4 * n4), slot);
  return shdr::check_launch("absmax");
}

extern "C" int shdr_conv2d_x3_input_absmax_f32(const float* x, int64_t n, float* prepared, void* stream) {
  SHDR_REQUIRE(x && prepared, SHDR_E_NULL, "conv2d_x3_input_absmax: null pointer");
  SHDR_REQUIRE(n > 0 && n % 4 == 0 && shdr::aligned16(x), SHDR_E_SHAPE, "conv2d_x3_input_absmax: n must be a positive multiple of 4, x 16-byte aligned");
  return shdr_absmax_f32(x, n, prepared + 2, stream);
}

static int x3_forward(const shdr_conv2d_desc* d, const float* x1, const float* x2, const float* prepared, const float* bias,
                      const float* scale, const float* shift, const float* residual, float* y, float* y_pool, const float* proj, float* y_proj,
                      const float* x1_range, const float* x2_range, float* y_range, void* stream) {
  SHDR_REQUIRE(d && x1 && prepared && (y || y_pool || y_proj), SHDR_E_NULL, "conv2d_x3: null desc/x1/filter or no output");
  SHDR_REQUIRE((proj == nullptr) == (y_proj == nullptr), SHDR_E_NULL, "conv2d_x3: proj and y_proj come together");
  SHDR_REQUIRE(!proj || (d->Cout == 64 && d->stride == 1 && shdr::aligned16(proj)), SHDR_E_SHAPE,
               "conv2d_x3: the projected output takes a stride-1 layer with 64 output channels (one cout slice per block) and a 16-byte aligned map");
  SHDR_REQUIRE(!y_pool || (d->Ho % 2 == 0 && d->Wo % 2 == 0 && shdr::aligned16(y_pool)), SHDR_E_SHAPE, "conv2d_x3: the fused 2x2 max-pool needs even Ho, Wo");
  const bool up = d->prologue == SHDR_PROLOGUE_BILINEAR2X, rs = d->prologue == SHDR_PROLOGUE_RANGE_SCALE;
  SHDR_REQUIRE(d->prologue == SHDR_PROLOGUE_NONE || rs || (up && d->stride == 1 && d->C2 == 0 && d->H % 2 == 0 && d->W % 2 == 0), SHDR_E_SHAPE,
               "conv2d_x3: the bilinear 2x prologue takes a stride-1 layer, one source and even (up-sampled) H, W");
  SHDR_REQUIRE(shdr_conv2d_x3_ok_f32(d), SHDR_E_SHAPE, "conv2d_x3: layer shape not taken by this kernel");
  SHDR_REQUIRE((d->C2 == 0) == (x2 == nullptr), SHDR_E_NULL, "conv2d_x3: x2 must be given iff C2 > 0");
  SHDR_REQUIRE((scale == nullptr) == (shift == nullptr), SHDR_E_NULL, "conv2d_x3: scale and shift come together");
  SHDR_REQUIRE(shdr::aligned16(x1) && (!x2 || shdr::aligned16(x2)) && shdr::aligned16(prepared) && (!y || shdr::aligned16(y)) &&
                   (!bias || shdr::aligned16(bias)) && (!scale || (shdr::aligned16(scale) && shdr::aligned16(shift))),
               SHDR_E_ALIGN, "conv2d_x3: tensors must be 16-byte aligned");
  SHDR_REQUIRE(!x2 || ((x1_range == nullptr) == (x2_range == nullptr)), SHDR_E_NULL, "conv2d_x3: give the range of both sources or of neither");
  X3Args a{};
  a.x1 = x1; a.x2 = x2 ? x2 : x1;
  a.bias = bias; a.scale = scale; a.shift = shift; a.y = y; a.yp = y_pool;
  a.pool_avg = d->pool == SHDR_POOL_AVG;
  a.N = d->N; a.H = d->Ho; a.W = d->Wo; a.C1 = d->C1; a.C2 = d->C2; a.Cout = d->Cout;
  a.Hin = d->H; a.Win = d->W;
  a.Hl = d->H / 2; a.Wl = d->W / 2;
  a.tiles_x = (a.W + 15) / 16;
  a.tiles_y = (a.H + 15) / 16;
  a.nblk_m = a.N * a.tiles_x * a.tiles_y;
  a.nblk_n = (a.Cout + 63) / 64;
  a.act1 = d->act1; a.act2 = d->act2;
  a.xr1 = reinterpret_cast<const unsigned*>(x1_range);
  a.xr2 = reinterpret_cast<const unsigned*>(x2 ? x2_range : nullptr);
  a.yr = reinterpret_cast<unsigned*>(y_range);
  a.proj = proj; a.yproj = y_proj;
  SHDR_REQUIRE(!residual || (d->stride == 1 && d->res_cstride >= d->Cout && d->res_cstride % 4 == 0 && shdr::aligned16(residual) && !y_pool && !proj), SHDR_E_SHAPE,
               "conv2d_x3: the residual takes a stride-1 layer, res_cstride >= Cout (a multiple of 4), a 16-byte aligned tensor, no pooled / projected output");
  a.res = residual; a.res_cs = d->res_cstride;
  hipStream_t st = reinterpret_cast<hipStream_t>(stream);
  X3Phase ph[4];
  const int n = x3_phases(d, ph);
  const int Ct = d->C1 + d->C2;
  a.hdr = prepared;
  a.wp = reinterpret_cast<const _Float16*>(prepared + X3_HEADER_FLOATS);
  if (rs && !x1_range) a.xr1 = reinterpret_cast<const unsigned*>(prepared) + 2;
  a.in_s = ph[0].step; a.bh = ph[0].bh; a.bw = ph[0].bw;
  if (n == 4) {
    const float* pk = prepared;
    a.nphase = 4;
    for (int i = 0; i < 4; ++i) {
      SHDR_REQUIRE(ph[i].th <= 4 && ph[i].tw <= 4 && ph[i].step == ph[0].step, SHDR_E_SHAPE, "conv2d_x3: unexpected phase geometry");
      a.pth[i] = ph[i].th; a.ptw[i] = ph[i].tw; a.pbh[i] = ph[i].bh; a.pbw[i] = ph[i].bw;
      a.pwp[i] = reinterpret_cast<const _Float16*>(pk + X3_HEADER_FLOATS);
      pk += x3_phase_floats(ph[i], Ct, d->Cout);
    }
    return launch_x3<false, 4, 4, true>(a, st);
  }
  if (ph[0].th == 3 && ph[0].tw == 3) {
    long wide_min_blocks = 256, wide_min_cout = up ? XW_UP_MIN_COUT : 512;
    if (const char* e = SHDR_ENV("SHDR_X3_WIDE_MIN_BLOCKS")) wide_min_blocks = atol(e);
    if (const char* e = SHDR_ENV("SHDR_X3_WIDE_MIN_COUT")) wide_min_cout = atol(e);
    const bool wide = d->stride == 1 && d->Cout % XW_BN == 0 && d->Cout >= wide_min_cout && !proj &&
                      (long)a.nblk_m * (d->Cout / XW_BN) >= wide_min_blocks && SHDR_ENV("SHDR_X3_SLICED") == nullptr;
    return wide ? (up ? launch_x3_wide<true>(a, st) : launch_x3_wide<false>(a, st)) : up ? launch_x3<true, 3, 3>(a, st) : launch_x3<false, 3, 3>(a, st);
  }
  if (ph[0].th == 1 && ph[0].tw == 1) {
    const bool wide = d->Cout % 128 == 0 && y && !y_pool && !proj && !up && SHDR_ENV("SHDR_X3_1X1_SLICED") == nullptr;
    return wide ? launch_x3_1x1(a, st) : launch_x3<false, 1, 1>(a, st);
  }
  return shdr::fail(SHDR_E_SHAPE, "conv2d_x3: no kernel for a %d x %d layer", ph[0].th, ph[0].tw);
}

extern "C" int shdr_conv2d_fwd_x3_ranged_f32(const shdr_conv2d_desc* d, const float* x1, const float* x2, const float* prepared, const float* bias,
                                             const float* scale, const float* shift, float* y, float* y_pool, const float* x1_range,
                                             const float* x2_range, float* y_range, void* stream) {
  SHDR_REQUIRE(y || y_pool, SHDR_E_NULL, "conv2d_x3: neither y nor y_pool");
  return x3_forward(d, x1, x2, prepared, bias, scale, shift, nullptr, y, y_pool, nullptr, nullptr, x1_range, x2_range, y_range, stream);
}

extern "C" int shdr_conv2d_fwd_x3_residual_f32(const shdr_conv2d_desc* d, const float* x1, const float* x2, const float* prepared, const float* bias,
                                               const float* scale, const float* shift, const float* residual, float* y, const float* x1_range,
                                               const float* x2_range, float* y_range, void* stream) {
  SHDR_REQUIRE(y, SHDR_E_NULL, "conv2d_x3: null y");
  return x3_forward(d, x1, x2, prepared, bias, scale, shift, residual, y, nullptr, nullptr, nullptr, x1_range, x2_range, y_range, stream);
}

extern "C" int shdr_conv2d_fwd_x3_projected_f32(const shdr_conv2d_desc* d, const float* x1, const float* x2, const float* prepared,
                                                const float* bias, const float* scale, const float* shift, const float* proj, float* y_proj,
                                                float* y, float* y_pool, const float* x1_range, const float* x2_range, float* y_range,
                                                void* stream) {
  SHDR_REQUIRE(proj && y_proj, SHDR_E_NULL, "conv2d_x3_projected: null proj / y_proj");
  return x3_forward(d, x1, x2, prepared, bias, scale, shift, nullptr, y, y_pool, proj, y_proj, x1_range, x2_range, y_range, stream);
}

extern "C" int shdr_conv2d_fwd_x3_f32(const shdr_conv2d_desc* d, const float* x1, const float* x2, const float* prepared, const float* bias,
                                      const float* scale, const float* shift, float* y, float* y_pool, void* stream) {
  return shdr_conv2d_fwd_x3_ranged_f32(d, x1, x2, prepared, bias, scale, shift, y, y_pool, nullptr, nullptr, nullptr, stream);
}
```

Before: 955.1.

## Chain several output tiles per block in the 3x3 x3 conv kernel

Adds a chained variant of the 3x3 conv_x3 kernel in which each block walks T consecutive output tiles, column-major. The next tile's patch geometry and first filter unit are prefetched during the last chunk of the current tile, so pipeline fill and drain are paid once per chain instead of once per tile. It targets layers with few input-channel chunks (1 or 3) and enough tiles, and it accumulates the range max across the chain. The cost is more complex filter-buffer parity handling and fewer blocks in the grid, which could hurt occupancy or load balance.

```diff
diff --git a/include/shdr.h b/include/shdr.h
--- a/include/shdr.h
+++ b/include/shdr.h
@@ -240,6 +240,7 @@
 
 int shdr_conv2d_x3_ok_f32(const shdr_conv2d_desc* d);
 int64_t shdr_conv2d_x3_filter_elems_f32(const shdr_conv2d_desc* d);
+int shdr_conv2d_x3_chain_f32(const shdr_conv2d_desc* d, int projected);
 int shdr_conv2d_x3_prepare_filter_f32(const shdr_conv2d_desc* d, const float* w, float* prepared, void* stream);
 int shdr_conv2d_x3_input_absmax_f32(const float* x, int64_t n, float* prepared, void* stream);
 int shdr_conv2d_fwd_x3_f32(const shdr_conv2d_desc* d, const float* x1, const float* x2, const float* prepared, const float* bias,
diff --git a/singlehdr-tf2_amd/_lib.py b/singlehdr-tf2_amd/_lib.py
--- a/singlehdr-tf2_amd/_lib.py
+++ b/singlehdr-tf2_amd/_lib.py
@@ -82,6 +82,7 @@
     "shdr_conv2d_winograd_fused_up2_f32": (c_int, [c_ptr] * 6 + [c_int] * 7 + [c_ptr]),
     "shdr_conv2d_x3_ok_f32": (c_int, [ctypes.POINTER(ConvDesc)]),
     "shdr_conv2d_x3_filter_elems_f32": (c_i64, [ctypes.POINTER(ConvDesc)]),
+    "shdr_conv2d_x3_chain_f32": (c_int, [ctypes.POINTER(ConvDesc), c_int]),
     "shdr_conv2d_x3_prepare_filter_f32": (c_int, [ctypes.POINTER(ConvDesc), c_ptr, c_ptr, c_ptr]),
     "shdr_conv2d_fwd_x3_f32": (c_int, [ctypes.POINTER(ConvDesc)] + [c_ptr] * 9),
     "shdr_conv2d_fwd_x3_ranged_f32": (c_int, [ctypes.POINTER(ConvDesc)] + [c_ptr] * 12),
diff --git a/singlehdr-tf2_amd/_ops.py b/singlehdr-tf2_amd/_ops.py
--- a/singlehdr-tf2_amd/_ops.py
+++ b/singlehdr-tf2_amd/_ops.py
@@ -514,6 +514,21 @@
     return _PLAN_NAMES[int(lib.shdr_conv2d_plan_f32(ctypes.byref(d), int(has_residual)))]
 
 
+def x3_chain(x_shape, w_shape, c2=0, projected=False):
+    lib = _lib.load()
+    n, h, wd, c1 = x_shape
+    kh, kw, cin, cout = w_shape
+    d = _lib.ConvDesc()
+    d.N, d.H, d.W, d.C1, d.C2 = n, h, wd, c1, c2
+    d.Cout, d.KH, d.KW, d.stride = cout, kh, kw, 1
+    d.cout_valid = cout
+    d.Ho, d.pad_t = same_pad(h, kh, 1)
+    d.Wo, d.pad_l = same_pad(wd, kw, 1)
+    d.x2_scale = 1.0
+    d.algo = _auto(ALGO_AUTO)
+    return int(lib.shdr_conv2d_x3_chain_f32(ctypes.byref(d), int(bool(projected))))
+
+
 def winograd_path(cin, cout):
     p = conv2d_plan((1, 64, 64, cin), (3, 3, cin, cout))
     return p if p in ("fused", "planes") else None
diff --git a/singlehdr-tf2_amd/csrc/conv_x3.hip b/singlehdr-tf2_amd/csrc/conv_x3.hip
--- a/singlehdr-tf2_amd/csrc/conv_x3.hip
+++ b/singlehdr-tf2_amd/csrc/conv_x3.hip
@@ -53,6 +53,7 @@
   const _Float16* pwp[4];
   const float* proj;
   float* yproj;
+  int chain, nchain;
 };
 
 __device__ __forceinline__ void x3_range_scale(const unsigned* r1, const unsigned* r2, float& xs, float& ixs) {
@@ -105,11 +106,11 @@
   }
 }
 
-template <int NW, bool PROJ>
+template <int NW, bool PROJ, bool RES_PAIRS = false>
 __device__ __forceinline__ void x3_tile_epilogue(const X3Args& a, f32x4 (&acc)[MT][NT], int img, int oh_row0, int ow, int pc, int fg, int n0, float ixs,
-                                                 int lane, int wave, unsigned* range_lds) {
+                                                 int lane, int wave, unsigned* range_lds, float& ym_chain, bool range_out) {
   const float inv_s = a.hdr[1] * ixs;
-  const unsigned yr_seen = a.yr ? __hip_atomic_load(a.yr, __ATOMIC_RELAXED, __HIP_MEMORY_SCOPE_AGENT) : 0u;
+  const unsigned yr_seen = (a.yr && range_out) ? __hip_atomic_load(a.yr, __ATOMIC_RELAXED, __HIP_MEMORY_SCOPE_AGENT) : 0u;
   int ep0 = n0;
   asm volatile("" : "+s"(ep0));
   f32x4 bias_r[NT], scale_r[NT], shift_r[NT];
@@ -121,25 +122,28 @@
     scale_r[ni] = (a.scale && cv) ? *reinterpret_cast<const f32x4*>(a.scale + ep0 + cl) : (f32x4){1.f, 1.f, 1.f, 1.f};
     shift_r[ni] = (a.scale && cv) ? *reinterpret_cast<const f32x4*>(a.shift + ep0 + cl) : (f32x4){0.f, 0.f, 0.f, 0.f};
   }
-  f32x4 res_r[MT / 2][NT][2];
-  if (a.res) {
-#pragma unroll
-    for (int mp = 0; mp < MT / 2; ++mp)
-#pragma unroll
-      for (int ni = 0; ni < NT; ++ni)
-#pragma unroll
-        for (int r = 0; r < 2; ++r) {
-          const int oh = oh_row0 + 2 * mp + r;
-          res_r[mp][ni][r] = (oh < a.H && ow < a.W && ep0 + ni * 16 + 4 * fg < a.Cout)
-                                 ? *reinterpret_cast<const f32x4*>(a.res + ((size_t)(img * a.H + oh) * a.W + ow) * a.res_cs + ep0 + ni * 16 + 4 * fg)
-                                 : (f32x4){0.f, 0.f, 0.f, 0.f};
-        }
+  f32x4 res_r[RES_PAIRS ? 1 : MT / 2][NT][2];
+  auto load_res = [&](int mp) __attribute__((always_inline)) {
+#pragma unroll
+    for (int ni = 0; ni < NT; ++ni)
+#pragma unroll
+      for (int r = 0; r < 2; ++r) {
+        const int oh = oh_row0 + 2 * mp + r;
+        res_r[RES_PAIRS ? 0 : mp][ni][r] = (oh < a.H && ow < a.W && ep0 + ni * 16 + 4 * fg < a.Cout)
+                                               ? *reinterpret_cast<const f32x4*>(a.res + ((size_t)(img * a.H + oh) * a.W + ow) * a.res_cs + ep0 + ni * 16 + 4 * fg)
+                                               : (f32x4){0.f, 0.f, 0.f, 0.f};
+      }
+  };
+  if (a.res && !RES_PAIRS) {
+#pragma unroll
+    for (int mp = 0; mp < MT / 2; ++mp) load_res(mp);
   }
   float ym = 0.0f;
 #pragma unroll
   for (int mp = 0; mp < MT / 2; ++mp) {
     const int oh = oh_row0 + 2 * mp;
     if (oh >= a.H) continue;
+    if (RES_PAIRS && a.res) load_res(mp);
     float pj[2][3] = {{0.f, 0.f, 0.f}, {0.f, 0.f, 0.f}};
 #pragma unroll
     for (int ni = 0; ni < NT; ++ni) {
@@ -152,7 +156,7 @@
         v[r] += bias_r[ni];
         shdr::act_apply4<0>(v[r], a.act1);
         if (a.scale) v[r] = v[r] * scale_r[ni] + shift_r[ni];
-        if (a.res) v[r] += res_r[mp][ni][r];
+        if (a.res) v[r] += res_r[RES_PAIRS ? 0 : mp][ni][r];
         shdr::act_apply4<0>(v[r], a.act2);
         if (a.y && oh + r < a.H && ow < a.W && n0 + cl < a.Cout)
           *reinterpret_cast<f32x4*>(a.y + ((size_t)(img * a.H + oh + r) * a.W + ow) * a.Cout + n0 + cl) = v[r];
@@ -201,8 +205,10 @@
     }
   }
 #ifndef SHDR_ABL_NO_TAIL
-  if (a.yr)
-    x3_range_out<NW>(a.yr, ow < a.W ? ym : 0.0f, lane, wave, yr_seen, range_lds);
+  if (a.yr) {
+    ym_chain = fmaxf(ym_chain, ow < a.W ? ym : 0.0f);
+    if (range_out) x3_range_out<NW>(a.yr, ym_chain, lane, wave, yr_seen, range_lds);
+  }
 #endif
 }
 
@@ -214,8 +220,8 @@
 __host__ __device__ inline int sx(int col) { return ((col >> 2) & 1) * 2; }
 __device__ __forceinline__ int pcol(int fi) { return fi < 4 ? fi : (fi >= 12 ? fi - 8 : fi + 4); }
 
-template <bool UP, int KH, int KW, bool MP = false, int LOOK = 1>
-__global__ __launch_bounds__(256, 2) void conv_x3_kernel(const X3Args a) {
+template <bool UP, int KH, int KW, bool MP, int LOOK, bool CHN>
+__device__ __forceinline__ void conv_x3_body(const X3Args a) {
   using G = X3G<KH, KW>;
   constexpr int PWID = G::PWID, PPIX = G::PPIX, PJ = G::PJ, PATCH_HALVES = G::PATCH_HALVES, NTAPS = KH * KW;
   static_assert(!UP || (KH == 3 && KW == 3), "the up-sampling prologue belongs to the 3 x 3 stride-1 form");
@@ -229,33 +235,43 @@
 
   const int tid = threadIdx.x, lane = tid & 63;
   const int wave = __builtin_amdgcn_readfirstlane(tid >> 6);
-  const int L = xcd_remap(blockIdx.x, a.nblk_m * a.nblk_n);
+  static_assert(!CHN || (!UP && !MP && KH == 3 && KW == 3 && LOOK == 2), "tile chains are built on the plain nine-tap form with LOOK = 2");
+  const int T = CHN ? a.chain : 1;
+  const int L = xcd_remap(blockIdx.x, (CHN ? a.nchain : a.nblk_m) * a.nblk_n);
   const int pn = L % a.nblk_n;
-  int pm = L / a.nblk_n;
-  const int tx = pm % a.tiles_x;
-  pm /= a.tiles_x;
-  const int ty = pm % a.tiles_y;
-  const int img = pm / a.tiles_y;
-  const int n0 = pn * BN, oh0 = ty * 16, ow0 = tx * 16;
+  int tq = (L / a.nblk_n) * T;
+  const int n0 = pn * BN;
+  int img, oh0, ow0;
+  auto tile_of = [&](int t, int& ti, int& th0, int& tw0) __attribute__((always_inline)) {
+    const int per = a.tiles_x * a.tiles_y;
+    ti = t / per;
+    const int r = t - ti * per;
+    const int ty = T > 1 ? r % a.tiles_y : r / a.tiles_x, tx = T > 1 ? r / a.tiles_y : r % a.tiles_x;
+    th0 = ty * 16;
+    tw0 = tx * 16;
+  };
+  tile_of(tq, img, oh0, ow0);
 
   int ppix[PJ];
   int pdst[PJ];
   int pcnt = 0;
-  auto patch_geometry = [&](int bh, int bw) __attribute__((always_inline)) {
+  auto patch_geometry = [&](int gi, int gh0, int gw0, int bh, int bw, bool first) __attribute__((always_inline)) {
     pcnt = 0;
+    int t0 = tid;
+    if (CHN && !first) asm volatile("" : "+v"(t0));
 #pragma unroll
     for (int j = 0; j < (UP ? 0 : PJ); ++j) {
-      const int p = tid + 256 * j;
+      const int p = t0 + 256 * j;
       const int pix = p >> 3, q = p & 7;
       const int py = pix / PWID, px = pix - py * PWID;
-      const int ih = a.in_s * (oh0 + py) + bh, iw = a.in_s * (ow0 + px) + bw;
+      const int ih = a.in_s * (gh0 + py) + bh, iw = a.in_s * (gw0 + px) + bw;
       const bool ok = pix < PPIX && (unsigned)ih < (unsigned)a.Hin && (unsigned)iw < (unsigned)a.Win;
-      ppix[j] = ok ? (img * a.Hin + ih) * a.Win + iw : -1;
-      pdst[j] = pix < PPIX ? pix * 32 + 8 * ((q >> 1) ^ sx(px)) + 4 * (q & 1) : -1;
+      ppix[j] = ok ? (gi * a.Hin + ih) * a.Win + iw : -1;
+      if (first) pdst[j] = pix < PPIX ? pix * 32 + 8 * ((q >> 1) ^ sx(px)) + 4 * (q & 1) : -1;
       pcnt += __ballot(ppix[j] >= 0) != 0ull;
     }
   };
-  if (!MP) patch_geometry(a.bh, a.bw);
+  if (!MP) patch_geometry(img, oh0, ow0, a.bh, a.bw, true);
   if (!MP && !UP) pcnt = __builtin_amdgcn_readfirstlane(pcnt);
   int lpix[LRJ];
   if (UP) {
@@ -373,25 +389,31 @@
   for (int s = 0; s < NFR; ++s)
 #pragma unroll
     for (int j = 0; j < FJ; ++j) fr[s][j] = (u32x4){0u, 0u, 0u, 0u};
+  bool more = false;
+  int upar = 0;
+  bool chained = false;
+  int nimg = 0, noh0 = 0, now0 = 0;
+  float ym_chain = 0.0f;
   const unsigned foff = 16u * (unsigned)tid + 2048u;
   auto issue_filt = [&](int u, int s) __attribute__((always_inline)) {
-    const _Float16* ub = wbase + (size_t)(u < nunits ? u : nunits - 1) * UNIT_HALVES;
+    const _Float16* ub = wbase + (size_t)(u < nunits ? u : (CHN && more) ? u - nunits : nunits - 1) * UNIT_HALVES;
     asm volatile("global_load_dwordx4 %0, %1, %2 offset:-2048" : "+v"(fr[s][0]) : "v"(foff), "s"(ub) : "memory");
     asm volatile("global_load_dwordx4 %0, %1, %2 offset:2048" : "+v"(fr[s][1]) : "v"(foff), "s"(ub) : "memory");
   };
   constexpr int PJL = UP ? LRJ : PJ;
   constexpr int WB = (LOOK - 1) * FJ;
 #define X3_WAIT_VM(N) asm volatile("s_waitcnt vmcnt(%0)" : : "n"(N) : "memory")
-  auto wait_store_filt = [&](int v, int s, int np, bool st) __attribute__((always_inline)) {
-    if (np < 0) X3_WAIT_VM(0);
+  auto wait_store_filt = [&](int v, int s, int np, bool st, bool skip = false) __attribute__((always_inline)) {
+    if (CHN && skip) {}
+    else if (np < 0) X3_WAIT_VM(0);
     else if (np >= PJL) X3_WAIT_VM(WB + PJL);
     else if (np >= PJL - 1) X3_WAIT_VM(WB + PJL - 1);
     else if (np >= PJL - 2) X3_WAIT_VM(WB + PJL - 2);
     else X3_WAIT_VM(WB);
     asm volatile("" : "+v"(fr[s][0]), "+v"(fr[s][1]) : : "memory");
-    if (st) {
-#pragma unroll
-      for (int j = 0; j < FJ; ++j) *reinterpret_cast<u32x4*>(filt + (v & 1) * UNIT_HALVES + fdst[j]) = fr[s][j];
+    if (st && !(CHN && skip)) {
+#pragma unroll
+      for (int j = 0; j < FJ; ++j) *reinterpret_cast<u32x4*>(filt + ((v ^ upar) & 1) * UNIT_HALVES + fdst[j]) = fr[s][j];
     }
   };
 
@@ -420,7 +442,7 @@
     kw_n = a.ptw[phase];
     nunits = nch * kh_n * kw_n;
     wbase = a.pwp[phase] + (size_t)pn * nunits * UNIT_HALVES;
-    patch_geometry(a.pbh[phase], a.pbw[phase]);
+    patch_geometry(img, oh0, ow0, a.pbh[phase], a.pbw[phase], true);
     pcnt = __builtin_amdgcn_readfirstlane(pcnt);
     if (phase > 0) __syncthreads();
   }
@@ -436,12 +458,17 @@
   wait_store_filt(0, 0, -1, true);
   if (LOOK == 2) issue_filt(1, 1);
   auto chunk = [&](int c, auto cur, auto nxt) __attribute__((always_inline)) {
-    const bool pf = c + DEPTH < nch;
+    const bool nt = CHN && more && c + 1 == nch;
+    if (nt) {
+      patch_geometry(nimg, noh0, now0, a.bh, a.bw, false);
+      pcnt = __builtin_amdgcn_readfirstlane(pcnt);
+    }
+    const bool pf = c + DEPTH < nch || nt;
     zero_patch(cur);
     __builtin_amdgcn_sched_barrier(0);
     issue_filt((MP ? c * kh_n * kw_n : c * NTAPS) + LOOK, LOOK % NFR);
     __builtin_amdgcn_sched_barrier(0);
-    if (pf) load_patch(c + DEPTH, cur, true);
+    if (pf) load_patch(nt ? 0 : c + DEPTH, cur, true);
     __builtin_amdgcn_sched_barrier(0);
     const int np = pf ? pcnt : 0;
 #define X3_SLOT(D) (NFR == 1 ? 0 : (kh * KW + kw + (D)) % NFR)
@@ -451,7 +478,7 @@
     const int u = MP ? (c * kh_n + kh) * kw_n + kw : c * NTAPS + kh * KW + kw;                                                 \
     __syncthreads();                                                                                                           \
     if (!(FIRST) || kw > 0) issue_filt(u + LOOK, X3_SLOT(LOOK));                                                               \
-    const _Float16* F = filt + (u & 1) * UNIT_HALVES;                                                                          \
+    const _Float16* F = filt + ((u ^ upar) & 1) * UNIT_HALVES;                                                                 \
     const int rowh = (wave * MT + kh) * PWID * 32;                                                                             \
                                                                                                                                \
     f16x8 wh[NT], ws[NT], wl[NT], ph[2], pl[2];                                                                                \
@@ -480,7 +507,8 @@
       for (int ni = 0; ni < NT; ++ni) acc[mi][ni] = __builtin_amdgcn_mfma_f32_16x16x32_f16(wl[ni], ph[mi & 1], acc[mi][ni], 0, 0, 0); \
       __builtin_amdgcn_sched_barrier(0);                                                                                       \
     }                                                                                                                          \
-    wait_store_filt(u + 1, X3_SLOT(1), ((FIRST) && kw < LOOK) ? np : 0, u + 1 < nunits);                                       \
+    wait_store_filt(u + 1, X3_SLOT(1), ((FIRST) && kw < LOOK) ? np : 0, u + 1 < nunits || (CHN && more),                      \
+                    CHN && (FIRST) && kw == 0 && chained && c == 0);                                                          \
   }
     if (LOOK == 1) {
       {
@@ -500,12 +528,13 @@
         for (int kw = 0; kw < KW; ++kw) X3_TAP(kh == 0)
       }
       asm volatile("s_waitcnt vmcnt(0)" : "+v"(fr[0][0]), "+v"(fr[0][1]) : : "memory");
+      if (CHN) __builtin_amdgcn_s_waitcnt(0x0f70);
 #pragma unroll
       for (int j = 0; j < FJ; ++j) fr[NFR - 1][j] = fr[0][j];
     }
 #undef X3_TAP
 #undef X3_SLOT
-    if (c + 1 < nch) {
+    if (c + 1 < nch || (CHN && more)) {
       if (UP) {
         park_lr();
         __syncthreads();
@@ -516,22 +545,63 @@
     }
   };
 #pragma unroll 1
-  for (int c = 0; c < nch; c += DEPTH) {
-    chunk(c, Set0{}, Set1{});
-    if (DEPTH == 2 && c + 1 < nch) chunk(c + 1, Set1{}, Set0{});
+  for (int t = 0;; ++t) {
+    if (CHN) {
+      more = t + 1 < T && tq + 1 < a.nblk_m;
+      if (more) tile_of(tq + 1, nimg, noh0, now0);
+    }
+#pragma unroll 1
+    for (int c = 0; c < nch; c += DEPTH) {
+      chunk(c, Set0{}, Set1{});
+      if (DEPTH == 2 && c + 1 < nch) chunk(c + 1, Set1{}, Set0{});
+    }
+    if constexpr (CHN) {
+      if (more) {
+#pragma unroll
+        for (int j = 0; j < FJ; ++j) *reinterpret_cast<u32x4*>(filt + ((1 ^ upar ^ nunits) & 1) * UNIT_HALVES + fdst[j]) = fr[NFR - 1][j];
+      }
+      int pc_e = pc, fg_e = fg;
+      asm volatile("" : "+v"(pc_e), "+v"(fg_e));
+      x3_tile_epilogue<4, true, true>(a, acc, img, oh0 + wave * MT, ow0 + pc_e, pc_e, fg_e, n0, ixs, lane, wave,
+                                      reinterpret_cast<unsigned*>(reinterpret_cast<char*>(xsm) + G::LDS_BYTES), ym_chain, !more);
+      if (!more) break;
+#pragma unroll
+      for (int mi = 0; mi < MT; ++mi)
+#pragma unroll
+        for (int ni = 0; ni < NT; ++ni) acc[mi][ni] = (f32x4){0.f, 0.f, 0.f, 0.f};
+      ++tq;
+      img = nimg; oh0 = noh0; ow0 = now0;
+      upar ^= nunits & 1;
+      chained = true;
+#pragma unroll
+      for (int s = 0; s < NFR; ++s)
+#pragma unroll
+        for (int j = 0; j < FJ; ++j) fr[s][j] = (u32x4){0u, 0u, 0u, 0u};
+    } else {
+      break;
+    }
   }
   }
 #undef pr
 #undef X3_WAIT_VM
 
-  x3_tile_epilogue<4, true>(a, acc, img, oh0 + wave * MT, ow0 + pc, pc, fg, n0, ixs, lane, wave,
-                            reinterpret_cast<unsigned*>(reinterpret_cast<char*>(xsm) + (UP ? G::LDS_BYTES_UP : G::LDS_BYTES)));
+  if constexpr (!CHN)
+    x3_tile_epilogue<4, true>(a, acc, img, oh0 + wave * MT, ow0 + pc, pc, fg, n0, ixs, lane, wave,
+                              reinterpret_cast<unsigned*>(reinterpret_cast<char*>(xsm) + (UP ? G::LDS_BYTES_UP : G::LDS_BYTES)), ym_chain, true);
 }
 
 #undef patch_h
 #undef patch_l
 #undef filt
 #undef lrs
+
+template <bool UP, int KH, int KW, bool MP = false, int LOOK = 1>
+__global__ __launch_bounds__(256, 2) void conv_x3_kernel(const X3Args a) {
+  conv_x3_body<UP, KH, KW, MP, LOOK, false>(a);
+}
+__global__ __launch_bounds__(256, 2) void conv_x3_chain_kernel(const X3Args a) {
+  conv_x3_body<false, 3, 3, false, 2, true>(a);
+}
 
 constexpr int X1_BP = 128;
 template <int NS>
@@ -998,8 +1068,9 @@
   }
 #undef XW_WAIT_VM
 
+  float ym_block = 0.0f;
   x3_tile_epilogue<8, false>(a, acc, img, oh0 + wq * MT, ow0 + pc, pc, fg, n0, ixs, lane, wave,
-                             reinterpret_cast<unsigned*>(reinterpret_cast<char*>(xsm) + XWG::LDS_BYTES + (UP ? XWG::LR_BYTES : 0)));
+                             reinterpret_cast<unsigned*>(reinterpret_cast<char*>(xsm) + XWG::LDS_BYTES + (UP ? XWG::LR_BYTES : 0)), ym_block, true);
 }
 #undef patch_buf
 #undef filt
@@ -1087,13 +1158,42 @@
   hipLaunchKernelGGL((conv_x3_kernel<UP, KH, KW, MP, LOOK>), dim3((unsigned)nblk), dim3(256), lds, st, a);
   return shdr::check_launch("conv_x3_kernel");
 }
+int launch_x3_chain(const X3Args& a, hipStream_t st) {
+  constexpr int lds = X3G<3, 3>::LDS_BYTES + X3G<3, 3>::RANGE_BYTES;
+  static bool attr_done[shdr::kMaxDevices] = {};
+  const int dev_slot = shdr::device_slot();
+  if (!attr_done[dev_slot]) {
+    hipError_t e = hipFuncSetAttribute(reinterpret_cast<const void*>(&conv_x3_chain_kernel), hipFuncAttributeMaxDynamicSharedMemorySize, lds);
+    if (e != hipSuccess) return shdr::fail(SHDR_E_ARCH, "hipFuncSetAttribute: %s", hipGetErrorString(e));
+    attr_done[dev_slot] = true;
+  }
+  if (a.chain < 2 || a.nchain != (a.nblk_m + a.chain - 1) / a.chain) return shdr::fail(SHDR_E_SHAPE, "conv2d_x3: chain %d x %d over %d tiles", a.nchain, a.chain, a.nblk_m);
+  const long nblk = (long)a.nchain * a.nblk_n;
+  if (nblk > 0x7fffffffL) return shdr::fail(SHDR_E_SHAPE, "conv2d_x3: grid of %ld blocks", nblk);
+  hipLaunchKernelGGL(conv_x3_chain_kernel, dim3((unsigned)nblk), dim3(256), lds, st, a);
+  return shdr::check_launch("conv_x3_chain_kernel");
+}
 template <bool UP, int KH, int KW, bool MP = false>
 int launch_x3(const X3Args& a, hipStream_t st) {
   int look = 2;
   if (const char* e = SHDR_ENV("SHDR_X3_LOOK")) look = atoi(e);
   constexpr bool look2 = KH == 3 && KW == 3 && !MP;
+  if (look >= 2 && look2 && !UP && a.chain > 1) return launch_x3_chain(a, st);
   if (look >= 2 && look2) return launch_x3_look<UP, KH, KW, MP, look2 ? 2 : 1>(a, st);
   return launch_x3_look<UP, KH, KW, MP, 1>(a, st);
+}
+
+constexpr int X3_CHAIN_MAX = 8;
+inline int x3_chain_default(int nch) { return nch == 1 ? 2 : (nch == 3 ? 4 : 1); }
+int x3_chain_len(int nch, long tiles, int nblk_n) {
+  if (SHDR_ENV("SHDR_X3_NO_CHAIN")) return 1;
+  long min_tiles = 1024;
+  if (const char* e = SHDR_ENV("SHDR_X3_CHAIN_MIN_TILES")) min_tiles = atol(e);
+  int T = x3_chain_default(nch);
+  if (const char* e = SHDR_ENV("SHDR_X3_CHAIN")) T = atoi(e);
+  T = T < 1 ? 1 : (T > X3_CHAIN_MAX ? X3_CHAIN_MAX : T);
+  while (T > 1 && tiles * nblk_n < min_tiles * T) --T;
+  return T;
 }
 
 int launch_x3_1x1(const X3Args& a0, hipStream_t st) {
@@ -1219,6 +1319,24 @@
   SHDR_REQUIRE(x && prepared, SHDR_E_NULL, "conv2d_x3_input_absmax: null pointer");
   SHDR_REQUIRE(n > 0 && n % 4 == 0 && shdr::aligned16(x), SHDR_E_SHAPE, "conv2d_x3_input_absmax: n must be a positive multiple of 4, x 16-byte aligned");
   return shdr_absmax_f32(x, n, prepared + 2, stream);
+}
+
+static bool x3_wide_3x3(const shdr_conv2d_desc* d, bool up, bool proj, long nblk_m) {
+  long wide_min_blocks = 256, wide_min_cout = up ? XW_UP_MIN_COUT : 512;
+  if (const char* e = SHDR_ENV("SHDR_X3_WIDE_MIN_BLOCKS")) wide_min_blocks = atol(e);
+  if (const char* e = SHDR_ENV("SHDR_X3_WIDE_MIN_COUT")) wide_min_cout = atol(e);
+  return d->stride == 1 && d->Cout % XW_BN == 0 && d->Cout >= wide_min_cout && !proj && nblk_m * (d->Cout / XW_BN) >= wide_min_blocks &&
+         SHDR_ENV("SHDR_X3_SLICED") == nullptr;
+}
+
+extern "C" int shdr_conv2d_x3_chain_f32(const shdr_conv2d_desc* d, int projected) {
+  if (!d || !shdr_conv2d_x3_ok_f32(d) || d->stride != 1 || d->KH != 3 || d->KW != 3 || d->prologue == SHDR_PROLOGUE_BILINEAR2X) return 0;
+  if (const char* e = SHDR_ENV("SHDR_X3_LOOK")) {
+    if (atoi(e) < 2) return 0;
+  }
+  const long tiles = (long)d->N * ((d->Ho + 15) / 16) * ((d->Wo + 15) / 16);
+  if (x3_wide_3x3(d, false, projected != 0, tiles)) return 0;
+  return x3_chain_len((d->C1 + d->C2) / 32, tiles, (d->Cout + 63) / 64);
 }
 
 static int x3_forward(const shdr_conv2d_desc* d, const float* x1, const float* x2, const float* prepared, const float* bias,
@@ -1250,6 +1368,7 @@
   a.tiles_y = (a.H + 15) / 16;
   a.nblk_m = a.N * a.tiles_x * a.tiles_y;
   a.nblk_n = (a.Cout + 63) / 64;
+  a.chain = 1; a.nchain = a.nblk_m;
   a.act1 = d->act1; a.act2 = d->act2;
   a.xr1 = reinterpret_cast<const unsigned*>(x1_range);
   a.xr2 = reinterpret_cast<const unsigned*>(x2 ? x2_range : nullptr);
@@ -1278,11 +1397,11 @@
     return launch_x3<false, 4, 4, true>(a, st);
   }
   if (ph[0].th == 3 && ph[0].tw == 3) {
-    long wide_min_blocks = 256, wide_min_cout = up ? XW_UP_MIN_COUT : 512;
-    if (const char* e = SHDR_ENV("SHDR_X3_WIDE_MIN_BLOCKS")) wide_min_blocks = atol(e);
-    if (const char* e = SHDR_ENV("SHDR_X3_WIDE_MIN_COUT")) wide_min_cout = atol(e);
-    const bool wide = d->stride == 1 && d->Cout % XW_BN == 0 && d->Cout >= wide_min_cout && !proj &&
-                      (long)a.nblk_m * (d->Cout / XW_BN) >= wide_min_blocks && SHDR_ENV("SHDR_X3_SLICED") == nullptr;
+    const bool wide = x3_wide_3x3(d, up, proj != nullptr, a.nblk_m);
+    if (!wide && !up) {
+      a.chain = x3_chain_len(Ct / 32, a.nblk_m, a.nblk_n);
+      a.nchain = (a.nblk_m + a.chain - 1) / a.chain;
+    }
     return wide ? (up ? launch_x3_wide<true>(a, st) : launch_x3_wide<false>(a, st)) : up ? launch_x3<true, 3, 3>(a, st) : launch_x3<false, 3, 3>(a, st);
   }
   if (ph[0].th == 1 && ph[0].tw == 1) {
```

Measured after the change: 951.9. No clear change (-0.3%).
